# adityaX1412/Experiment-YOLO

Hardware: AMD Instinct MI355X
Metric: images/sec (train) DEAL-YOLO-N 640x640 bs=64/GPU (higher is better)
Workload: dtype f16; 1 GPU; DEAL-YOLO-N (yolov8n-ASF-P2P2.yaml) train step 640x640, per-GPU batch 64, fwd+TAL/WIOU+NWD/DFL/BCE loss+bwd+SGD+EMA, BASELINE.json configs[1]; loss_mode=wiou+nwd, settle_steps=18, capture_retries=0, global_batch=64, parallelism=dp1, hipgraph=True

## Files before the change

### experiment-yolo_amd/csrc/conv_wgrad.hip

```cpp
#include <cstdio>
#include "common.h"
#include "dealyolo_hip.h"

typedef short short4v __attribute__((ext_vector_type(4)));
typedef unsigned int u32x4 __attribute__((ext_vector_type(4)));

struct WgArgs {
  const f16* x;
  const f16* dy;
  float* slabs;
  int ldx, lddy;
  int N, H, W, Ho, Wo;
  int cin_p, cout_p;
  int cin_r8, cout_r8;
  int nci_chunks;
  int tiles_x, tiles_y, ntiles;
  long npix;
  const f16* raw;
  f16* draw;
  const float* coef;
  const double* acc;
  float* dgamma;
  float* dbeta;
  int ldraw, cout;
  float count;
  DySegs xs;
  int dy_csplit;
  unsigned dy_plane;
  const f16* wt;
  f16* dx;
  int lddx, dx_acc;
  int dg_mt, dg_rows;
  DySegs dxs;
};

static __device__ __forceinline__ half8 tr_frag(const char* base0, const char* base1) {
  union {
    short4v s[2];
    half8 h;
  } u;
  u.s[0] = __builtin_amdgcn_ds_read_tr16_b64_v4i16((LDS_AS short4v*)(base0));
  u.s[1] = __builtin_amdgcn_ds_read_tr16_b64_v4i16((LDS_AS short4v*)(base1));
  return u.h;
}

static constexpr __host__ __device__ int wg_th(int ks, int stride, int nci, int mtc) {
  if (ks == 1) return (nci + mtc <= 4) ? 8 : 4;
  if (stride == 1) return (nci * mtc <= 1) ? 16 : ((nci + mtc <= 4) ? 8 : 4);
  return (nci * mtc <= 1) ? 8 : ((nci + mtc <= 4) ? 4 : 2);
}

template <int KS, int STRIDE, int NCI, int MTC, int BNF>
__global__ __launch_bounds__(256, (BNF & 8) ? 3 : ((KS == 3 && NCI * MTC >= 16) ? 1 : 2)) void conv_wgrad_kernel(const WgArgs a) {
  constexpr bool FLAT = (KS == 1);
  constexpr bool DG = (BNF & 4) != 0;
  constexpr bool NOX = (BNF & 8) != 0;
  static_assert(!NOX || DG, "the form without X exists for the fused input gradient only");
  constexpr bool BN1 = ((BNF & 3) == 1 || (BNF & 3) == 3);
  constexpr bool XSEG = ((BNF & 3) == 3);
  static_assert(!DG || (KS == 1 && BN1), "the fused input gradient exists for the 1x1 BatchNorm forms");
  constexpr int TAPS = KS * KS;
  constexpr int NCOL = NCI * TAPS;
  constexpr int CPW = (NCOL + 3) / 4;
  constexpr int TH = wg_th(KS, STRIDE, NCI, MTC), TW = 32;
  constexpr int HWX = FLAT ? TH * TW : (TW - 1) * STRIDE + KS;
  constexpr int HHX = FLAT ? 1 : (TH - 1) * STRIDE + KS;
  constexpr int PAD = KS / 2;
  constexpr int CIN_C = 16 * NCI, COUT_C = 16 * MTC;
  constexpr int PSX = (STRIDE == 2) ? CIN_C * 2 + 16 : (((CIN_C / 2 + 7) / 16) * 16 + 8) * 4;
  constexpr int PSY = (((COUT_C / 2 + 7) / 16) * 16 + 8) * 4;
  constexpr int XBYTES = NOX ? 0 : HHX * HWX * PSX, YBYTES = TH * TW * PSY;
  __shared__ __attribute__((aligned(16))) char smem[XBYTES + YBYTES];
  char* const sx = smem;
  char* const sy = smem + XBYTES;
  __shared__ __attribute__((aligned(16))) float sbn[BN1 ? 4 * COUT_C : (BNF == 2 ? 256 * 8 : 4)];
  float bsum[8] = {0.f, 0.f, 0.f, 0.f, 0.f, 0.f, 0.f, 0.f};
  (void)bsum;
  constexpr int DKS = MTC == 4 ? 2 : (MTC == 3 ? 3 : 1), DCPK = (MTC & 1) ? 16 : 32;
  constexpr int DNT = TH / 2;
  constexpr int DNC = 4 * NCI;
  constexpr int DXROW = CIN_C * 2 + 16;
  constexpr int DPPR = CIN_C / 8;
  constexpr int DPIXPASS = 64 / DPPR > 16 ? 16 : 64 / DPPR;
  constexpr int DNPASS = (16 + DPIXPASS - 1) / DPIXPASS;
  __shared__ __attribute__((aligned(16))) char sdx[DG ? 4 * 16 * DXROW : 16];

  const int tid = threadIdx.x, wave = tid >> 6, lane = tid & 63, p = lane & 15, q = lane >> 4;
  const int qq = p >> 2, pp = p & 3;
  const int co_chunk = blockIdx.y / a.nci_chunks, ci_chunk = blockIdx.y - co_chunk * a.nci_chunks;
  const int ci0 = ci_chunk * CIN_C, co0 = co_chunk * COUT_C;

  f32x4 acc[NOX ? 1 : MTC][NOX ? 1 : CPW];
  if (!NOX) {
#pragma unroll
    for (int m = 0; m < MTC; ++m)
#pragma unroll
      for (int c = 0; c < CPW; ++c) acc[NOX ? 0 : m][NOX ? 0 : c] = (f32x4){0.f, 0.f, 0.f, 0.f};
  }
  (void)acc;

  constexpr int NGX = HHX * HWX * (CIN_C / 8), NGY = TH * TW * (COUT_C / 8);
  constexpr int NPX = NOX ? 1 : (NGX + 255) / 256, NPY = (NGY + 255) / 256;
  uint4 pfx[NPX], pfy[NPY];
  uint4 pfr[BN1 ? NPY : 1];
  unsigned roff[BN1 ? NPY : 1];
  int ncur = 0, nnext = 0;
  (void)ncur; (void)nnext;
  unsigned vnext = 0, vcur = 0, ornext = 0, orcur = 0;
  (void)pfr; (void)roff; (void)vnext; (void)vcur; (void)ornext; (void)orcur;
  constexpr unsigned NEVER = 0x80000000u;
  constexpr int CPGX = CIN_C / 8, CPGY = COUT_C / 8;
  unsigned xoff[NPX], yoff[NPY];
  (void)pfx; (void)xoff;
#pragma unroll
  for (int i = 0; i < NPX; ++i) {
    const int id = tid + i * 256;
    const int pixel = id / CPGX, part = id - pixel * CPGX;
    const bool ok = !NOX && id < NGX && ci0 + part * 8 < a.cin_r8;
    const int hy = FLAT ? 0 : pixel / HWX, hx = FLAT ? pixel : pixel - hy * HWX;
    xoff[i] = ok ? (unsigned)(((hy * a.W + hx) * a.ldx + ci0 + part * 8) * 2) : NEVER;
  }
  constexpr bool XIN = XSEG && !NOX;
  const char* xb[XIN ? NPX : 1];
  int xl[XIN ? NPX : 1];
  unsigned xup = 0;
  bool any_up = false;
  if (XIN)
    for (int k = 0; k < a.xs.nseg; ++k) any_up = any_up || (a.xs.acc[k] & 2);
  (void)xb; (void)xl; (void)xup; (void)any_up;
  if (XIN) {
#pragma unroll
    for (int i = 0; i < NPX; ++i) {
      const int id = tid + i * 256;
      const int part = id % CPGX, ch = ci0 + part * 8;
      int sg = 0;
      while (sg + 1 < a.xs.nseg && ch >= a.xs.c_end[sg]) ++sg;
      const int cb = sg ? a.xs.c_end[sg - 1] : 0;
      const bool ok = id < NGX && ch < a.cin_r8;
      xb[XIN ? i : 0] = ok ? reinterpret_cast<const char*>(a.xs.ptr[sg]) + (ch - cb) * 2 : nullptr;
      xl[XIN ? i : 0] = a.xs.ld[sg] * 2;
      if (ok && (a.xs.acc[sg] & 2)) xup |= 1u << i;
    }
  }
#pragma unroll
  for (int i = 0; i < NPY; ++i) {
    const int id = tid + i * 256;
    const int pixel = id / CPGY, part = id - pixel * CPGY;
    const bool ok = id < NGY && co0 + part * 8 < a.cout_r8;
    const int ty = FLAT ? 0 : pixel / TW, tx = FLAT ? pixel : pixel - ty * TW;
    yoff[i] = ok ? (unsigned)(((ty * a.Wo + tx) * a.lddy + co0 + part * 8) * 2) : NEVER;
    if (FLAT && BN1 && a.dy_csplit && ok) {
      const int ch = co0 + part * 8;
      yoff[i] = (unsigned)((tx * a.lddy + (ch < a.dy_csplit ? ch : ch - a.dy_csplit)) * 2) + (ch < a.dy_csplit ? 0u : a.dy_plane);
    }
    if (BN1) roff[i] = ok ? (unsigned)(((ty * a.Wo + tx) * a.ldraw + co0 + part * 8) * 2) : NEVER;
  }
  if (BN1) {
    for (int c = tid; c < COUT_C; c += 256) {
      const int ch = co0 + c;
      float sc = 0.f, sh = 0.f, kb = 0.f, kc = 0.f;
      if (ch < a.cout) {
        double s1 = 0.0, s2 = 0.0;
#pragma unroll
        for (int k = 0; k < DY_BN_COPIES; ++k) {
          s1 += a.acc[(size_t)(k * 2 + 0) * a.cout + ch];
          s2 += a.acc[(size_t)(k * 2 + 1) * a.cout + ch];
        }
        const float mg = (float)(s1 / a.count), mgx = (float)(s2 / a.count);
        sc = a.coef[ch];
        sh = a.coef[a.cout + ch];
        const float mean = a.coef[2 * a.cout + ch], inv = a.coef[3 * a.cout + ch];
        kb = sc * inv * mgx;
        kc = sc * mg - kb * mean;
        if (!NOX && blockIdx.x == 0 && ci_chunk == 0) {
          if (a.dbeta) a.dbeta[ch] = (float)s1;
          if (a.dgamma) a.dgamma[ch] = (float)s2;
        }
      }
      sbn[c] = sc;
      sbn[COUT_C + c] = sh;
      sbn[2 * COUT_C + c] = kb;
      sbn[3 * COUT_C + c] = kc;
    }
    __syncthreads();
  }
  half8 wf[DG ? DKS : 1][DG ? NCI : 1];
  unsigned dboff[DG ? DKS : 1];
  char* dxb = nullptr;
  unsigned dxld2 = 0;
  bool dxacc = false, dxadd = false;
  const int dpix = lane / DPPR, dpiece = lane - dpix * DPPR;
  (void)wf; (void)dboff; (void)dxb; (void)dxld2; (void)dxacc; (void)dxadd; (void)dpix; (void)dpiece;
  if (DG) {
#pragma unroll
    for (int k = 0; k < DKS; ++k) {
      dboff[DG ? k : 0] = (unsigned)((k * DCPK + ((q * 8) & (DCPK - 1))) * 2);
#pragma unroll
      for (int j = 0; j < NCI; ++j) {
        const int ch = ci0 + (p >> 2) * DNC + 4 * j + (p & 3);
        const int gw = 16 * a.dg_mt, g = ch / gw, rem = ch - g * gw;
        const int row = g * gw + ((rem % (4 * a.dg_mt)) >> 2) * 16 + (rem / (4 * a.dg_mt)) * 4 + (rem & 3);
        const int grow = (g * DKS + k) * gw + (row - g * gw);
        half8 v;
#pragma unroll
        for (int e = 0; e < 8; ++e) v[e] = (f16)0.f;
        if (row < a.dg_rows) v = *reinterpret_cast<const half8*>(a.wt + ((size_t)grow * 32 + q * 8));
        wf[DG ? k : 0][DG ? j : 0] = v;
      }
    }
    const int chn = ci0 + dpiece * 8;
    if (lane < DPIXPASS * DPPR && chn < a.cin_r8) {
      if (XSEG) {
        int sg = 0;
        while (sg + 1 < a.dxs.nseg && chn >= a.dxs.c_end[sg]) ++sg;
        const int cb = sg ? a.dxs.c_end[sg - 1] : 0;
        dxb = reinterpret_cast<char*>(const_cast<void*>(a.dxs.ptr[sg])) + (chn - cb) * 2;
        dxld2 = (unsigned)a.dxs.ld[sg] * 2u;
        dxacc = a.dxs.acc[sg] != 0;
      } else {
        dxb = reinterpret_cast<char*>(a.dx) + chn * 2;
        dxld2 = (unsigned)a.lddx * 2u;
        dxacc = a.dx_acc != 0;
      }
    }
    if (XSEG) {
      for (int k = 0; k < a.dxs.nseg; ++k) dxadd = dxadd || a.dxs.acc[k] != 0;
    } else {
      dxadd = a.dx_acc != 0;
    }
  }
  union DU4 { uint4 u; half2_ h[4]; };
  DU4 dold[DG ? DNT : 1][DG ? DNPASS : 1];
  (void)dold;
  auto ld16 = [](__amdgpu_buffer_rsrc_t r, unsigned off) {
    const auto v = __builtin_amdgcn_raw_buffer_load_b128(r, (int)off, 0, 0);
    return *reinterpret_cast<const uint4*>(&v);
  };
  auto prefetch = [&](int tile) {
    if (FLAT) {
      const auto rx = __builtin_amdgcn_make_buffer_rsrc(const_cast<f16*>(a.x), 0, (int)((unsigned)a.npix * (unsigned)a.ldx * 2u), 0x00020000);
      const auto ry = __builtin_amdgcn_make_buffer_rsrc(const_cast<f16*>(a.dy), 0, (int)((unsigned)a.npix * (unsigned)a.lddy * 2u + (a.dy_csplit ? a.dy_plane : 0u)), 0x00020000);
      const unsigned ox = (unsigned)tile * (TH * TW) * a.ldx * 2u, oy = (unsigned)tile * (TH * TW) * a.lddy * 2u;
      if (NOX) {
      } else if (XIN) {
        const long p0 = (long)tile * (TH * TW);
        int n0 = 0, y0 = 0, x0 = 0;
        if (any_up) {
          const int hw = a.H * a.W, g0 = (int)p0;
          n0 = g0 / hw;
          const int r0 = g0 - n0 * hw;
          y0 = r0 / a.W;
          x0 = r0 - y0 * a.W;
        }
        const float invW = 1.0f / (float)a.W, invH = 1.0f / (float)a.H;
#pragma unroll
        for (int i = 0; i < NPX; ++i) {
          const int lp = (tid + i * 256) / CPGX;
          long gp = p0 + lp;
          const bool inside = gp < a.npix;
          if ((xup >> i) & 1u) {
            const int xx = x0 + lp, dy_ = (int)(((float)xx + 0.5f) * invW), x = xx - dy_ * a.W;
            const int yt = y0 + dy_, dn = (int)(((float)yt + 0.5f) * invH), y = yt - dn * a.H;
            gp = ((long)(n0 + dn) * (a.H >> 1) + (y >> 1)) * (a.W >> 1) + (x >> 1);
          }
          const char* src = xb[XIN ? i : 0];
          pfx[i] = (src && inside) ? *reinterpret_cast<const uint4*>(src + gp * xl[XIN ? i : 0]) : make_uint4(0, 0, 0, 0);
        }
      } else {
#pragma unroll
        for (int i = 0; i < NPX; ++i) pfx[i] = ld16(rx, xoff[i] + ox);
      }
#pragma unroll
      for (int i = 0; i < NPY; ++i) pfy[i] = ld16(ry, yoff[i] + oy);
      if (BN1) {
        const unsigned nbytes = (unsigned)a.npix * (unsigned)a.ldraw * 2u;
        const auto rr = __builtin_amdgcn_make_buffer_rsrc(const_cast<f16*>(a.raw), 0, (int)nbytes, 0x00020000);
        ornext = (unsigned)tile * (TH * TW) * a.ldraw * 2u;
        vnext = 0;
#pragma unroll
        for (int i = 0; i < NPY; ++i) {
          const unsigned off = roff[i] + ornext;
          pfr[i] = ld16(rr, off);
          vnext |= (roff[i] != NEVER && off < nbytes) ? (1u << i) : 0u;
        }
      }
    } else {
      const int bx = tile % a.tiles_x;
      const int t2 = tile / a.tiles_x;
      const int n = t2 / a.tiles_y;
      const int oy0 = (t2 % a.tiles_y) * TH, ox0 = bx * TW;
      const int iy0 = oy0 * STRIDE - PAD, ix0 = ox0 * STRIDE - PAD;
      const auto rx = __builtin_amdgcn_make_buffer_rsrc(const_cast<f16*>(a.x) + (size_t)n * a.H * a.W * a.ldx, 0, a.H * a.W * a.ldx * 2, 0x00020000);
      const auto ry = __builtin_amdgcn_make_buffer_rsrc(const_cast<f16*>(a.dy) + (size_t)n * a.Ho * a.Wo * a.lddy, 0, a.Ho * a.Wo * a.lddy * 2, 0x00020000);
      const unsigned ox = (unsigned)((iy0 * a.W + ix0) * a.ldx * 2), oy = (unsigned)((oy0 * a.Wo + ox0) * a.lddy * 2);
      if (ix0 >= 0 && ix0 + HWX <= a.W) {
#pragma unroll
        for (int i = 0; i < NPX; ++i) pfx[i] = ld16(rx, xoff[i] + ox);
      } else {
#pragma unroll
        for (int i = 0; i < NPX; ++i) {
          const int hx = ((tid + i * 256) / CPGX) % HWX;
          pfx[i] = ld16(rx, (unsigned)(ix0 + hx) < (unsigned)a.W ? xoff[i] + ox : NEVER);
        }
      }
      if (ox0 + TW <= a.Wo) {
#pragma unroll
        for (int i = 0; i < NPY; ++i) pfy[i] = ld16(ry, yoff[i] + oy);
      } else {
#pragma unroll
        for (int i = 0; i < NPY; ++i) {
          const int tx = ((tid + i * 256) / CPGY) % TW;
          pfy[i] = ld16(ry, ox0 + tx < a.Wo ? yoff[i] + oy : NEVER);
        }
      }
      if (BN1) {
        const unsigned nbytes = (unsigned)(a.Ho * a.Wo * a.ldraw * 2);
        const auto rr = __builtin_amdgcn_make_buffer_rsrc(const_cast<f16*>(a.raw) + (size_t)n * a.Ho * a.Wo * a.ldraw, 0, (int)nbytes, 0x00020000);
        ornext = (unsigned)((oy0 * a.Wo + ox0) * a.ldraw * 2);
        vnext = 0;
        const bool xfull = ox0 + TW <= a.Wo;
#pragma unroll
        for (int i = 0; i < NPY; ++i) {
          unsigned off = roff[i] == NEVER ? NEVER : roff[i] + ornext;
          if (!xfull) {
            const int tx = ((tid + i * 256) / CPGY) % TW;
            off = ox0 + tx < a.Wo ? off : NEVER;
          }
          pfr[i] = ld16(rr, off);
          vnext |= off < nbytes ? (1u << i) : 0u;
        }
        nnext = n;
      }
    }
  };


  int tile = (!FLAT && !(gridDim.x & 7)) ? (int)(blockIdx.x & 7) * (int)(gridDim.x >> 3) + (int)(blockIdx.x >> 3) : (int)blockIdx.x;
  if (tile < a.ntiles) prefetch(tile);
  for (; tile < a.ntiles; tile += gridDim.x) {
    __syncthreads();
#pragma unroll
    for (int i = 0; i < NPX; ++i) {
      const int id = tid + i * 256;
      if (!NOX && id < NGX) *reinterpret_cast<uint4*>(sx + (id / (CIN_C / 8)) * PSX + (id % (CIN_C / 8)) * 16) = pfx[i];
    }
    if (BN1) {
      vcur = vnext; orcur = ornext; ncur = nnext;
      const unsigned nbytes = FLAT ? (unsigned)a.npix * (unsigned)a.ldraw * 2u : (unsigned)(a.Ho * a.Wo * a.ldraw * 2);
      const auto rd = __builtin_amdgcn_make_buffer_rsrc(FLAT ? a.draw : a.draw + (size_t)ncur * a.Ho * a.Wo * a.ldraw, 0, (int)nbytes, 0x00020000);
#pragma unroll
      for (int i = 0; i < NPY; ++i) {
        const int id = tid + i * 256;
        const int part = id % CPGY;
        const bool valid = (vcur >> i) & 1u;
        const float* cf = sbn + part * 8;
        union { half8 h; uint4 u; u32x4 v; } o;
        o.h = bn_bwd_apply8<DY_ACT_SILU>(*reinterpret_cast<const half8*>(&pfy[i]), *reinterpret_cast<const half8*>(&pfr[i]), cf,
                                         cf + COUT_C, cf + 2 * COUT_C, cf + 3 * COUT_C);
        if (!valid) o.u = make_uint4(0, 0, 0, 0);
        if (id < NGY) *reinterpret_cast<uint4*>(sy + (id / (COUT_C / 8)) * PSY + (id % (COUT_C / 8)) * 16) = o.u;
        if (!DG && ci_chunk == 0 && a.draw) __builtin_amdgcn_raw_buffer_store_b128(o.v, rd, (int)(valid ? roff[i] + orcur : NEVER), 0, 0);
      }
    } else {
#pragma unroll
      for (int i = 0; i < NPY; ++i) {
        const int id = tid + i * 256;
        if (id < NGY) *reinterpret_cast<uint4*>(sy + (id / (COUT_C / 8)) * PSY + (id % (COUT_C / 8)) * 16) = pfy[i];
        if (BNF == 2 && id < NGY) {
          const half8 v = *reinterpret_cast<const half8*>(&pfy[i]);
#pragma unroll
          for (int j = 0; j < 8; ++j) bsum[j] += (float)v[j];
        }
      }
    }
    __syncthreads();
    const long dpix0 = (long)tile * (TH * TW) + wave * (16 * DNT);
    (void)dpix0;
    if (DG && dxadd) {
#pragma unroll
      for (int t = 0; t < DNT; ++t)
#pragma unroll
        for (int ps = 0; ps < DNPASS; ++ps) {
          const int rowi = ps * DPIXPASS + dpix;
          const long gp = dpix0 + t * 16 + rowi;
          const bool ok = dxb && dxacc && rowi < 16 && gp < a.npix;
          dold[DG ? t : 0][DG ? ps : 0].u = ok ? *reinterpret_cast<const uint4*>(dxb + (size_t)gp * dxld2) : make_uint4(0, 0, 0, 0);
        }
      __builtin_amdgcn_sched_barrier(0);
    }
    if (tile + (int)gridDim.x < a.ntiles) prefetch(tile + gridDim.x);
    if constexpr (!NOX) {
    const int kpix = 4 * q + qq;
    half8 af[2][MTC], bf[2];
    auto load_a = [&](int buf, int r) {
#pragma unroll
      for (int m = 0; m < MTC; ++m) {
        const char* b0 = sy + (r * TW + kpix) * PSY + (m * 16 + 4 * pp) * 2;
        af[buf][m] = tr_frag(b0, b0 + 16 * PSY);
      }
    };
    auto load_b = [&](int buf, int r, int c) {
      const int col = wave + 4 * c;
      if (col < NCOL) {
        const int cit = col / TAPS, tap = col - cit * TAPS;
        const int dy = tap / KS, dx = tap - dy * KS;
        const char* b0;
        int step;
        if (FLAT) {
          b0 = sx + (r * TW + kpix) * PSX + (cit * 16 + 4 * pp) * 2;
          step = 16 * PSX;
        } else {
          b0 = sx + ((r * STRIDE + dy) * HWX + kpix * STRIDE + dx) * PSX + (cit * 16 + 4 * pp) * 2;
          step = 16 * STRIDE * PSX;
        }
        bf[buf] = tr_frag(b0, b0 + step);
      }
    };
    load_a(0, 0);
    load_b(0, 0, 0);
#pragma unroll
    for (int r = 0; r < TH; ++r) {
      if (r + 1 < TH) load_a((r + 1) & 1, r + 1);
#pragma unroll
      for (int c = 0; c < CPW; ++c) {
        const int lin = r * CPW + c;
        if (c + 1 < CPW) load_b((lin + 1) & 1, r, c + 1);
        else if (r + 1 < TH) load_b((lin + 1) & 1, r + 1, 0);
        __builtin_amdgcn_sched_barrier(0);
        if (wave + 4 * c < NCOL) {
#pragma unroll
          for (int m = 0; m < MTC; ++m)
            acc[NOX ? 0 : m][NOX ? 0 : c] = __builtin_amdgcn_mfma_f32_16x16x32_f16(af[r & 1][m], bf[lin & 1], acc[NOX ? 0 : m][NOX ? 0 : c], 0, 0, 0);
        }
        __builtin_amdgcn_sched_barrier(0);
      }
    }
    }
    if (DG) {
      half8 db[DNT][DKS];
#pragma unroll
      for (int t = 0; t < DNT; ++t)
#pragma unroll
        for (int k = 0; k < DKS; ++k)
          db[t][k] = *reinterpret_cast<const half8*>(sy + ((wave * DNT + t) * 16 + p) * PSY + dboff[DG ? k : 0]);
      f32x4 dacc[NCI][DNT];
#pragma unroll
      for (int j = 0; j < NCI; ++j)
#pragma unroll
        for (int t = 0; t < DNT; ++t) dacc[j][t] = (f32x4){0.f, 0.f, 0.f, 0.f};
#pragma unroll
      for (int k = 0; k < DKS; ++k)
#pragma unroll
        for (int j = 0; j < NCI; ++j)
#pragma unroll
          for (int t = 0; t < DNT; ++t)
            dacc[j][t] = __builtin_amdgcn_mfma_f32_16x16x32_f16(wf[DG ? k : 0][DG ? j : 0], db[t][k], dacc[j][t], 0, 0, 0);
      typedef uint2 __attribute__((may_alias)) uint2_a;
      typedef uint4 __attribute__((may_alias)) uint4_a;
      char* const xs = sdx + wave * (16 * DXROW);
      char* const xw = xs + p * DXROW + q * (DNC * 2);
      const int rrow = dpix < 16 ? dpix : 15;
      auto lds_order = []() {
        __builtin_amdgcn_fence(__ATOMIC_RELEASE, "wavefront", "local");
        __builtin_amdgcn_wave_barrier();
        __builtin_amdgcn_fence(__ATOMIC_ACQUIRE, "wavefront", "local");
      };
#pragma unroll
      for (int t = 0; t < DNT; ++t) {
        union { half2_ h[DNC / 2]; uint2 u2[DNC / 4]; } hv;
#pragma unroll
        for (int j = 0; j < NCI; ++j) {
          const f32x2 lo = {dacc[j][t][0], dacc[j][t][1]}, hi = {dacc[j][t][2], dacc[j][t][3]};
          hv.h[j * 2] = __builtin_convertvector(lo, half2_);
          hv.h[j * 2 + 1] = __builtin_convertvector(hi, half2_);
        }
        lds_order();
#pragma unroll
        for (int j = 0; j < NCI; ++j) reinterpret_cast<uint2_a*>(xw)[j] = hv.u2[j];
        lds_order();
#pragma unroll
        for (int ps = 0; ps < DNPASS; ++ps) {
          const int rowi = ps * DPIXPASS + dpix;
          const int rr = ps * DPIXPASS + rrow < 16 ? ps * DPIXPASS + rrow : 15;
          DU4 v;
          v.u = *reinterpret_cast<const uint4_a*>(xs + rr * DXROW + dpiece * 16);
          const long gp = dpix0 + t * 16 + rowi;
          if (dxadd) {
#pragma unroll
            for (int k = 0; k < 4; ++k)
              v.h[k] = __builtin_convertvector(__builtin_convertvector(v.h[k], f32x2) + __builtin_convertvector(dold[DG ? t : 0][DG ? ps : 0].h[k], f32x2), half2_);
          }
          if (dxb && rowi < 16 && gp < a.npix) *reinterpret_cast<uint4*>(dxb + (size_t)gp * dxld2) = v.u;
        }
      }
    }
  }

  if (BNF == 2 && ci_chunk == 0) {
    __syncthreads();
#pragma unroll
    for (int j = 0; j < 8; ++j) sbn[tid * 8 + j] = bsum[j];
    __syncthreads();
    if (tid < COUT_C && co0 + tid < a.cout) {
      const int part = tid >> 3, j = tid & 7;
      float t = 0.f;
      for (int k = part; k < 256; k += CPGY) t += sbn[k * 8 + j];
      unsafeAtomicAdd(const_cast<double*>(a.acc) + (size_t)(blockIdx.x % DY_BN_COPIES) * a.cout + co0 + tid, (double)t);
    }
  }
  if constexpr (NOX) return;
  float* slab = a.slabs + (size_t)blockIdx.x * TAPS * a.cout_p * a.cin_p;
#pragma unroll
  for (int c = 0; c < CPW; ++c) {
    const int col = wave + 4 * c;
    if (col < NCOL) {
      const int cit = col / TAPS, tap = col - cit * TAPS;
#pragma unroll
      for (int m = 0; m < MTC; ++m)
#pragma unroll
        for (int r = 0; r < 4; ++r) {
          const int co = co0 + m * 16 + q * 4 + r, ci = ci0 + cit * 16 + p;
          slab[((size_t)tap * a.cout_p + co) * a.cin_p + ci] = acc[NOX ? 0 : m][NOX ? 0 : c][r];
        }
    }
  }
}

static __device__ __forceinline__ void wgrad_reduce_block(int block, const float* slabs, int nslabs, float* dw, int cout, int cin,
                                                          int taps, int cout_p, int cin_p, int accumulate,
                                                          int ld_taps, int ld_cphys, int ld_cin) {
  const int lane = threadIdx.x & 63, grp = threadIdx.x >> 6;
  const long S = (long)taps * cout_p * cin_p;
  const long o = (long)block * 64 + lane;
  float s0 = 0.f, s1 = 0.f, s2 = 0.f, s3 = 0.f;
  if (o < S) {
    const float* p = slabs + o;
    int k = grp;
    for (; k + 12 < nslabs; k += 16) {
      s0 += p[(long)k * S];
      s1 += p[(long)(k + 4) * S];
      s2 += p[(long)(k + 8) * S];
      s3 += p[(long)(k + 12) * S];
    }
    for (; k < nslabs; k += 4) s0 += p[(long)k * S];
  }
  __shared__ float red[4][64];
  red[grp][lane] = (s0 + s1) + (s2 + s3);
  __syncthreads();
  if (grp == 0 && o < S) {
    const float tot = (red[0][lane] + red[1][lane]) + (red[2][lane] + red[3][lane]);
    const int ci = (int)(o % cin_p);
    const long t = o / cin_p;
    const int co = (int)(t % cout_p), tap = (int)(t / cout_p);
    if (ld_taps) {
      const int n = ci / ld_cphys, ch = ci - n * ld_cphys;
      if (co < cout && n < ld_taps && ch < ld_cin) {
        float* d = dw + ((long)co * ld_cin + ch) * ld_taps + n;
        *d = accumulate ? *d + tot : tot;
      }
    } else if (co < cout && ci < cin) {
      float* d = dw + ((long)co * cin + ci) * taps + tap;
      *d = accumulate ? *d + tot : tot;
    }
  }
}

__global__ __launch_bounds__(256) void wgrad_reduce_kernel(const float* slabs, int nslabs, float* dw, int cout, int cin,
                                                           int taps, int cout_p, int cin_p, int accumulate,
                                                           int ld_taps, int ld_cphys, int ld_cin) {
  wgrad_reduce_block(blockIdx.x, slabs, nslabs, dw, cout, cin, taps, cout_p, cin_p, accumulate, ld_taps, ld_cphys, ld_cin);
}

struct WgReduceDesc {
  const float* slabs;
  float* dw;
  int nslabs, cout, cin, taps, cout_p, cin_p, accumulate, ld_taps, ld_cphys, ld_cin;
  int first_block, bias_c;
  const double* bias_acc;
  float* dbias;
};
__global__ __launch_bounds__(256) void wgrad_reduce_batched_kernel(const WgReduceDesc* descs, int n) {
  int lo = 0, hi = n - 1;
  while (lo < hi) {
    const int mid = (lo + hi + 1) >> 1;
    if (descs[mid].first_block <= (int)blockIdx.x) lo = mid;
    else hi = mid - 1;
  }
  const WgReduceDesc d = descs[lo];
  if (d.bias_c > 0 && (int)blockIdx.x == d.first_block && (int)threadIdx.x < d.bias_c) {
    double t = 0.0;
#pragma unroll
    for (int k = 0; k < DY_BN_COPIES; ++k) t += d.bias_acc[(size_t)k * d.bias_c + threadIdx.x];
    d.dbias[threadIdx.x] = (float)t;
  }
  wgrad_reduce_block(blockIdx.x - d.first_block, d.slabs, d.nslabs, d.dw, d.cout, d.cin, d.taps, d.cout_p, d.cin_p, d.accumulate,
                     d.ld_taps, d.ld_cphys, d.ld_cin);
}
extern "C" int dy_wgrad_reduce_desc_bytes(void) { return (int)sizeof(WgReduceDesc); }
static void wgrad_geometry(int cin, int cout, int ks, int stride, int* cin_p, int* cout_p, int* nci, int* mtc, long npix_out = 0);
extern "C" int dy_wgrad_reduce_desc_fill(void* desc, const float* slabs, int nslabs, float* dw, int cin, int cout, int ks, int stride,
                                         int accumulate, int ld_taps, int ld_cphys, int ld_cin, int first_block) {
  if (!desc || !slabs || !dw || nslabs < 1) return DY_ERR_ARG;
  int cp, op, nci, mtc;
  const int cin_eff = ld_taps ? ld_taps * ld_cphys : cin;
  wgrad_geometry(cin_eff, cout, ld_taps ? 1 : ks, ld_taps ? 1 : stride, &cp, &op, &nci, &mtc);
  const int taps = ld_taps ? 1 : ks * ks;
  WgReduceDesc* d = reinterpret_cast<WgReduceDesc*>(desc);
  *d = WgReduceDesc{slabs, dw, nslabs, cout, cin_eff, taps, op, cp, accumulate, ld_taps, ld_cphys, ld_cin, first_block, 0, nullptr, nullptr};
  return cdiv(taps * op * cp, 64);
}
extern "C" int dy_wgrad_reduce_desc_bias(void* desc, const double* bias_acc, float* dbias, int c) {
  if (!desc || !bias_acc || !dbias || c < 1 || c > 256) return DY_ERR_ARG;
  WgReduceDesc* d = reinterpret_cast<WgReduceDesc*>(desc);
  d->bias_acc = bias_acc; d->dbias = dbias; d->bias_c = c;
  return DY_OK;
}
extern "C" int dy_wgrad_reduce_batched(const void* descs_device, int n, int total_blocks, hipStream_t stream) {
  if (n <= 0 || total_blocks <= 0 || !descs_device) return DY_ERR_ARG;
  hipLaunchKernelGGL(wgrad_reduce_batched_kernel, dim3(total_blocks), dim3(256), 0, stream, (const WgReduceDesc*)descs_device, n);
  DY_CHECK_LAUNCH();
  return DY_OK;
}

template <int KS, int STRIDE, int NCI, int MTC>
static int launch_wgrad(const WgArgs& a, int gx, int gy, hipStream_t s) {
  if (a.wt) {
    if constexpr (KS == 1) {
      if (!a.raw || gy != a.nci_chunks) return DY_ERR_ARG;
      if (!a.x) {
        if (a.dxs.nseg > 0) hipLaunchKernelGGL((conv_wgrad_kernel<KS, STRIDE, NCI, MTC, 15>), dim3(gx, gy), dim3(256), 0, s, a);
        else hipLaunchKernelGGL((conv_wgrad_kernel<KS, STRIDE, NCI, MTC, 13>), dim3(gx, gy), dim3(256), 0, s, a);
      } else if (a.xs.nseg > 0) hipLaunchKernelGGL((conv_wgrad_kernel<KS, STRIDE, NCI, MTC, 7>), dim3(gx, gy), dim3(256), 0, s, a);
      else hipLaunchKernelGGL((conv_wgrad_kernel<KS, STRIDE, NCI, MTC, 5>), dim3(gx, gy), dim3(256), 0, s, a);
    } else return DY_ERR_ARG;
  } else if (a.raw && a.xs.nseg > 0) {
    if constexpr (KS == 1) hipLaunchKernelGGL((conv_wgrad_kernel<KS, STRIDE, NCI, MTC, 3>), dim3(gx, gy), dim3(256), 0, s, a);
    else return DY_ERR_ARG;
  } else if (a.raw) hipLaunchKernelGGL((conv_wgrad_kernel<KS, STRIDE, NCI, MTC, 1>), dim3(gx, gy), dim3(256), 0, s, a);
  else if (a.acc && MTC != 3) hipLaunchKernelGGL((conv_wgrad_kernel<KS, STRIDE, NCI, MTC, 2>), dim3(gx, gy), dim3(256), 0, s, a);
  else if (a.acc) return DY_ERR_ARG;
  else hipLaunchKernelGGL((conv_wgrad_kernel<KS, STRIDE, NCI, MTC, 0>), dim3(gx, gy), dim3(256), 0, s, a);
  DY_CHECK_LAUNCH();
  return DY_OK;
}
template <int KS, int STRIDE>
static int dispatch_wgrad(int nci, int mtc, const WgArgs& a, int gx, int gy, hipStream_t s) {
#define DY_CASE(I, M) \
  if (nci == I && mtc == M) return launch_wgrad<KS, STRIDE, I, M>(a, gx, gy, s);
  DY_CASE(1, 1) DY_CASE(1, 2) DY_CASE(1, 4)
  DY_CASE(2, 1) DY_CASE(2, 2) DY_CASE(2, 4)
  if (!(KS == 3 && STRIDE == 2)) { DY_CASE(4, 1) DY_CASE(4, 2) DY_CASE(4, 4) }
  if (KS == 1) {
    DY_CASE(3, 1) DY_CASE(3, 2) DY_CASE(3, 4) DY_CASE(1, 3) DY_CASE(2, 3) DY_CASE(4, 3) DY_CASE(3, 3)
  }
#undef DY_CASE
  return DY_ERR_ARG;
}

static int wgrad_per_cu(int ks, int nci, int mtc) {
  static const int light = getenv("DY_WGRAD_LIGHT_WGS") ? atoi(getenv("DY_WGRAD_LIGHT_WGS")) : 2;
  if (ks == 3 && nci * mtc >= 16) return 1;
  return nci * mtc <= 2 ? light : 2;
}
static long wgrad_columns(int ks, int nci, int mtc, int cp, int op) {
  const int gy = (cp / (16 * nci)) * (op / (16 * mtc));
  const int per_cu = wgrad_per_cu(ks, nci, mtc);
  int gx = (256 * per_cu) / gy;
  return gx < 32 ? 32 : gx;
}
static void wgrad_geometry(int cin, int cout, int ks, int stride, int* cin_p, int* cout_p, int* nci, int* mtc, long npix_out) {
  *cin_p = (cin + 15) / 16 * 16;
  *cout_p = (cout + 15) / 16 * 16;
  const int cit = *cin_p / 16, cot = *cout_p / 16;
  const int cap = (ks == 3 && stride == 2) ? 2 : 4;
  *nci = (cit % 4 == 0 && cap >= 4) ? 4 : ((ks == 1 && cit % 3 == 0) ? 3 : (cit % 2 == 0 ? 2 : 1));
  *mtc = cot % 4 == 0 ? 4 : ((ks == 1 && cot % 3 == 0) ? 3 : (cot % 2 == 0 ? 2 : 1));
  static const bool split = !(getenv("DY_WGRAD_SPLIT") && atoi(getenv("DY_WGRAD_SPLIT")) == 0);
  static const double f = getenv("DY_WGRAD_SPLIT_F") ? atof(getenv("DY_WGRAD_SPLIT_F")) : 2.0;
  if (!split || npix_out <= 0) return;
  const double wbytes = (double)ks * ks * *cin_p * *cout_p * 4.0;
  const double act = (double)npix_out * (*cin_p * stride * stride + *cout_p) * 2.0;
  while (2.0 * wgrad_columns(ks, *nci, *mtc, *cin_p, *cout_p) * wbytes > f * act) {
    if (*mtc % 2 == 0 && *mtc >= *nci) *mtc /= 2;
    else if (*nci % 2 == 0) *nci /= 2;
    else if (*mtc % 2 == 0) *mtc /= 2;
    else break;
  }
}

extern "C" int dy_wgrad_workspace(int n, int h, int w, int cin, int cout, int ks, int stride, int* nslabs,
                                  long* slab_elems) {
  int cp, op, nci, mtc;
  const int pad = ks / 2, Ho = (h + 2 * pad - ks) / stride + 1, Wo = (w + 2 * pad - ks) / stride + 1;
  wgrad_geometry(cin, cout, ks, stride, &cp, &op, &nci, &mtc, (long)n * Ho * Wo);
  const int th = wg_th(ks, stride, nci, mtc);
  int ntiles;
  if (ks == 1) ntiles = (int)(((long)n * Ho * Wo + th * 32 - 1) / (th * 32));
  else ntiles = cdiv(Wo, 32) * cdiv(Ho, th) * n;
  *slab_elems = (long)ks * ks * cp * op;
  const int gy = (cp / (16 * nci)) * (op / (16 * mtc));
  const int per_cu = wgrad_per_cu(ks, nci, mtc);
  int gx = (256 * per_cu) / gy;
  if (gx < 32) gx = 32;
  static const int tpb = getenv("DY_WGRAD_TPB") ? atoi(getenv("DY_WGRAD_TPB")) : 1;
  if (tpb > 1 && gx > ntiles / tpb) gx = ntiles / tpb > 32 ? ntiles / tpb : (ntiles < 32 ? ntiles : 32);
  if (gx > ntiles) gx = ntiles;
  if (gx < 1) gx = 1;
  *nslabs = gx;
  return DY_OK;
}

struct WgBnHost {
  const void* raw; void* draw; const float* coef; const double* acc; float* dgamma; float* dbeta; int ldraw; float count;
  const DySegs* xs = nullptr;
  int dy_csplit = 0;
  unsigned dy_plane = 0;
  const void* wt = nullptr; void* dx = nullptr; int lddx = 0, dx_acc = 0; const DySegs* dxs = nullptr;
  bool dgrad_only = false;
};
static int conv_wgrad_impl(const void* x, int ldx, const void* dy, int lddy, float* slabs, float* dw, int n, int h, int w,
                           int cin, int cout, int ks, int stride, int accumulate, int ld_taps, int ld_cphys, int ld_cin,
                           hipStream_t stream, const WgBnHost* bn = nullptr);

extern "C" int dy_wgrad_kernel_name(int cin, int cout, int ks, int stride, char* out, int cap) {
  if (!out || cap < 8) return DY_ERR_ARG;
  int cp, op, nci, mtc;
  wgrad_geometry(cin, cout, ks, stride, &cp, &op, &nci, &mtc);
  snprintf(out, cap, "conv_wgrad_kernel<%d, %d, %d, %d, 0>", ks, stride, nci, mtc);
  return DY_OK;
}

extern "C" int dy_wgrad_kernel_name_at(int n, int h, int w, int cin, int cout, int ks, int stride, char* out, int cap) {
  if (!out || cap < 8) return DY_ERR_ARG;
  int cp, op, nci, mtc;
  wgrad_geometry(cin, cout, ks, stride, &cp, &op, &nci, &mtc,
                 (long)n * ((h + 2 * (ks / 2) - ks) / stride + 1) * ((w + 2 * (ks / 2) - ks) / stride + 1));
  snprintf(out, cap, "conv_wgrad_kernel<%d, %d, %d, %d, 0>", ks, stride, nci, mtc);
  return DY_OK;
}

extern "C" int dy_conv_wgrad(const void* x, int ldx, const void* dy, int lddy, float* slabs, float* dw, int n, int h,
                             int w, int cin, int cout, int ks, int stride, int accumulate, hipStream_t stream) {
  return conv_wgrad_impl(x, ldx, dy, lddy, slabs, dw, n, h, w, cin, cout, ks, stride, accumulate, 0, 0, 0, stream);
}
extern "C" int dy_conv_wgrad_ld(const void* x, int ldx, const void* dy, int lddy, float* slabs, float* dw, int n, int h,
                                int w, int cout, int ld_cin, int ld_taps, int ld_cphys, int accumulate, hipStream_t stream) {
  return conv_wgrad_impl(x, ldx, dy, lddy, slabs, dw, n, h, w, ld_taps * ld_cphys, cout, 1, 1, accumulate, ld_taps, ld_cphys,
                         ld_cin, stream);
}

extern "C" int dy_conv_wgrad_bn(const void* x, int ldx, const void* dy, int lddy, const void* raw, int ldraw, void* draw,
                                const float* coef, const double* acc, float* dgamma, float* dbeta, float count, float* slabs,
                                float* dw, int n, int h, int w, int cin, int cout, int ks, int stride, int accumulate,
                                hipStream_t stream) {
  if (!raw || !coef || !acc || (ldraw & 7) || ((uintptr_t)raw & 15) || ((uintptr_t)draw & 15) || (cout & 15)) return DY_ERR_ARG;
  const WgBnHost bn{raw, draw, coef, acc, dgamma, dbeta, ldraw, count};
  return conv_wgrad_impl(x, ldx, dy, lddy, slabs, dw, n, h, w, cin, cout, ks, stride, accumulate, 0, 0, 0, stream, &bn);
}
extern "C" int dy_conv_wgrad_bias(const void* x, int ldx, const void* dy, int lddy, double* bias_acc, float* slabs, float* dw, int n,
                                  int h, int w, int cin, int cout, int ks, int stride, int accumulate, hipStream_t stream) {
  if (!bias_acc) return DY_ERR_ARG;
  const WgBnHost bn{nullptr, nullptr, nullptr, bias_acc, nullptr, nullptr, 0, 1.f};
  return conv_wgrad_impl(x, ldx, dy, lddy, slabs, dw, n, h, w, cin, cout, ks, stride, accumulate, 0, 0, 0, stream, &bn);
}
extern "C" int dy_conv1x1_wgrad_bn_segs(const DySegs* xs, const void* dy, int lddy, const void* raw, int ldraw, void* draw, const float* coef,
                                        const double* acc, float* dgamma, float* dbeta, float count, float* slabs, float* dw, int n, int h,
                                        int w, int cin, int cout, int accumulate, hipStream_t stream) {
  if (!raw || !coef || !acc || (ldraw & 7) || ((uintptr_t)raw & 15) || ((uintptr_t)draw & 15) || (cout & 15)) return DY_ERR_ARG;
  if (!xs || xs->nseg < 1 || xs->nseg > DY_MAX_SEGS || xs->c_end[xs->nseg - 1] != cin) return DY_ERR_ARG;
  for (int k = 0; k < xs->nseg; ++k)
    if ((xs->c_end[k] & 7) || (xs->ld[k] & 7) || !xs->ptr[k] || ((uintptr_t)xs->ptr[k] & 15) || xs->c_end[k] <= (k ? xs->c_end[k - 1] : 0) ||
        ((xs->acc[k] & 2) && ((h | w) & 1))) return DY_ERR_ARG;
  WgBnHost bn{raw, draw, coef, acc, dgamma, dbeta, ldraw, count};
  bn.xs = xs;
  return conv_wgrad_impl(xs->ptr[0], 8, dy, lddy, slabs, dw, n, h, w, cin, cout, 1, 1, accumulate, 0, 0, 0, stream, &bn);
}
extern "C" int dy_conv1x1_wgrad_bn_planes(const DySegs* xs, const void* x, int ldx, const void* dy, const void* dy2, int lddy, int csplit,
                                          const void* raw, int ldraw, void* draw, const float* coef, const double* acc, float* dgamma,
                                          float* dbeta, float count, float* slabs, float* dw, int n, int h, int w, int cin, int cout,
                                          int accumulate, hipStream_t stream) {
  if (!raw || !coef || !acc || (ldraw & 7) || ((uintptr_t)raw & 15) || ((uintptr_t)draw & 15) || (cout & 15)) return DY_ERR_ARG;
  if (!dy || !dy2 || (csplit & 7) || csplit <= 0 || csplit >= cout || ((uintptr_t)dy2 & 15)) return DY_ERR_ARG;
  const long plane = (const char*)dy2 - (const char*)dy;
  if (plane < (long)n * h * w * lddy * 2 || plane + (double)n * h * w * lddy * 2.0 >= 2147483648.0) return DY_ERR_ARG;
  if (xs) {
    if (xs->nseg < 1 || xs->nseg > DY_MAX_SEGS || xs->c_end[xs->nseg - 1] != cin) return DY_ERR_ARG;
    for (int k = 0; k < xs->nseg; ++k)
      if ((xs->c_end[k] & 7) || (xs->ld[k] & 7) || !xs->ptr[k] || ((uintptr_t)xs->ptr[k] & 15) || xs->c_end[k] <= (k ? xs->c_end[k - 1] : 0) ||
          ((xs->acc[k] & 2) && ((h | w) & 1))) return DY_ERR_ARG;
  }
  WgBnHost bn{raw, draw, coef, acc, dgamma, dbeta, ldraw, count};
  bn.xs = xs;
  bn.dy_csplit = csplit; bn.dy_plane = (unsigned)plane;
  return conv_wgrad_impl(xs ? xs->ptr[0] : x, xs ? 8 : ldx, dy, lddy, slabs, dw, n, h, w, cin, cout, 1, 1, accumulate, 0, 0, 0, stream, &bn);
}

struct WgDgPlan { int ok, nci, mtc, dg_mt, dg_rows; };
static WgDgPlan wgrad_dgrad_plan(int n, int h, int w, int cin, int cout) {
  WgDgPlan r{};
  if (n < 1 || h < 1 || w < 1 || cin < 8 || (cin & 7) || cout < 16 || (cout & 15) || cout > 64) return r;
  int cp, op, nci, mtc;
  wgrad_geometry(cin, cout, 1, 1, &cp, &op, &nci, &mtc, (long)n * h * w);
  if (16 * mtc != op) return r;
  int gcin, gcout, cc, nch, mt, ng, kst, pe;
  if (dy_conv_geometry(cout, cin, 1, 1, &gcin, &gcout, &cc, &nch, &mt, &ng, &kst, &pe) != DY_OK) return r;
  const int dks = mtc == 4 ? 2 : (mtc == 3 ? 3 : 1), dcpk = (mtc & 1) ? 16 : 32;
  if (gcin != cout || nch * kst != dks || (cc < 32 ? cc : 32) != dcpk || gcout < cp) return r;
  r.ok = 1; r.nci = nci; r.mtc = mtc; r.dg_mt = mt; r.dg_rows = gcout;
  return r;
}
extern "C" int dy_conv1x1_wgrad_dgrad_supported(int n, int h, int w, int cin, int cout) { return wgrad_dgrad_plan(n, h, w, cin, cout).ok; }
extern "C" int dy_wgrad_dgrad_kernel_name(int n, int h, int w, int cin, int cout, int segs, char* out, int cap) {
  const WgDgPlan pl = wgrad_dgrad_plan(n, h, w, cin, cout);
  if (!out || cap < 8 || !pl.ok) return DY_ERR_ARG;
  snprintf(out, cap, "conv_wgrad_kernel<1, 1, %d, %d, %d>", pl.nci, pl.mtc, segs ? 7 : 5);
  return DY_OK;
}
static bool dgrad_segs_valid(const DySegs* xs, const DySegs* dxs) {
  if (!xs || !dxs || dxs->nseg != xs->nseg) return false;
  for (int k = 0; k < dxs->nseg; ++k) {
    const int cb = k ? dxs->c_end[k - 1] : 0;
    if (dxs->c_end[k] != xs->c_end[k] || (dxs->ld[k] & 7) || dxs->ld[k] < dxs->c_end[k] - cb || !dxs->ptr[k] || ((uintptr_t)dxs->ptr[k] & 15) ||
        (dxs->acc[k] & ~1)) return false;
  }
  return true;
}
static bool segs_in_valid(const DySegs* xs, int cin, int h, int w) {
  if (!xs || xs->nseg < 1 || xs->nseg > DY_MAX_SEGS || xs->c_end[xs->nseg - 1] != cin) return false;
  for (int k = 0; k < xs->nseg; ++k)
    if ((xs->c_end[k] & 7) || (xs->ld[k] & 7) || !xs->ptr[k] || ((uintptr_t)xs->ptr[k] & 15) || xs->c_end[k] <= (k ? xs->c_end[k - 1] : 0) ||
        ((xs->acc[k] & 2) && ((h | w) & 1))) return false;
  return true;
}
static int dgrad_only_columns(int ntiles, int gy) {
  int gx = (256 * 3) / (gy > 0 ? gy : 1);
  if (gx < 32) gx = 32;
  if (gx > ntiles) gx = ntiles;
  return gx < 1 ? 1 : gx;
}
extern "C" int dy_conv1x1_dgrad_bn_supported(int n, int h, int w, int cin, int cout) { return wgrad_dgrad_plan(n, h, w, cin, cout).ok; }
extern "C" int dy_dgrad_only_kernel_name(int n, int h, int w, int cin, int cout, int segs, char* out, int cap) {
  const WgDgPlan pl = wgrad_dgrad_plan(n, h, w, cin, cout);
  if (!out || cap < 8 || !pl.ok) return DY_ERR_ARG;
  snprintf(out, cap, "conv_wgrad_kernel<1, 1, %d, %d, %d>", pl.nci, pl.mtc, segs ? 15 : 13);
  return DY_OK;
}
extern "C" int dy_conv1x1_dgrad_bn(const void* dy, const void* dy2, int lddy, int csplit, const void* raw, int ldraw, const float* coef,
                                   const double* acc, float count, const void* w_packed_t, void* dx, int lddx, int dx_accumulate,
                                   const DySegs* dxs, int n, int h, int w, int cin, int cout, hipStream_t stream) {
  if (!dy || !raw || !coef || !acc || (ldraw & 7) || ((uintptr_t)raw & 15)) return DY_ERR_ARG;
  if (!w_packed_t || ((uintptr_t)w_packed_t & 15) || !wgrad_dgrad_plan(n, h, w, cin, cout).ok) return DY_ERR_ARG;
  long plane = 0;
  if (dy2) {
    if ((csplit & 7) || csplit <= 0 || csplit >= cout || ((uintptr_t)dy2 & 15)) return DY_ERR_ARG;
    plane = (const char*)dy2 - (const char*)dy;
    if (plane < (long)n * h * w * lddy * 2 || plane + (double)n * h * w * lddy * 2.0 >= 2147483648.0) return DY_ERR_ARG;
  } else if (csplit) {
    return DY_ERR_ARG;
  }
  if (dxs) {
    if (dxs->nseg < 1 || dxs->nseg > DY_MAX_SEGS || dxs->c_end[dxs->nseg - 1] != cin) return DY_ERR_ARG;
    for (int k = 0; k < dxs->nseg; ++k) {
      const int cb = k ? dxs->c_end[k - 1] : 0;
      if ((dxs->c_end[k] & 7) || dxs->c_end[k] <= cb || (dxs->ld[k] & 7) || dxs->ld[k] < dxs->c_end[k] - cb || !dxs->ptr[k] ||
          ((uintptr_t)dxs->ptr[k] & 15) || (dxs->acc[k] & ~1)) return DY_ERR_ARG;
    }
  } else if (!dx || ((uintptr_t)dx & 15) || (lddx & 7) || lddx < cin || (double)n * h * w * lddx * 2.0 >= 2147483648.0) {
    return DY_ERR_ARG;
  }
  WgBnHost bn{raw, nullptr, coef, acc, nullptr, nullptr, ldraw, count};
  bn.dy_csplit = dy2 ? csplit : 0; bn.dy_plane = (unsigned)plane;
  bn.wt = w_packed_t; bn.dxs = dxs; bn.dx = dxs ? nullptr : dx; bn.lddx = lddx; bn.dx_acc = dx_accumulate != 0;
  bn.dgrad_only = true;
  return conv_wgrad_impl(nullptr, 8, dy, lddy, nullptr, nullptr, n, h, w, cin, cout, 1, 1, 0, 0, 0, 0, stream, &bn);
}
extern "C" int dy_conv1x1_wgrad_dgrad_bn(const void* x, int ldx, const void* dy, int lddy, const void* raw, int ldraw, const float* coef,
                                         const double* acc, float* dgamma, float* dbeta, float count, float* slabs, float* dw,
                                         const void* w_packed_t, void* dx, int lddx, int dx_accumulate, int n, int h, int w, int cin,
                                         int cout, int accumulate, hipStream_t stream) {
  if (!raw || !coef || !acc || (ldraw & 7) || ((uintptr_t)raw & 15)) return DY_ERR_ARG;
  if (!w_packed_t || ((uintptr_t)w_packed_t & 15) || !dx || ((uintptr_t)dx & 15) || (lddx & 7) || lddx < cin) return DY_ERR_ARG;
  if (!wgrad_dgrad_plan(n, h, w, cin, cout).ok || (double)n * h * w * lddx * 2.0 >= 2147483648.0) return DY_ERR_ARG;
  WgBnHost bn{raw, nullptr, coef, acc, dgamma, dbeta, ldraw, count};
  bn.wt = w_packed_t; bn.dx = dx; bn.lddx = lddx; bn.dx_acc = dx_accumulate != 0;
  return conv_wgrad_impl(x, ldx, dy, lddy, slabs, dw, n, h, w, cin, cout, 1, 1, accumulate, 0, 0, 0, stream, &bn);
}
extern "C" int dy_conv1x1_wgrad_dgrad_bn_segs(const DySegs* xs, const void* dy, int lddy, const void* raw, int ldraw, const float* coef,
                                              const double* acc, float* dgamma, float* dbeta, float count, float* slabs, float* dw,
                                              const void* w_packed_t, const DySegs* dxs, int n, int h, int w, int cin, int cout,
                                              int accumulate, hipStream_t stream) {
  if (!raw || !coef || !acc || (ldraw & 7) || ((uintptr_t)raw & 15)) return DY_ERR_ARG;
  if (!w_packed_t || ((uintptr_t)w_packed_t & 15) || !segs_in_valid(xs, cin, h, w) || !dgrad_segs_valid(xs, dxs)) return DY_ERR_ARG;
  if (!wgrad_dgrad_plan(n, h, w, cin, cout).ok) return DY_ERR_ARG;
  WgBnHost bn{raw, nullptr, coef, acc, dgamma, dbeta, ldraw, count};
  bn.xs = xs; bn.wt = w_packed_t; bn.dxs = dxs;
  return conv_wgrad_impl(xs->ptr[0], 8, dy, lddy, slabs, dw, n, h, w, cin, cout, 1, 1, accumulate, 0, 0, 0, stream, &bn);
}
extern "C" int dy_conv1x1_wgrad_dgrad_bn_planes(const DySegs* xs, const void* x, int ldx, const void* dy, const void* dy2, int lddy, int csplit,
                                                const void* raw, int ldraw, const float* coef, const double* acc, float* dgamma,
                                                float* dbeta, float count, float* slabs, float* dw, const void* w_packed_t, void* dx,
                                                int lddx, int dx_accumulate, const DySegs* dxs, int n, int h, int w, int cin, int cout,
                                                int accumulate, hipStream_t stream) {
  if (!raw || !coef || !acc || (ldraw & 7) || ((uintptr_t)raw & 15)) return DY_ERR_ARG;
  if (!dy || !dy2 || (csplit & 7) || csplit <= 0 || csplit >= cout || ((uintptr_t)dy2 & 15)) return DY_ERR_ARG;
  const long plane = (const char*)dy2 - (const char*)dy;
  if (plane < (long)n * h * w * lddy * 2 || plane + (double)n * h * w * lddy * 2.0 >= 2147483648.0) return DY_ERR_ARG;
  if (!w_packed_t || ((uintptr_t)w_packed_t & 15) || !wgrad_dgrad_plan(n, h, w, cin, cout).ok) return DY_ERR_ARG;
  if (xs) {
    if (!segs_in_valid(xs, cin, h, w) || !dgrad_segs_valid(xs, dxs)) return DY_ERR_ARG;
  } else if (dxs || !dx || ((uintptr_t)dx & 15) || (lddx & 7) || lddx < cin || (double)n * h * w * lddx * 2.0 >= 2147483648.0) {
    return DY_ERR_ARG;
  }
  WgBnHost bn{raw, nullptr, coef, acc, dgamma, dbeta, ldraw, count};
  bn.xs = xs; bn.dy_csplit = csplit; bn.dy_plane = (unsigned)plane;
  bn.wt = w_packed_t; bn.dxs = xs ? dxs : nullptr; bn.dx = xs ? nullptr : dx; bn.lddx = lddx; bn.dx_acc = dx_accumulate != 0;
  return conv_wgrad_impl(xs ? xs->ptr[0] : x, xs ? 8 : ldx, dy, lddy, slabs, dw, n, h, w, cin, cout, 1, 1, accumulate, 0, 0, 0, stream, &bn);
}
extern "C" int dy_conv_wgrad_ld_bn(const void* x, int ldx, const void* dy, int lddy, const void* raw, int ldraw, void* draw,
                                   const float* coef, const double* acc, float* dgamma, float* dbeta, float count, float* slabs,
                                   float* dw, int n, int h, int w, int cout, int ld_cin, int ld_taps, int ld_cphys, int accumulate,
                                   hipStream_t stream) {
  if (!raw || !coef || !acc || (ldraw & 7) || ((uintptr_t)raw & 15) || ((uintptr_t)draw & 15) || (cout & 15)) return DY_ERR_ARG;
  const WgBnHost bn{raw, draw, coef, acc, dgamma, dbeta, ldraw, count};
  return conv_wgrad_impl(x, ldx, dy, lddy, slabs, dw, n, h, w, ld_taps * ld_cphys, cout, 1, 1, accumulate, ld_taps, ld_cphys, ld_cin,
                         stream, &bn);
}

static int conv_wgrad_impl(const void* x, int ldx, const void* dy, int lddy, float* slabs, float* dw, int n, int h, int w,
                           int cin, int cout, int ks, int stride, int accumulate, int ld_taps, int ld_cphys, int ld_cin,
                           hipStream_t stream, const WgBnHost* bn) {
  if (!(ks == 1 || ks == 3) || !(stride == 1 || stride == 2) || (ks == 1 && stride != 1)) return DY_ERR_ARG;
  if ((ldx & 7) || (lddy & 7) || ((uintptr_t)x & 15) || ((uintptr_t)dy & 15)) return DY_ERR_ALIGN;
  const bool dgrad_only = bn && bn->dgrad_only;
  if (dgrad_only != (x == nullptr) || (dgrad_only && (!bn->wt || slabs || dw))) return DY_ERR_ARG;
  if ((ks == 1 ? (double)n : 1.0) * h * w * (ldx > lddy ? ldx : lddy) * 2.0 >= 2147483648.0) return DY_ERR_ARG;
  int cp, op, nci, mtc;
  wgrad_geometry(cin, cout, ks, stride, &cp, &op, &nci, &mtc,
                 (long)n * ((h + 2 * (ks / 2) - ks) / stride + 1) * ((w + 2 * (ks / 2) - ks) / stride + 1));
  WgArgs a{};
  a.x = (const f16*)x; a.dy = (const f16*)dy; a.slabs = slabs; a.ldx = ldx; a.lddy = lddy;
  a.N = n; a.H = h; a.W = w;
  const int pad = ks / 2;
  a.Ho = (h + 2 * pad - ks) / stride + 1;
  a.Wo = (w + 2 * pad - ks) / stride + 1;
  a.cin_p = cp; a.cout_p = op;
  a.cin_r8 = (cin + 7) / 8 * 8; a.cout_r8 = (cout + 7) / 8 * 8;
  if (bn) {
    if ((ks == 1 ? (double)n : 1.0) * a.Ho * a.Wo * bn->ldraw * 2.0 >= 2147483648.0) return DY_ERR_ARG;
    a.raw = (const f16*)bn->raw; a.draw = (f16*)bn->draw; a.coef = bn->coef; a.acc = bn->acc;
    a.dgamma = bn->dgamma; a.dbeta = bn->dbeta; a.ldraw = bn->ldraw; a.count = bn->count;
    a.cout = bn->raw ? cout : (cout + 7) / 8 * 8;
    if (bn->xs) a.xs = *bn->xs;
    a.dy_csplit = bn->dy_csplit; a.dy_plane = bn->dy_plane;
    if (bn->wt) {
      const WgDgPlan pl = wgrad_dgrad_plan(n, h, w, cin, cout);
      if (!pl.ok || pl.nci != nci || pl.mtc != mtc || ks != 1 || ld_taps) return DY_ERR_ARG;
      a.wt = (const f16*)bn->wt; a.dx = (f16*)bn->dx; a.lddx = bn->lddx; a.dx_acc = bn->dx_acc;
      a.dg_mt = pl.dg_mt; a.dg_rows = pl.dg_rows;
      if (bn->dxs) a.dxs = *bn->dxs;
    }
  }
  a.nci_chunks = cp / (16 * nci);
  const int nco_chunks = op / (16 * mtc);
  const int th = wg_th(ks, stride, nci, mtc);
  if (ks == 1) {
    a.npix = (long)n * a.Ho * a.Wo;
    a.ntiles = (int)((a.npix + th * 32 - 1) / (th * 32));
  } else {
    a.tiles_x = cdiv(a.Wo, 32);
    a.tiles_y = cdiv(a.Ho, th);
    a.ntiles = a.tiles_x * a.tiles_y * n;
  }
  int nslabs;
  long slab_elems;
  dy_wgrad_workspace(n, h, w, cin, cout, ks, stride, &nslabs, &slab_elems);
  const int gy = a.nci_chunks * nco_chunks;
  if (dgrad_only) nslabs = dgrad_only_columns(a.ntiles, gy);
  int rc;
  if (ks == 1) rc = dispatch_wgrad<1, 1>(nci, mtc, a, nslabs, gy, stream);
  else if (stride == 1) rc = dispatch_wgrad<3, 1>(nci, mtc, a, nslabs, gy, stream);
  else rc = dispatch_wgrad<3, 2>(nci, mtc, a, nslabs, gy, stream);
  if (rc != DY_OK) return rc;
  if (!dw) return DY_OK;
  const int total = ks * ks * op * cp;
  hipLaunchKernelGGL(wgrad_reduce_kernel, dim3(cdiv(total, 64)), dim3(256), 0, stream, slabs, nslabs, dw, cout, cin,
                     ks * ks, op, cp, accumulate, ld_taps, ld_cphys, ld_cin);
  DY_CHECK_LAUNCH();
  return DY_OK;
}
```

### experiment-yolo_amd/ultralytics/hip/__init__.py

```python
from __future__ import annotations

import ctypes as C
import os
import sys

_FLAG = "DEBUG_CLR_GRAPH_PACKET_CAPTURE"


def _hip_already_up():
    t = sys.modules.get("torch")
    try:
        return bool(t is not None and t.cuda.is_initialized())
    except Exception:
        return False


if os.environ.get(_FLAG) is None and not _hip_already_up():
    os.environ[_FLAG] = "0"
GRAPH_SAFE = os.environ.get(_FLAG) == "0"

_HERE = os.path.dirname(os.path.abspath(__file__))
LIB_PATH = os.environ.get("DY_HIP_LIB") or os.path.normpath(os.path.join(_HERE, "..", "..", "csrc", "libdealyolo_hip.so"))

DY_EPI_STATS, DY_EPI_BIAS, DY_EPI_SILU, DY_EPI_F32OUT, DY_EPI_ACCUM, DY_EPI_STATS_ACC = 1, 2, 4, 8, 16, 32
DY_BN_COPIES = 16
DY_ACT_NONE, DY_ACT_SILU, DY_ACT_LEAKY = 0, 1, 2
_ERR = {-1: "DY_ERR_ARG (unsupported shape/argument)", -2: "DY_ERR_LAUNCH (HIP launch failed)",
        -3: "DY_ERR_ALIGN (pointer/stride alignment)", -4: "DY_ERR_CAPACITY (more items than the kernel's table holds)"}

vp, i32, f32, i64, sz = C.c_void_p, C.c_int, C.c_float, C.c_long, C.c_size_t
ip = C.POINTER(C.c_int)
lp = C.POINTER(C.c_long)


class DyLossArgs(C.Structure):
    _fields_ = [("nl", i32), ("B", i32), ("nc", i32), ("ncp", i32), ("nmax", i32),
                ("box", vp * 4), ("cls", vp * 4), ("dbox", vp * 4), ("dcls", vp * 4),
                ("H", i32 * 4), ("W", i32 * 4), ("stride", f32 * 4),
                ("t_batch_idx", vp), ("t_cls", vp), ("t_boxes", vp), ("n_targets", i32), ("n_targets_dev", vp),
                ("img_w", f32), ("img_h", f32), ("hyp_box", f32), ("hyp_cls", f32), ("hyp_dfl", f32),
                ("use_wiou", i32), ("use_nwd", i32), ("iou_ratio", f32), ("gscale", vp), ("scalars", vp),
                ("workspace", vp), ("dbox_rows_only", i32), ("box_from_input", i32), ("box_in", vp * 4), ("box_in_ld", i32 * 4),
                ("box_w", vp * 4), ("box_b", vp * 4), ("box_in_coef", vp * 4),
                ("box_family", i32), ("box_ltype", i32), ("box_fm", i32), ("box_modifier", i32), ("inner_ratio", f32),
                ("focaler_d", f32), ("focaler_u", f32), ("shape_scale", f32), ("piou_lambda", f32)]


class DySegs(C.Structure):
    _fields_ = [("nseg", i32), ("c_end", i32 * 8), ("ld", i32 * 8), ("acc", i32 * 8), ("ptr", vp * 8)]


SIGNATURES = {
    "dy_abi_version": (i32, []),
    "dy_loss_args_bytes": (i32, []),
    "dy_conv_geometry": (i32, [i32, i32, i32, i32, ip, ip, ip, ip, ip, ip, ip, ip]),
    "dy_pack_weights": (i32, [vp, vp, vp, i32, i32, i32, i32, i32, vp]),
    "dy_pack_desc_bytes": (i32, []),
    "dy_pack_desc_fill": (i32, [vp, vp, vp, vp, i32, i32, i32, i32, i32, i32, i32, i32]),
    "dy_pack_weights_batched": (i32, [vp, i32, i32, vp]),
    "dy_conv_forward": (i32, [vp, i32, vp, vp, vp, i32, vp, i32, i32, i32, i32, i32, i32, i32, i32, i32, i32, i32, ip, vp]),
    "dy_segs_bytes": (i32, []),
    "dy_conv1x1_segs_supported": (i32, [i32, i32, C.POINTER(DySegs)]),
    "dy_conv1x1_forward_segs": (i32, [C.POINTER(DySegs), vp, vp, vp, i32, vp, i32, i32, i32, i32, i32, i32, vp]),
    "dy_conv1x1_input_grad_segs": (i32, [vp, i32, vp, C.POINTER(DySegs), i32, i32, i32, i32, i32, vp]),
    "dy_conv1x1_wgrad_bn_segs": (i32, [C.POINTER(DySegs), vp, i32, vp, i32, vp, vp, vp, vp, vp, f32, vp, vp, i32, i32, i32, i32, i32, i32, vp]),
    "dy_conv_res_supported": (i32, [i32, i32, i32, i32]),
    "dy_conv_forward_res": (i32, [vp, i32, vp, vp, vp, i32, vp, i32, i32, i32, i32, i32, i32, i32, i32, vp]),
    "dy_conv_red_supported": (i32, [i32, i32, i32]),
    "dy_conv_input_grad_red": (i32, [vp, i32, vp, vp, i32, i32, i32, i32, i32, i32, i32, vp, i32, vp, vp, i32, vp]),
    "dy_conv_kernel_name": (i32, [i32, i32, i32, i32, C.c_char_p, i32]),
    "dy_conv1x1_segs_kernel_name": (i32, [i32, i32, C.POINTER(DySegs), C.c_char_p, i32]),
    "dy_conv1x1_kernel_name_live": (i32, [i32, i32, i32, i32, i32, i32, C.POINTER(DySegs), C.POINTER(DySegs), C.c_char_p, i32]),
    "dy_conv_kernel_name_at": (i32, [i32, i32, i32, i32, i32, i32, i32, C.c_char_p, i32]),
    "dy_wgrad_kernel_name": (i32, [i32, i32, i32, i32, C.c_char_p, i32]),
    "dy_wgrad_kernel_name_at": (i32, [i32, i32, i32, i32, i32, i32, i32, C.c_char_p, i32]),
    "dy_wgrad_reduce_desc_bytes": (i32, []),
    "dy_wgrad_reduce_desc_fill": (i32, [vp, vp, i32, vp, i32, i32, i32, i32, i32, i32, i32, i32, i32]),
    "dy_wgrad_reduce_batched": (i32, [vp, i32, i32, vp]),
    "dy_match_predictions": (i32, [vp, vp, vp, vp, vp, i32, vp, vp, i32, i32, i32, i32, vp, vp, vp, vp]),
    "dy_box_iou": (i32, [vp, i32, vp, i32, vp, vp]),
    "dy_conv_num_partials": (i32, [i32, i32, i32, i32, i32, i32, i32, i32]),
    "dy_wgrad_workspace": (i32, [i32, i32, i32, i32, i32, i32, i32, ip, lp]),
    "dy_conv_wgrad": (i32, [vp, i32, vp, i32, vp, vp, i32, i32, i32, i32, i32, i32, i32, i32, vp]),
    "dy_stem_grid": (i32, [i32, i32, i32]),
    "dy_stem_forward": (i32, [vp, vp, vp, i32, vp, i32, i32, i32, f32, vp]),
    "dy_stem_forward_eval": (i32, [vp, vp, vp, vp, i32, i32, i32, i32, f32, i32, vp]),
    "dy_stem_wgrad_bn": (i32, [vp, vp, i32, vp, i32, vp, vp, vp, vp, f32, vp, i32, i32, i32, f32, vp]),
    "dy_conv_wgrad_bias": (i32, [vp, i32, vp, i32, vp, vp, vp, i32, i32, i32, i32, i32, i32, i32, i32, vp]),
    "dy_wgrad_reduce_desc_bias": (i32, [vp, vp, vp, i32]),
    "dy_conv_wgrad_bn": (i32, [vp, i32, vp, i32, vp, i32, vp, vp, vp, vp, vp, f32, vp, vp, i32, i32, i32, i32, i32, i32, i32, i32, vp]),
    "dy_conv_wgrad_ld_bn": (i32, [vp, i32, vp, i32, vp, i32, vp, vp, vp, vp, vp, f32, vp, vp, i32, i32, i32, i32, i32, i32, i32, i32, vp]),
    "dy_ldconv_sample": (i32, [vp, i32, vp, i32, vp, vp, i32, i32, i32, i32, i32, i32, i32, i32, i32, vp]),
    "dy_ldconv_sample_backward": (i32, [vp, i32, vp, i32, vp, vp, i32, vp, vp, i32, i32, i32, i32, i32, i32, i32, i32, i32, vp]),
    "dy_ldconv_sample_backward_gather": (i32, [vp, i32, vp, i32, vp, vp, i32, vp, i32, i32, vp, vp, i32, vp, i32, i32, i32, i32, i32, i32, i32, i32, i32, vp]),
    "dy_f32_to_f16_add": (i32, [vp, vp, i32, i64, i32, i32, vp]),
    "dy_pack_weights_ld": (i32, [vp, vp, i32, i32, i32, i32, i32, vp]),
    "dy_conv_wgrad_ld": (i32, [vp, i32, vp, i32, vp, vp, i32, i32, i32, i32, i32, i32, i32, i32, vp]),
    "dy_bn_finalize": (i32, [vp, i32, f32, vp, i32, f32, vp, i32, f32, vp, vp, vp, vp, vp, i32, f32, f32, f32, i32, vp]),
    "dy_bn_eval_coef": (i32, [vp, vp, vp, vp, vp, i32, f32, vp]),
    "dy_bn_act_apply": (i32, [vp, i32, vp, i32, vp, i32, vp, i64, i32, i32, vp]),
    "dy_bn_act_apply_acc": (i32, [vp, i32, vp, i32, vp, i32, vp, vp, vp, vp, vp, vp, i64, i32, i32, f32, f32, f32, vp]),
    "dy_bn_act_bwd_reduce_acc": (i32, [vp, i32, vp, i32, vp, vp, i64, i32, i32, vp, i32, i32, vp]),
    "dy_bn_act_bwd_apply_acc": (i32, [vp, i32, vp, i32, vp, i32, vp, vp, vp, vp, i64, i32, i32, f32, vp]),
    "dy_bn_act_bwd_reduce": (i32, [vp, i32, vp, i32, vp, vp, i32, i64, i32, i32, ip, vp]),
    "dy_bn_bwd_finalize": (i32, [vp, i32, vp, vp, vp, i32, f32, i32, vp]),
    "dy_bn_act_bwd_apply": (i32, [vp, i32, vp, i32, vp, i32, vp, vp, i64, i32, i32, i32, vp]),
    "dy_bn_finalize_ld": (i32, [vp, i32, i32, vp, vp, vp, vp, vp, i32, f32, f32, f32, i32, vp, vp]),
    "dy_bn_act_apply_c": (i32, [vp, i32, vp, i32, vp, i32, vp, i64, i32, i32, vp]),
    "dy_bn_act_bwd_reduce_c": (i32, [vp, i32, vp, i32, vp, vp, i32, i64, i32, i32, ip, vp]),
    "dy_bn_bwd_finalize_ld": (i32, [vp, i32, i32, vp, vp, vp, i32, f32, i32, vp]),
    "dy_bn_act_bwd_apply_c": (i32, [vp, i32, vp, i32, vp, i32, vp, vp, i64, i32, i32, i32, vp]),
    "dy_pad_f32": (i32, [vp, i32, vp, i32, vp]),
    "dy_import_image": (i32, [vp, vp, i32, i32, i32, i32, i32, f32, vp]),
    "dy_crop_letterbox_u8": (i32, [vp, i32, i32, vp, vp, i32, i32, vp, vp]),
    "dy_refine_select": (i32, [vp, vp, vp, vp, vp, i32, C.c_float, C.c_float, vp, vp, vp]),
    "dy_nms_hard": (i32, [vp, vp, vp, i32, C.c_float, vp, vp]),
    "dy_crop_letterbox_u8_multi": (i32, [vp, vp, vp, vp, vp, vp, i32, i32, vp, vp]),
    "dy_refine_select_multi": (i32, [vp, vp, vp, vp, vp, vp, vp, i32, vp, vp, vp]),
    "dy_two_stage_merge": (i32, [vp, vp, vp, vp, vp, vp, i32, f32, vp, vp, f32, i32, vp, vp, vp, vp]),
    "dy_tile_gather_f32": (i32, [vp, vp, vp, vp, vp, vp, vp, i32, i32, vp, vp]),
    "dy_tile_merge": (i32, [vp, vp, vp, vp, vp, i32, i32, i32, f32, i32, i32, vp, vp, vp, vp, vp]),
    "dy_warp_import_u8": (i32, [vp, vp, vp, i32, i32, i32, vp]),
    "dy_warp_slot_bytes": (i32, []),
    "dy_import_image_u8": (i32, [vp, vp, i32, i32, i32, i32, vp, vp, vp, vp]),
    "dy_add": (i32, [vp, i32, vp, i32, vp, i32, vp, i32, i64, i32, vp]),
    "dy_upsample2x": (i32, [vp, i32, vp, i32, i32, i32, i32, i32, i32, i32, vp]),
    "dy_space_to_depth": (i32, [vp, i32, vp, i32, i32, i32, i32, i32, i32, i32, vp]),
    "dy_dysample_supported": (i32, [i32, i32, i32]),
    "dy_dysample": (i32, [vp, i32, vp, i32, vp, i32, i32, i32, i32, i32, i32, i32, vp]),
    "dy_dysample_backward": (i32, [vp, i32, vp, i32, vp, i32, vp, i32, i32, vp, vp, i32, vp, i32, i32, i32, i32, i32, i32, i32, vp]),
    "dy_maxpool5": (i32, [vp, i32, vp, i32, vp, i32, i32, i32, i32, vp]),
    "dy_maxpool5_backward": (i32, [vp, i32, vp, vp, i32, i32, i32, i32, i32, i32, vp]),
    "dy_bn_group_max": (i32, []),
    "dy_bn_act_apply_acc_split": (i32, [vp, i32, vp, i32, vp, i32, i32, vp, vp, vp, vp, vp, vp, i64, i32, i32, f32, f32, f32, vp]),
    "dy_bn_act_bwd_reduce_acc_split": (i32, [vp, i32, vp, i32, i32, vp, i32, vp, vp, i64, i32, i32, vp]),
    "dy_conv1x1_wgrad_bn_planes": (i32, [C.POINTER(DySegs), vp, i32, vp, vp, i32, i32, vp, i32, vp, vp, vp, vp, vp, f32, vp, vp, i32, i32, i32,
                                         i32, i32, i32, vp]),
    "dy_conv1x1_wgrad_dgrad_supported": (i32, [i32, i32, i32, i32, i32]),
    "dy_wgrad_dgrad_kernel_name": (i32, [i32, i32, i32, i32, i32, i32, C.c_char_p, i32]),
    "dy_conv1x1_wgrad_dgrad_bn": (i32, [vp, i32, vp, i32, vp, i32, vp, vp, vp, vp, f32, vp, vp, vp, vp, i32, i32, i32, i32, i32, i32, i32, i32, vp]),
    "dy_conv1x1_wgrad_dgrad_bn_segs": (i32, [C.POINTER(DySegs), vp, i32, vp, i32, vp, vp, vp, vp, f32, vp, vp, vp, C.POINTER(DySegs), i32, i32,
                                             i32, i32, i32, i32, vp]),
    "dy_conv1x1_wgrad_dgrad_bn_planes": (i32, [C.POINTER(DySegs), vp, i32, vp, vp, i32, i32, vp, i32, vp, vp, vp, vp, f32, vp, vp, vp, vp, i32, i32,
                                               C.POINTER(DySegs), i32, i32, i32, i32, i32, i32, vp]),
    "dy_conv1x1_dgrad_bn_supported": (i32, [i32, i32, i32, i32, i32]),
    "dy_dgrad_only_kernel_name": (i32, [i32, i32, i32, i32, i32, i32, C.c_char_p, i32]),
    "dy_conv1x1_dgrad_bn": (i32, [vp, vp, i32, i32, vp, i32, vp, vp, f32, vp, vp, i32, i32, C.POINTER(DySegs), i32, i32, i32, i32, i32, vp]),
    "dy_bn_act_apply_acc_group": (i32, [i32, vp, vp, vp, vp, vp, vp, vp, vp, vp, vp, vp, vp, vp, vp, vp, vp]),
    "dy_bn_act_bwd_reduce_acc_group": (i32, [i32, vp, vp, vp, vp, vp, vp, vp, vp, vp]),
    "dy_bn_act_bwd_reduce_rows": (i32, [vp, i32, vp, i32, vp, vp, i32, i32, i32, i32, vp, i32, i32, vp]),
    "dy_head_box_decode": (i32, [vp, i32, vp, vp, vp, vp, i32, i32, i32, i32, i32, i32, i32, vp]),
    "dy_cls_head_supported": (i32, [i32, i32]),
    "dy_cls_head_slabs": (i32, []),
    "dy_cls_head_forward": (i32, [vp, i32, vp, vp, vp, vp, i64, i32, i32, vp]),
    "dy_cls_head_backward": (i32, [vp, i32, vp, vp, vp, vp, i32, i32, vp, vp, i64, i32, i32, vp]),
    "dy_head_box_decode_levels": (i32, [i32, vp, vp, vp, vp, vp, vp, i32, vp, i32, vp, vp, i32, i32, vp]),
    "dy_conv1x1_rows_backward_levels": (i32, [i32, vp, vp, vp, vp, vp, vp, i32, vp, vp, vp, vp, vp, vp, vp, i32, vp, vp, i32, i32, vp]),
    "dy_cls_head_forward_levels": (i32, [i32, vp, vp, vp, vp, vp, vp, vp, i32, i32, vp]),
    "dy_cls_head_backward_levels": (i32, [i32, vp, vp, vp, vp, vp, vp, vp, vp, vp, vp, vp, i32, i32, vp]),
    "dy_conv1x1_rows_supported": (i32, [i32, i32]),
    "dy_conv1x1_rows_slabs": (i32, [i32, i32, i32]),
    "dy_conv1x1_rows_backward": (i32, [vp, i32, vp, vp, i32, vp, i32, i32, vp, vp, i32, i32, vp, vp, i32, i32, i32, i32, i32, vp]),
    "dy_sppf_pool3_supported": (i32, [i32, i32, i32]),
    "dy_sppf_pool3": (i32, [vp, i32, i32, vp, vp, vp, i32, i32, i32, vp]),
    "dy_sppf_pool3_backward": (i32, [vp, i32, i32, vp, vp, vp, i32, i32, i32, i32, i32, i32, vp]),
    "dy_scalseq_tail": (i32, [vp, i32, vp, i32, vp, i32, vp, i32, vp, i32, vp, i32, i32, i32, i32, vp]),
    "dy_scalseq_tail_backward": (i32, [vp, i32, vp, i32, vp, i32, vp, i32, vp, i32, vp, vp, vp, i32, i32, i32, i32, i32,
                                       i32, i32, ip, vp]),
    "dy_scalseq_tail_backward_all": (i32, [vp, i32, vp, i32, vp, i32, vp, i32, vp, i32, vp, i32, vp, i32, vp, vp, vp, i32, i32,
                                           i32, i32, i32, i32, ip, vp]),
    "dy_scalseq_bwd_grid_cap": (i32, [i32]),
    "dy_zoom_pool": (i32, [vp, i32, vp, i32, i32, i32, i32, i32, vp]),
    "dy_zoom_pool_backward": (i32, [vp, i32, vp, i32, vp, i32, i32, i32, i32, i32, i32, vp]),
    "dy_copy_slice": (i32, [vp, i32, vp, i32, i64, i32, vp]),
    "dy_fill_zero": (i32, [vp, sz, vp]),
    "dy_loss_workspace_bytes": (sz, [i32, i32, i32]),
    "dy_loss_workspace_layout": (i32, [i32, i32, i32, C.POINTER(sz), C.POINTER(sz), C.POINTER(sz)]),
    "dy_detection_loss": (i32, [C.POINTER(DyLossArgs), vp]),
    "dy_tal_assign": (i32, [vp, ip, ip, C.POINTER(f32), i32, i32, i32, i32, i32, vp, vp, vp, vp, vp, vp, vp, vp]),
    "dy_head_infer_supported": (i32, [i32, i32, i32, i32]),
    "dy_head_infer_levels": (i32, [i32, vp, vp, vp, vp, vp, vp, vp, vp, vp, vp, vp, i32, i32, i32, vp, vp]),
    "dy_head_infer_levels_logits": (i32, [i32, vp, vp, vp, vp, vp, vp, vp, vp, vp, vp, vp, i32, i32, i32, vp, vp, vp, vp]),
    "dy_decode_predictions": (i32, [vp, vp, ip, ip, C.POINTER(f32), i32, i32, i32, i32, vp, vp]),
    "dy_nms_candidates": (i32, [vp, i32, i32, i32, f32, i32, vp, i32, vp, vp, vp, vp, i32, vp]),
    "dy_nms_presort_workspace": (sz, [i32, i32]),
    "dy_nms_presort": (i32, [vp, vp, vp, vp, i32, i32, i32, vp, vp, vp, vp, vp]),
    "dy_soft_nms": (i32, [vp, vp, vp, vp, vp, vp, vp, vp, i32, i32, f32, f32, f32, f32, vp]),
    "dy_set_hyper": (i32, [vp, vp, vp]),
    "dy_optimizer_step": (i32, [vp, vp, vp, vp, vp, i64, i64, i64, vp, vp, vp, i64, vp, vp, vp, i32, vp]),
    "dy_optimizer_step_seg": (i32, [vp, vp, vp, vp, vp, i64, lp, vp, vp, vp, i64, vp, vp, vp, i32, vp]),
    "dy_axpy_f32": (i32, [vp, vp, f32, i64, vp]),
    "dy_scale_img": (i32, [vp, i32, i32, i32, i32, i32, i32, i32, i32, vp, vp]),
    "dy_tta_merge": (i32, [i32, C.POINTER(vp), ip, ip, ip, C.POINTER(f32), ip, i32, i32, i32, i32, vp, vp]),
    "dy_bootstrap_ap": (i32, [vp, vp, vp, vp, vp, i32, i32, i32, i32, vp, vp, vp]),
    "dy_confusion_matrix": (i32, [vp, vp, i32, vp, vp, vp, i32, vp, i32, i32, i32, i32, f32, f32, i32, vp, vp, vp]),
    "dy_count_fp": (i32, [vp, vp, vp, vp, vp, i32, f32, C.c_double, vp, vp, vp]),
}

_LIB = None


def lib():
    global _LIB
    if _LIB is None:
        if not os.path.exists(LIB_PATH):
            raise RuntimeError(
                f"{LIB_PATH} not found. The DEAL-YOLO hot path has no CPU/PyTorch fallback: build the HIP library "
                f"first (python -c 'import __graft_entry__ as g; g.build()' or `make -C experiment-yolo_amd/csrc`).")
        L = C.CDLL(LIB_PATH)
        for name, (res, args) in SIGNATURES.items():
            fn = getattr(L, name)
            fn.restype, fn.argtypes = res, args
        if L.dy_segs_bytes() != C.sizeof(DySegs):
            raise RuntimeError(f"{LIB_PATH} lays DySegs out in {L.dy_segs_bytes()} bytes, this binding in {C.sizeof(DySegs)}: rebuild the library")
        if L.dy_loss_args_bytes() != C.sizeof(DyLossArgs):
            raise RuntimeError(f"{LIB_PATH} was built with a DyLossArgs of {L.dy_loss_args_bytes()} bytes, this binding lays out "
                               f"{C.sizeof(DyLossArgs)}: rebuild the library (make -C experiment-yolo_amd/csrc)")
        _LIB = L
    return _LIB


def check(rc, name):
    if rc != 0:
        raise RuntimeError(f"{name} failed: {_ERR.get(rc, rc)}")
```

### experiment-yolo_amd/ultralytics/hip/engine.py

```python
from __future__ import annotations

import ctypes as C
import os

import numpy as np
import torch

from . import (DY_ACT_LEAKY, DY_ACT_NONE, DY_ACT_SILU, DY_BN_COPIES, DY_EPI_ACCUM, DY_EPI_BIAS, DY_EPI_F32OUT, DY_EPI_SILU,
               DY_EPI_STATS, DY_EPI_STATS_ACC, DySegs, check, lib)

BN2D_EPS, BN2D_MOM = 1e-3, 0.03
BN3D_EPS, BN3D_MOM = 1e-5, 0.1


def _ptr(t):
    return 0 if t is None else t.data_ptr()


POISON = os.environ.get("DY_POISON", "0") == "1"

BN_ACC = os.environ.get("DY_BN_ACC", "1") != "0"
BN_WGRAD = BN_ACC and os.environ.get("DY_BN_WGRAD", "1") != "0"
STEM_DIRECT = BN_WGRAD and os.environ.get("DY_STEM_DIRECT", "1") != "0"
BN_RES = BN_ACC and os.environ.get("DY_BN_RES", "1") != "0"
BIAS_WGRAD = BN_ACC and os.environ.get("DY_BIAS_WGRAD", "1") != "0"
SPPF_FUSED = True
PLANAR_CV1 = os.environ.get("DY_PLANAR_CV1", "1") != "0"
UPSEG = os.environ.get("DY_UPSEG", "1") != "0"
SIDE_SMALL = int(os.environ.get("DY_SIDE_SMALL", "0"))
UPSEG_TRAIN = UPSEG and os.environ.get("DY_UPSEG_TRAIN", "1") != "0"
ADD_ALIAS = os.environ.get("DY_ADD_ALIAS", "1") != "0"
SCALSEQ_ADD = os.environ.get("DY_SCALSEQ_ADD", "1") != "0"
HEAD_ROWS = BIAS_WGRAD and os.environ.get("DY_HEAD_ROWS", "1") != "0"
HEAD_DECODE = HEAD_ROWS and os.environ.get("DY_HEAD_DECODE", "1") != "0"
HEAD_CLS = BIAS_WGRAD and os.environ.get("DY_HEAD_CLS", "1") != "0"
HEAD_BATCH = os.environ.get("DY_HEAD_BATCH", "1") != "0"
BN_GROUP = BN_ACC and os.environ.get("DY_BN_GROUP", "1") != "0"
HEAD_STREAMS = os.environ.get("DY_HEAD_STREAMS", "0") != "0"
CONV_RES = os.environ.get("DY_CONV_RES", "1") != "0"
PLANAR = os.environ.get("DY_PLANAR", "1") != "0"
HEAD_APPLY = HEAD_DECODE and os.environ.get("DY_SILU_FAST", "1") != "0" and os.environ.get("DY_HEAD_APPLY", "1") != "0"
BN_DGRED = BN_WGRAD and os.environ.get("DY_BN_DGRED", "0") != "0"
WGRAD_DGRAD = BN_WGRAD and not BN_DGRED and os.environ.get("DY_WGRAD_DGRAD", "1") != "0"
FROZEN_DGRAD = BN_WGRAD and not BN_DGRED and os.environ.get("DY_FROZEN_DGRAD", "1") != "0"
BN_DGRED_MAXC = int(os.environ.get("DY_BN_DGRED_MAXC", "64"))
BN_DGRED_MAXPIX = int(os.environ.get("DY_BN_DGRED_MAXPIX", str(1 << 40)))


def round8(c):
    return (c + 7) // 8 * 8


def dev_empty(shape, dtype, device):
    t = torch.empty(shape, dtype=dtype, device=device)
    if POISON and t.numel():
        t.view(-1).view(torch.uint8).fill_(0xFF)
    return t


class Arena:

    ALIGN = 256

    def __init__(self, nbytes, device, measure=False):
        self.device, self.measure = torch.device(device), measure
        self.buf = None if measure else dev_empty(int(nbytes), torch.uint8, self.device)
        self.cap, self.off, self.peak = int(nbytes), 0, 0

    def reset(self):
        self.off = 0
        if POISON and self.buf is not None:
            self.buf.fill_(0xFF)

    def take(self, shape, dtype):
        n = int(np.prod(shape)) * torch.empty((), dtype=dtype).element_size()
        start = (self.off + self.ALIGN - 1) // self.ALIGN * self.ALIGN
        self.off = start + n
        self.peak = max(self.peak, self.off)
        if self.measure:
            return dev_empty(shape, dtype, self.device)
        if self.off > self.cap:
            raise MemoryError(f"step-local buffers need more than the shared arena's {self.cap / 2**30:.2f} GiB "
                              f"(request of {n / 2**20:.1f} MiB at offset {start / 2**30:.2f} GiB): the arena is sized on the largest input size")
        return self.buf[start:start + n].view(dtype).view(shape)


class Storage:

    def __init__(self, eng, N, H, W, C, dtype=torch.float16):
        assert C % 8 == 0, f"channel count {C} must be a multiple of 8"
        self.eng, self.N, self.H, self.W, self.C = eng, N, H, W, C
        self.buf = eng.transient((N, H, W, C), dtype)
        self.gbuf = None
        self.gwritten = []

    nograd = ()

    def grad_free(self, c0, c1):
        pos = c0
        for a, b in sorted(self.nograd):
            if a > pos:
                break
            pos = max(pos, b)
        return pos >= c1

    def act(self, c0=0, C=None):
        return Act(self, c0, self.C - c0 if C is None else C)

    @classmethod
    def grad_only(cls, eng, N, H, W, C):
        st = object.__new__(cls)
        st.eng, st.N, st.H, st.W, st.C = eng, N, H, W, C
        st.buf, st.gbuf, st.gwritten = None, None, []
        return st

    @classmethod
    def over(cls, eng, t):
        assert t.dim() == 4 and t.is_contiguous() and t.shape[3] % 8 == 0
        st = object.__new__(cls)
        st.eng, (st.N, st.H, st.W, st.C) = eng, t.shape
        st.buf, st.gbuf, st.gwritten = t, None, []
        return st


class Act:
    __slots__ = ("st", "c0", "C", "needs_grad")

    def __init__(self, st, c0, C, needs_grad=None):
        assert c0 % 8 == 0 and C >= 1 and c0 + round8(C) <= st.C, (c0, C, st.C)
        if needs_grad is None:
            needs_grad = not (st.nograd and st.grad_free(c0, c0 + C))
        self.st, self.c0, self.C, self.needs_grad = st, c0, C, needs_grad

    N = property(lambda s: s.st.N)
    H = property(lambda s: s.st.H)
    W = property(lambda s: s.st.W)
    ld = property(lambda s: s.st.C)
    Cp = property(lambda s: round8(s.C))
    npix = property(lambda s: s.st.N * s.st.H * s.st.W)

    @property
    def ptr(self):
        return self.st.buf.data_ptr() + self.c0 * self.st.buf.element_size()

    def sub(self, c0, C):
        return Act(self.st, self.c0 + c0, C, self.needs_grad)

    def _gbuf(self):
        st = self.st
        if st.gbuf is None:
            st.gbuf = (st.eng.transient(tuple(st.buf.shape), st.buf.dtype) if st.buf is not None
                       else st.eng.transient((st.N, st.H, st.W, st.C), torch.float16))
            st.eng.hold(st.gbuf)
        return st.gbuf

    @property
    def gptr(self):
        g = self._gbuf()
        return g.data_ptr() + self.c0 * g.element_size()

    def grad_ready(self):
        c0, c1 = self.c0, self.c0 + self.C
        cov = sorted(self.st.gwritten)
        pos = c0
        for a, b in cov:
            if a > pos:
                break
            pos = max(pos, b)
            if pos >= c1:
                return True
        return pos >= c1

    def grad_target(self):
        gw = self.st.eng._gw
        k = (id(self.st), self.c0, self.C)
        gw[k] = gw.get(k, 0) + 1
        c0, c1 = self.c0, self.c0 + self.C
        self._gbuf()
        overl = [(a, b) for a, b in self.st.gwritten if a < c1 and b > c0]
        if not overl:
            self.st.gwritten.append((c0, c1))
            return 0
        if self.grad_ready():
            return 1
        covered = torch.zeros(self.st.C, dtype=torch.bool)
        for a, b in self.st.gwritten:
            covered[a:b] = True
        c = c0
        while c < c1:
            if not covered[c]:
                e = c
                while e < c1 and not covered[e]:
                    e += 1
                self.st.eng.zero_grad_slice(self.st, c, e)
                c = e
            else:
# ... 611 lines not shown
        if self.tape is not None and not spec.trainable:
            self._no_grad(y)
        elif self.tape is not None:
            def bwd():
                assert y.grad_ready(), f"gradient of {spec.name} output incomplete"
                self.call("dy_bn_act_bwd_reduce_acc", y.gptr, y.ld, raw.ptr, raw.ld, spec.coef.data_ptr(), self._acc_ready(spec.acc_b), npix,
                          spec.cout, spec.act, 0, 0, 0)
                ns = self.L.dy_stem_grid(x.N, x.H, x.W)
                se = 9 * 16 * 16
                deferred = self.deferred_wgrad is not None
                slabs = self.transient((ns * se,), torch.float32) if deferred else self.scratch("slabs", ns * se * 4)
                self.hold(slabs)
                self.call("dy_stem_wgrad_bn", x.img.data_ptr(), y.gptr, y.ld, raw.ptr, raw.ld, spec.coef.data_ptr(), spec.acc_b.data_ptr(),
                          spec.gbn_w.data_ptr(), spec.gbn_b.data_ptr(), float(npix), slabs.data_ptr(), x.N, x.H, x.W, x.mul)
                if deferred:
                    self.deferred_wgrad.append((spec, slabs, ns))
                else:
                    keep, self.deferred_wgrad = self.deferred_wgrad, [(spec, slabs, ns)]
                    self.flush_wgrad()
                    self.deferred_wgrad = keep
            self.tape.append(bwd)
        return y

    def conv_bn_act_group(self, members, defer=None):
        defer = list(defer) if defer is not None else [False] * len(members)
        ok = (BN_GROUP and self.training and self.tape is not None and 1 < len(members) <= self.L.dy_bn_group_max()
              and all(sp.acc_f is not None and sp.acc_b is not None and sp.act == DY_ACT_SILU and sp.ld is None and not isinstance(x, ImageAct)
                      and self._live(sp, x) for sp, x in members))
        if not ok:
            return [self.conv_bn_act(sp, x, defer_apply=d) for (sp, x), d in zip(members, defer)]
        outs = []
        for (spec, x), d in zip(members, defer):
            assert x.C == spec.cin_phys, (spec.name, x.C, spec.cin_phys)
            Ho, Wo = self.out_hw(spec, x)
            raw = self.new_act(x.N, Ho, Wo, spec.cout)
            y = self.new_act(x.N, Ho, Wo, spec.cout)
            self._use(x)
            self._prod[(id(y.st), y.c0, y.C)] = (spec, raw)
            self._conv_raw(spec, x, raw.ptr, raw.ld, DY_EPI_STATS | DY_EPI_STATS_ACC, self._acc_ready(spec.acc_f))
            outs.append((spec, x, raw, y, bool(d)))
        P, I, Lg, F = C.c_void_p, C.c_int, C.c_long, C.c_float
        bn = [sp.bn for sp, *_ in outs]
        npx = [y.npix for _, _, _, y, _ in outs]
        self.call("dy_bn_act_apply_acc_group", len(outs), self._arr(P, [raw.ptr for _, _, raw, _, _ in outs]), self._arr(I, [raw.ld for _, _, raw, _, _ in outs]),
                  self._arr(P, [y.ptr for _, _, _, y, _ in outs]), self._arr(I, [y.ld for _, _, _, y, _ in outs]),
                  self._arr(P, [sp.acc_f.data_ptr() for sp, *_ in outs]), self._arr(P, [b["weight"].data_ptr() for b in bn]),
                  self._arr(P, [b["bias"].data_ptr() for b in bn]), self._arr(P, [b["running_mean"].data_ptr() for b in bn]),
                  self._arr(P, [b["running_var"].data_ptr() for b in bn]), self._arr(P, [sp.coef.data_ptr() for sp, *_ in outs]),
                  self._arr(Lg, [0 if d else n for n, (*_, d) in zip(npx, outs)]), self._arr(I, [sp.cout for sp, *_ in outs]),
                  self._arr(F, [float(n) for n in npx]), self._arr(F, [sp.bn_eps for sp, *_ in outs]), self._arr(F, [sp.bn_mom for sp, *_ in outs]))
        for spec, x, raw, y, d in outs:
            if d:
                self._unapplied[(id(y.st), y.c0, y.C)] = (raw, spec)

        def bwd():
            dense = []
            for spec, x, raw, y, _ in outs:
                assert y.grad_ready(), f"gradient of {spec.name} output incomplete"
                ykey = (id(y.st), y.c0, y.C)
                rows = self._rows_grad.get(ykey)
                if rows is not None and self._gw.get(ykey) == 1:
                    asg, A, a0 = rows
                    self.call("dy_bn_act_bwd_reduce_rows", y.gptr, y.ld, raw.ptr, raw.ld, spec.coef.data_ptr(), self._acc_ready(spec.acc_b),
                              y.N, y.H * y.W, spec.cout, spec.act, asg, A, a0)
                else:
                    dense.append((spec, raw, y))
            if len(dense) == 1:
                spec, raw, y = dense[0]
                self.call("dy_bn_act_bwd_reduce_acc", y.gptr, y.ld, raw.ptr, raw.ld, spec.coef.data_ptr(), self._acc_ready(spec.acc_b), y.npix,
                          spec.cout, spec.act, 0, 0, 0)
            elif dense:
                self.call("dy_bn_act_bwd_reduce_acc_group", len(dense), self._arr(P, [y.gptr for _, _, y in dense]), self._arr(I, [y.ld for _, _, y in dense]),
                          self._arr(P, [raw.ptr for _, raw, _ in dense]), self._arr(I, [raw.ld for _, raw, _ in dense]),
                          self._arr(P, [sp.coef.data_ptr() for sp, _, _ in dense]), self._arr(P, [self._acc_ready(sp.acc_b) for sp, _, _ in dense]),
                          self._arr(Lg, [y.npix for _, _, y in dense]), self._arr(I, [sp.cout for sp, _, _ in dense]))
            for spec, x, raw, y, _ in reversed(outs):
                self._conv_bn_act_bwd(spec, x, raw, y, None, reduced=True)
        self.tape.append(bwd)
        return [y for _, _, _, y, _ in outs]

    def _conv_bn_act_bwd(self, spec, x, raw, y, res, reduced=False):
        if isinstance(y, SegAct):
            y0, y1 = y.parts
            assert y0.grad_ready() and y1.grad_ready(), f"gradient of {spec.name} output incomplete"
            assert y1.gptr - y0.gptr == y0.npix * y0.ld * 2 and y0.ld == y1.ld == y0.C, "the planes' gradients are not one allocation"
            npix = y0.npix
            self.call("dy_bn_act_bwd_reduce_acc_split", y0.gptr, y0.ld, y1.gptr, y1.ld, y0.C, raw.ptr, raw.ld, spec.coef.data_ptr(),
                      self._acc_ready(spec.acc_b), npix, spec.cout, spec.act)
            if not spec.trainable and self._dgrad_only_ok(spec, x):
                self._dgrad_only(spec, x, raw, y0.gptr, y0.ld, npix, planes=(y1.gptr, y0.C))
                return
            if self._wgrad_dgrad_ok(spec, x):
                draw = None
            elif self.cur_sid:
                draw = self.transient((npix * spec.cout,), torch.float16)
                self.hold(draw)
            else:
                draw = self.scratch("draw", npix * spec.cout * 2)
            bn = (raw, draw, spec.coef.data_ptr(), spec.acc_b.data_ptr(), spec.gbn_w.data_ptr(), spec.gbn_b.data_ptr(), float(npix))
            self._conv_bwd(spec, x, y0.gptr, y0.ld, y0.H, y0.W, bn=bn, planes=(y1.gptr, y0.C))
            return
        assert y.grad_ready(), f"gradient of {spec.name} output incomplete"
        npix = y.npix
        acc = BN_ACC and spec.acc_b is not None
        fused_red = id(spec) in self._reduced
        if fused_red and self._gw.get((id(y.st), y.c0, y.C)) != 1:
            raise RuntimeError(f"{spec.name}: BatchNorm backward reduce was fused into a dgrad that is not the only writer of the gradient")
        rg = (0, 0, 0)
        if res is not None and res.needs_grad:
            racc = res.grad_target()
            if acc and BN_RES and res.C == spec.cout and not fused_red:
                rg = (res.gptr, res.ld, racc)
            elif racc:
                self.call("dy_add", res.gptr, res.ld, y.gptr, y.ld, 0, 0, res.gptr, res.ld, npix, res.C)
            else:
                self.call("dy_copy_slice", y.gptr, y.ld, res.gptr, res.ld, npix, res.C)
        ykey = (id(y.st), y.c0, y.C)
        rows = self._rows_grad.get(ykey)
        if rows is not None and self._gw.get(ykey) != 1:
            rows = None
        if acc and (fused_red or reduced):
            pass
        elif acc and rows is not None and rg == (0, 0, 0):
            asg, A, a0 = rows
            self.call("dy_bn_act_bwd_reduce_rows", y.gptr, y.ld, raw.ptr, raw.ld, spec.coef.data_ptr(), self._acc_ready(spec.acc_b),
                      y.N, y.H * y.W, spec.cout, spec.act, asg, A, a0)
        elif acc:
            self.call("dy_bn_act_bwd_reduce_acc", y.gptr, y.ld, raw.ptr, raw.ld, spec.coef.data_ptr(), self._acc_ready(spec.acc_b),
                      npix, spec.cout, spec.act, *rg)
        elif spec.cout != spec.cout_phys:
            part = self._partials(2048 * 2 * spec.cout_phys * 4 + 4096)
            n = C.c_int(0)
            self.call("dy_bn_act_bwd_reduce_c", y.gptr, y.ld, raw.ptr, raw.ld, spec.coef.data_ptr(), part.data_ptr(), 2048, npix,
                      spec.cout, spec.act, C.byref(n))
            self.call("dy_bn_bwd_finalize_ld", part.data_ptr(), n.value, spec.cout_phys, spec.gbn_w.data_ptr(), spec.gbn_b.data_ptr(),
                      spec.bwdcoef.data_ptr(), spec.cout, float(npix), 0)
        else:
            part = self._partials(2048 * 2 * spec.cout * 4 + 4096)
            n = C.c_int(0)
            self.call("dy_bn_act_bwd_reduce", y.gptr, y.ld, raw.ptr, raw.ld, spec.coef.data_ptr(), part.data_ptr(), 2048, npix,
                      spec.cout, spec.act, C.byref(n))
            self.call("dy_bn_bwd_finalize", part.data_ptr(), n.value, spec.gbn_w.data_ptr(), spec.gbn_b.data_ptr(),
                      spec.bwdcoef.data_ptr(), spec.cout, float(npix), 0)
        frozen = not spec.trainable
        if frozen:
            if not x.needs_grad:
                return
            if acc and spec.act == DY_ACT_SILU and self._dgrad_only_ok(spec, x):
                self._dgrad_only(spec, x, raw, y.gptr, y.ld, npix)
                return
        side_small = bool(not frozen and SIDE_SMALL and npix <= SIDE_SMALL and self.deferred_wgrad is not None and not self.cur_sid and not self.side_wgrad
                          and acc and isinstance(x, Act) and x.needs_grad and spec.ld is None)
        bn_wgrad = bool(not frozen and acc and BN_WGRAD and spec.act == DY_ACT_SILU and not self.side_wgrad and not side_small and raw.ld == spec.cout)
        if bn_wgrad and self._wgrad_dgrad_ok(spec, x):
            draw = None
        elif ((self.side_wgrad or side_small) and self.deferred_wgrad is not None) or self.cur_sid:
            draw = self.transient((npix * spec.cout_phys,), torch.float16)
            self.hold(draw)
        else:
            draw = self.scratch("draw", npix * spec.cout_phys * 2)
        if bn_wgrad:
            bn = (raw, draw, spec.coef.data_ptr(), spec.acc_b.data_ptr(), spec.gbn_w.data_ptr(), spec.gbn_b.data_ptr(), float(npix))
            self._conv_bwd(spec, x, y.gptr, y.ld, y.H, y.W, bn=bn)
            return
        if acc:
            self.call("dy_bn_act_bwd_apply_acc", y.gptr, y.ld, raw.ptr, raw.ld, draw.data_ptr(), spec.cout, spec.coef.data_ptr(),
                      spec.acc_b.data_ptr(), spec.gbn_w.data_ptr(), spec.gbn_b.data_ptr(), npix, spec.cout, spec.act, float(npix))
        else:
            self.call("dy_bn_act_bwd_apply_c" if spec.cout != spec.cout_phys else "dy_bn_act_bwd_apply", y.gptr, y.ld, raw.ptr, raw.ld,
                      draw.data_ptr(), spec.cout_phys, spec.coef.data_ptr(), spec.bwdcoef.data_ptr(), npix, spec.cout, spec.act, 0)
        self._conv_bwd(spec, x, draw.data_ptr(), spec.cout_phys, y.H, y.W, side_hint=side_small, wgrad=not frozen)

    def _dgrad_only_ok(self, spec, x):
        if not (FROZEN_DGRAD and BN_ACC and spec.bn is not None and spec.acc_b is not None and spec.act == DY_ACT_SILU and spec.ks == 1
                and spec.stride == 1 and spec.ld is None and isinstance(x, (Act, SegAct)) and x.needs_grad
                and spec.cout == spec.cout_phys and spec.cin == spec.cin_phys):
            return False
        return bool(self.L.dy_conv1x1_dgrad_bn_supported(x.N, x.H, x.W, spec.cin, spec.cout))

    def _dgrad_only(self, spec, x, raw, dy_ptr, lddy, npix, planes=None):
        if isinstance(x, SegAct):
            accs = [q.grad_target() if q.needs_grad else 0 for q in x.parts]
            dxs, dx = C.byref(self._segs(x, grad=True, acc=accs)), (0, 0, 0)
        else:
            acc = x.grad_target()
            dxs, dx = None, (x.gptr, x.ld, int(acc))
        self.call("dy_conv1x1_dgrad_bn", dy_ptr, planes[0] if planes else 0, lddy, planes[1] if planes else 0, raw.ptr, raw.ld,
                  spec.coef.data_ptr(), spec.acc_b.data_ptr(), float(npix), spec.wpack_t.data_ptr(), *dx, dxs, x.N, x.H, x.W, spec.cin, spec.cout)

    def _wgrad_dgrad_ok(self, spec, x):
        if not (WGRAD_DGRAD and spec.ks == 1 and spec.stride == 1 and spec.ld is None and isinstance(x, (Act, SegAct)) and x.needs_grad
                and not self.cur_sid and not self.side_wgrad and spec.cout == spec.cout_phys and spec.cin == spec.cin_phys):
            return False
        return bool(self.L.dy_conv1x1_wgrad_dgrad_supported(x.N, x.H, x.W, spec.cin, spec.cout))

    def _conv_bwd(self, spec, x, dy_ptr, lddy, Ho, Wo, accumulate_w=0, defer=True, bn=None, bias_acc=None, planes=None, side_hint=False,
                  wgrad=True):
        if not wgrad:
            assert bn is None and bias_acc is None and planes is None
            return self._input_grad(spec, x, dy_ptr, lddy, Ho, Wo)
        ns, se = C.c_int(), C.c_long()
        self.L.dy_wgrad_workspace(x.N, x.H, x.W, spec.cin, spec.cout, spec.ks, spec.stride, C.byref(ns), C.byref(se))
        deferred = defer and not accumulate_w and self.deferred_wgrad is not None
        if self.wgrad_log is not None and not deferred:
            self.wgrad_log.append(spec)
        if deferred:
            slabs = self.transient((ns.value * se.value,), torch.float32)
            self.hold(slabs)
            self.deferred_wgrad.append((spec, slabs, ns.value) if bias_acc is None else (spec, slabs, ns.value, bias_acc))
            dw = 0
        else:
            slabs = self.scratch("slabs", ns.value * se.value * 4)
            dw = spec.gweight.data_ptr()
        side = deferred and (self.side_wgrad or side_hint)
        if side:
            self._side_used = True
            self.fork()
        if bn is not None and bn[1] is None:
            raw, _, coef, accb, gw, gb, cnt = bn
            assert not side and self._wgrad_dgrad_ok(spec, x)
            seg = isinstance(x, SegAct)
            if seg:
                accs = [q.grad_target() if q.needs_grad else 0 for q in x.parts]
                dxs, dx = C.byref(self._segs(x, grad=True, acc=accs)), (0, 0, 0)
            else:
                acc = x.grad_target()
                dxs, dx = None, (x.gptr, x.ld, int(acc))
            tail = (x.N, x.H, x.W, spec.cin, spec.cout, accumulate_w)
            wt = spec.wpack_t.data_ptr()
            if planes is not None:
                self.call("dy_conv1x1_wgrad_dgrad_bn_planes", C.byref(self._segs(x)) if seg else None, 0 if seg else x.ptr, 0 if seg else x.ld,
                          dy_ptr, planes[0], lddy, planes[1], raw.ptr, raw.ld, coef, accb, gw, gb, cnt, slabs.data_ptr(), dw, wt, *dx, dxs, *tail)
            elif seg:
                self.call("dy_conv1x1_wgrad_dgrad_bn_segs", C.byref(self._segs(x)), dy_ptr, lddy, raw.ptr, raw.ld, coef, accb, gw, gb, cnt,
                          slabs.data_ptr(), dw, wt, dxs, *tail)
            else:
                self.call("dy_conv1x1_wgrad_dgrad_bn", x.ptr, x.ld, dy_ptr, lddy, raw.ptr, raw.ld, coef, accb, gw, gb, cnt, slabs.data_ptr(), dw,
                          wt, *dx, *tail)
            return
        if planes is not None:
            raw, draw, coef, accb, gw, gb, cnt = bn
            seg = isinstance(x, SegAct)
            self.call("dy_conv1x1_wgrad_bn_planes", C.byref(self._segs(x)) if seg else None, 0 if seg else x.ptr, 0 if seg else x.ld, dy_ptr,
                      planes[0], lddy, planes[1], raw.ptr, raw.ld, draw.data_ptr() if x.needs_grad else 0, coef, accb, gw, gb, cnt,
                      slabs.data_ptr(), dw, x.N, x.H, x.W, spec.cin, spec.cout, accumulate_w)
            dy_ptr, lddy = draw.data_ptr(), spec.cout
        elif bn is not None and isinstance(x, SegAct):
            raw, draw, coef, accb, gw, gb, cnt = bn
            self.call("dy_conv1x1_wgrad_bn_segs", C.byref(self._segs(x)), dy_ptr, lddy, raw.ptr, raw.ld, draw.data_ptr() if x.needs_grad else 0,
                      coef, accb, gw, gb, cnt, slabs.data_ptr(), dw, x.N, x.H, x.W, spec.cin, spec.cout, accumulate_w)
            dy_ptr, lddy = draw.data_ptr(), spec.cout
        elif bn is not None:
            raw, draw, coef, accb, gw, gb, cnt = bn
            head = (x.ptr, x.ld, dy_ptr, lddy, raw.ptr, raw.ld, draw.data_ptr() if x.needs_grad else 0, coef, accb, gw, gb, cnt,
                    slabs.data_ptr(), dw, x.N, x.H, x.W)
            if spec.ld is not None:
                n, cphys, cin = spec.ld
                self.call("dy_conv_wgrad_ld_bn", *head, spec.cout, cin, n, cphys, accumulate_w)
            else:
                self.call("dy_conv_wgrad_bn", *head, spec.cin, spec.cout, spec.ks, spec.stride, accumulate_w)
            dy_ptr, lddy = draw.data_ptr(), spec.cout
        elif bias_acc is not None:
            assert deferred
            self.call("dy_conv_wgrad_bias", x.ptr, x.ld, dy_ptr, lddy, self._acc_ready(bias_acc), slabs.data_ptr(), dw, x.N, x.H, x.W,
                      spec.cin, spec.cout, spec.ks, spec.stride, accumulate_w)
        elif spec.ld is not None:
            n, cphys, cin = spec.ld
            self.call("dy_conv_wgrad_ld", x.ptr, x.ld, dy_ptr, lddy, slabs.data_ptr(), dw, x.N, x.H, x.W,
                      spec.cout, cin, n, cphys, accumulate_w, side=side)
        else:
            self.call("dy_conv_wgrad", x.ptr, x.ld, dy_ptr, lddy, slabs.data_ptr(), dw, x.N, x.H, x.W,
                      spec.cin, spec.cout, spec.ks, spec.stride, accumulate_w, side=side)
        if isinstance(x, SegAct):
            assert bn is not None, f"{spec.name}: a segmented input needs the BatchNorm-in-the-weight-gradient path"
        self._input_grad(spec, x, dy_ptr, lddy, Ho, Wo)

    wgrad_log = None

    def _input_grad(self, spec, x, dy_ptr, lddy, Ho, Wo):
        if isinstance(x, SegAct):
            if x.needs_grad:
                accs = [q.grad_target() if q.needs_grad else 0 for q in x.parts]
                self.call("dy_conv1x1_input_grad_segs", dy_ptr, lddy, spec.wpack_t.data_ptr(), C.byref(self._segs(x, grad=True, acc=accs)),
                          x.N, Ho, Wo, spec.cout_phys, spec.cin)
            return
        if x.needs_grad:
            acc = x.grad_target()
            prod = self._sole_consumer_of_conv(x) if (BN_DGRED and not acc and spec.stride == 1 and spec.ld is None) else None
            if prod is not None:
                ps, praw = prod
                if not (ps.act == DY_ACT_SILU and ps.acc_b is not None and ps.cout == x.C == spec.cin and x.C <= BN_DGRED_MAXC and x.npix <= BN_DGRED_MAXPIX
                        and (praw.N, praw.H, praw.W) == (x.N, x.H, x.W)
                        and self.L.dy_conv_red_supported(spec.cout_phys, spec.cin, spec.ks)):
                    prod = None
            if prod is not None:
                self.call("dy_conv_input_grad_red", dy_ptr, lddy, spec.wpack_t.data_ptr(), x.gptr, x.ld, x.N, Ho, Wo, spec.cout_phys, spec.cin,
                          spec.ks, praw.ptr, praw.ld, ps.coef.data_ptr(), self._acc_ready(ps.acc_b), ps.cout)
                self._reduced.add(id(ps))
            else:
                cin = spec.cin_phys if x.C != x.Cp else spec.cin
                self.call("dy_conv_forward", dy_ptr, lddy, spec.wpack_t.data_ptr(), 0, x.gptr, x.ld, 0, x.N, Ho, Wo,
                          spec.cout_phys, cin, spec.ks, 1, spec.stride, x.H, x.W, DY_EPI_ACCUM if acc else 0, None)

    deferred_wgrad = None
    tape_mark = None

    def flush_wgrad(self):
        items, self.deferred_wgrad = self.deferred_wgrad, None
        if self.side_wgrad or self._side_used:
            self.join()
            self._side_used = False
        if not items:
            return
        if self.wgrad_log is not None:
            self.wgrad_log.extend(it[0] for it in items)
        sz = self.L.dy_wgrad_reduce_desc_bytes()
        host = (C.c_char * (sz * len(items)))()
        blocks = 0
        for i, (spec, slabs, ns, *bias) in enumerate(items):
            ld = spec.ld or (0, 0, 0)
            nb = self.L.dy_wgrad_reduce_desc_fill(C.byref(host, i * sz), slabs.data_ptr(), ns, spec.gweight.data_ptr(), spec.cin, spec.cout,
                                                  spec.ks, spec.stride, 0, ld[0], ld[1], ld[2], blocks)
            if nb < 0:
                raise RuntimeError(f"dy_wgrad_reduce_desc_fill failed for {spec.name}")
            if bias:
                check(self.L.dy_wgrad_reduce_desc_bias(C.byref(host, i * sz), bias[0].data_ptr(), spec.gbias.data_ptr(), (spec.cout + 7) // 8 * 8),
                      "dy_wgrad_reduce_desc_bias")
            blocks += nb
        dev = torch.frombuffer(bytearray(host), dtype=torch.uint8).to(self.device)
        self.keep.append(dev)
        self.call("dy_wgrad_reduce_batched", dev.data_ptr(), len(items), blocks)

    def conv_fused(self, spec: ConvSpec, x: Act, out: Act | None = None, res: Act | None = None):
        if isinstance(x, ImageAct):
            if STEM_DIRECT and self._stem_eval_ok(spec, res) and spec.bias is not None:
                Ho, Wo = (x.H - 1) // 2 + 1, (x.W - 1) // 2 + 1
                y = out if out is not None else self.new_act(x.N, Ho, Wo, spec.cout)
                self.call("dy_stem_forward_eval", x.img.data_ptr(), spec.weight.data_ptr(), spec.bias.data_ptr(), y.ptr, y.ld, x.N, x.H, x.W,
                          x.mul, 1 if spec.act == DY_ACT_SILU else 0)
                return y
            x = x.materialize()
        if isinstance(x, UpAct) or (isinstance(x, SegAct) and not self.seg_conv_ok(spec, x)):
            x = self.dense(x)
        Ho, Wo = self.out_hw(spec, x)
        y = out if out is not None else self.new_act(x.N, Ho, Wo, spec.cout)
        epi = DY_EPI_BIAS | (DY_EPI_SILU if spec.act == DY_ACT_SILU else 0)
        if spec.cout != spec.cout_phys:
            if isinstance(x, SegAct):
                x = self.dense(x)
            if res is not None:
                raise NotImplementedError(f"{spec.name}: a residual operand of width {spec.cout} (not a multiple of 8)")
            if getattr(spec, "bias_pad", None) is None:
                spec.bias_pad = self.f32(spec.cout_phys, 0.0)
            self.call("dy_pad_f32", spec.bias.data_ptr(), spec.cout, spec.bias_pad.data_ptr(), spec.cout_phys)
            self._conv_raw(spec, x, y.ptr, y.ld, epi, 0, spec.bias_pad, cout=spec.cout_phys)
            return y
        if (res is not None and CONV_RES and spec.act == DY_ACT_SILU and spec.ld is None
                and self.L.dy_conv_res_supported(x.C, spec.cout, spec.ks, spec.stride)):
            self.call("dy_conv_forward_res", x.ptr, x.ld, spec.wpack.data_ptr(), spec.bias.data_ptr(), res.ptr, res.ld, y.ptr, y.ld,
                      x.N, x.H, x.W, x.C, spec.cout, spec.ks, spec.stride)
            return y
        self._conv_raw(spec, x, y.ptr, y.ld, epi, 0, spec.bias)
        if res is not None:
            self.call("dy_add", y.ptr, y.ld, res.ptr, res.ld, 0, 0, y.ptr, y.ld, y.npix, y.C)
        return y

    def conv_bias(self, spec: ConvSpec, x: Act, y_ptr, ldy, f32out=True, dy_ptr_fn=None, out_hw=None, rows_level=None):
        x = self.dense(x)
        live = self._live(spec, x)
        if live:
            self._use(x)
        self._conv_raw(spec, x, y_ptr, ldy, DY_EPI_BIAS | (DY_EPI_F32OUT if f32out else 0), 0, spec.bias)
        if self.tape is not None and live:
            if (rows_level is not None and self.rows_used is not None and spec.ks == 1 and spec.ld is None and spec.acc_bias is not None
                    and self.L.dy_conv1x1_rows_supported(spec.cin, spec.cout)):
                self.rows_used.add(rows_level)
            else:
                rows_level = None
            self.tape.append(lambda: self._conv_bias_bwd(spec, x, dy_ptr_fn, rows_level=rows_level))

    def rows_capable(self, spec):
        return (self.rows_used is not None and self.tape is not None and spec.ks == 1 and spec.ld is None and spec.acc_bias is not None
                and spec.bias is not None and bool(self.L.dy_conv1x1_rows_supported(spec.cin, spec.cout)))
# ... 504 lines not shown
```

### experiment-yolo_amd/ultralytics/hip/train.py

```python
from __future__ import annotations

import ctypes as C
import math
import os
import sys

import numpy as np
import torch
import torch.distributed as dist

from . import check, lib
from .dist import all_reduce_flat
from .engine import Recorder


class StepPlan:
    def __init__(self, model, batch_size, imgsz, nmax=16, optimizer="SGD", hyp=None, world_size=1, use_graph=False,
                 init_scale=65536.0, side_wgrad=None, dynamic_scale=True, share=None, arena=None, input_act=False):
        self.model = model
        self.arena = arena
        self.side_wgrad = bool(int(os.environ.get("DY_SIDE_WGRAD", "0"))) if side_wgrad is None else bool(side_wgrad)
        dev = next(model.parameters()).device
        self.rt = model._runtime(dev)
        self.eng = self.rt.eng
# ... 489 lines not shown
    def _soap_apply_pending(self):
        saved, self._soap_pending = getattr(self, "_soap_pending", None), None
        if not saved:
            return
        from .soap import _State
        dev = self.rt.flat_p.device
        mv = lambda t: None if t is None else t.to(dev)
        for i, (n, o, k, sh, _g) in enumerate(self._soap_views):
            if n in saved:
                d = saved[n]
                st = self._soap.state.get(i) or _State(self.rt.flat_p[o:o + k].view(sh))
                st.step, st.m, st.v, st.gg = d["step"], mv(d["m"]), mv(d["v"]), [mv(t) for t in d["gg"]]
                st.q = None if d["q"] is None else [mv(t) for t in d["q"]]
                self._soap.state[i] = st

    def optimizer_step(self):
        rt, eng = self.rt, self.eng
        grads = self.gsum if self._micro else rt.flat_g
        if self.soap:
            self._soap_step(grads)
        key = grads.data_ptr()
        if key not in self.rec_opt:
            eng.rec = Recorder()
            try:
                b = (C.c_long * 5)(*rt.seg_bounds)
                eng.call("dy_optimizer_step_seg", rt.flat_p.data_ptr(), grads.data_ptr(), self.mom.data_ptr(),
                         0 if self.adam_v is None else self.adam_v.data_ptr(), self.ema.data_ptr(), rt.n_params_flat, b,
                         rt.frozen.data_ptr(), rt.flat_b.data_ptr(), self.ema_b.data_ptr(), rt.n_buffers_flat,
                         self.hyper.data_ptr(), self.state.data_ptr(), self.partials.data_ptr(), self.mode)
            finally:
                self.rec_opt[key], eng.rec = eng.rec, None
            if self.use_graph:
                torch.cuda.synchronize()
                g = torch.cuda.CUDAGraph()
                with torch.cuda.graph(g, capture_error_mode="thread_local"):
                    eng.replay(self.rec_opt[key])
                self.graph_opt[key] = g
        elif key in self.graph_opt:
            self.graph_opt[key].replay()
        else:
            eng.replay(self.rec_opt[key])
        self.ema_updates += 1
        self.opt_calls += 1
        self._micro = 0
        rt.mark_dirty()

    def check_progress(self):
        st = self.state.cpu().tolist()
        scale, taken, skipped = st[0], int(st[5]), int(st[6])
        if taken + skipped != self.opt_calls:
            raise RuntimeError(f"optimizer step counter out of step with the host: {self.opt_calls} optimizer_step() calls, device took "
                               f"{taken} and skipped {skipped} -- the recorded optimizer launches are not executing")
        if not self.dynamic_scale and skipped:
            raise RuntimeError(f"{skipped} of {self.opt_calls} optimizer steps were skipped for non-finite gradients at the fixed loss "
                               f"scale {scale:g} (amp=False): the gradients are corrupt or overflow fp16 -- nothing was learned from them")
        if self.dynamic_scale and (scale < 1.0 or (self.opt_calls >= 32 and taken == 0)):
            raise RuntimeError(f"dynamic loss scale collapsed to {scale:g} ({skipped} of {self.opt_calls} optimizer steps skipped): "
                               "gradients stay non-finite however small the scale")
        self.crit.check_capacity()
        return taken, skipped, scale

    def step(self, batch, lr, momentum, wd):
        self.set_hyper(lr, momentum, wd)
        self.forward_backward(batch)
        self.all_reduce()
        self.optimizer_step()

    def loss_items(self):
        s = self.crit.scalars.cpu()
        self.crit.check_capacity(s)
        return float(s[8]), s[5:8].clone()

    def profile_ops(self, reps=3):
        ops = [o for o in self.rec_fb.ops if o[0] is not None]
        s = self.eng.stream
        evs = [torch.cuda.Event(enable_timing=True) for _ in range(len(ops) + 1)]
        tot = [0.0] * len(ops)
        for _ in range(reps):
            torch.cuda._sleep(60_000_000)
            evs[0].record()
            for i, (fn, args, name, _side) in enumerate(ops):
                rc = fn(*args, s)
                if rc != 0:
                    check(rc, name)
                evs[i + 1].record()
            torch.cuda.synchronize()
            for i in range(len(ops)):
                tot[i] += evs[i].elapsed_time(evs[i + 1])
        cal = [torch.cuda.Event(enable_timing=True) for _ in range(33)]
        torch.cuda._sleep(20_000_000)
        for e in cal:
            e.record()
        torch.cuda.synchronize()
        gaps = sorted(cal[i].elapsed_time(cal[i + 1]) for i in range(32))
        self.event_gap_ms = gaps[len(gaps) // 2]
        return [(ops[i][2], ops[i][1], max(tot[i] / reps - self.event_gap_ms, 0.0)) for i in range(len(ops))]

    @staticmethod
    def conv_algorithmic_bytes(args):
        (_x, _ldx, _w, _b, _y, _ldy, _p, n, h, w, cin, cout, ks, stride, dil, oh, ow, epi, _np) = args
        H, W = (2 * h, 2 * w) if dil == 2 else (h, w)
        pad = ks // 2
        Ho, Wo = ((H + 2 * pad - ks) // stride + 1, (W + 2 * pad - ks) // stride + 1) if not oh else (oh, ow)
        ob = 4 if epi & 8 else 2
        out = n * Ho * Wo * cout * ob
        return n * h * w * cin * 2 + out * (2 if epi & 16 else 1)

    @staticmethod
    def wgrad_algorithmic_bytes(args):
        (_x, _ldx, _dy, _lddy, _sl, _dw, n, h, w, cin, cout, ks, stride, _acc) = args[:14]
        pad = ks // 2
        Ho, Wo = (h + 2 * pad - ks) // stride + 1, (w + 2 * pad - ks) // stride + 1
        return n * h * w * ((cin + 7) // 8 * 8) * 2 + n * Ho * Wo * ((cout + 7) // 8 * 8) * 2

    def kernel_of(self, name, args):
        key, alg = self._kernel_alg(name, args)
        own = alg
        e = 2
        if name == "dy_bn_act_apply":
            own = int(args[7]) * int(args[8]) * e * (3 if args[2] else 2)
        elif name == "dy_bn_act_apply_acc":
            own = int(args[12]) * int(args[13]) * e * (3 if args[2] else 2)
        elif name == "dy_bn_act_bwd_reduce":
            own = int(args[7]) * int(args[8]) * e * 2
        elif name == "dy_bn_act_bwd_reduce_acc":
            own = int(args[6]) * int(args[7]) * e * (2 + ((2 if args[11] else 1) if args[9] else 0))
        elif name == "dy_bn_act_bwd_apply":
            own = int(args[8]) * int(args[9]) * e * 3
        elif name == "dy_bn_act_bwd_apply_acc":
            own = int(args[10]) * int(args[11]) * e * 3
        elif name in ("dy_conv_wgrad_bn", "dy_conv_wgrad_ld_bn"):
            n, h, w = args[14:17]
            if name == "dy_conv_wgrad_bn":
                cin, cout, ks, stride = args[17:21]
            else:
                cout, ks, stride = args[17], 1, 1
            pad = ks // 2
            own = alg + 2 * n * ((h + 2 * pad - ks) // stride + 1) * ((w + 2 * pad - ks) // stride + 1) * ((cout + 7) // 8 * 8) * e
        elif name == "dy_stem_wgrad_bn":
            n, h, w = args[11:14]
            own = alg + n * ((h - 1) // 2 + 1) * ((w - 1) // 2 + 1) * 16 * e
        elif name in ("dy_conv1x1_wgrad_bn_segs", "dy_conv1x1_wgrad_bn_planes") and alg:
            n, h, w, _cin, cout = args[13:18] if name.endswith("segs") else args[17:22]
            own = alg + 2 * n * h * w * ((cout + 7) // 8 * 8) * e
        elif name in self._FUSED_BWD and alg:
            n, h, w, cin, cout, old = self._fused_bwd_shape(name, args)
            own = n * h * w * (2 * cin + 2 * cout + old) * e
        elif name == "dy_bn_act_apply_acc_split":
            own = int(args[13]) * int(args[14]) * e * 2
        elif name == "dy_bn_act_bwd_reduce_acc_split":
            own = int(args[9]) * int(args[10]) * e * 2
        return key, alg, own

    _FUSED_BWD = {"dy_conv1x1_wgrad_dgrad_bn": 17, "dy_conv1x1_wgrad_dgrad_bn_segs": 14, "dy_conv1x1_wgrad_dgrad_bn_planes": 21}

    def _fused_bwd_shape(self, name, args):
        i = self._FUSED_BWD[name]
        n, h, w, cin, cout = args[i:i + 5]
        dxs = args[13] if name.endswith("segs") else (args[20] if name.endswith("planes") else None)
        if dxs is not None:
            t = dxs._obj
            old = sum((t.c_end[k] - (t.c_end[k - 1] if k else 0)) for k in range(t.nseg) if t.acc[k])
        else:
            old = cin if args[16 if name.endswith("bn") else 19] else 0
        return n, h, w, cin, cout, old

    def _kernel_alg(self, name, args):
        import ctypes as C
        L, buf = self.eng.L, C.create_string_buffer(128)
        if name in self._FUSED_BWD:
            n, h, w, cin, cout, old = self._fused_bwd_shape(name, args)
            seg = name.endswith("segs") or (name.endswith("planes") and args[0] is not None)
            if L.dy_wgrad_dgrad_kernel_name(n, h, w, cin, cout, int(seg), buf, 128) == 0:
                return buf.value.decode(), n * h * w * (2 * (cin + cout) + (0 if seg else old)) * 2
        if name == "dy_conv1x1_dgrad_bn":
            n, h, w, cin, cout = args[14:19]
            if L.dy_dgrad_only_kernel_name(n, h, w, cin, cout, int(args[13] is not None), buf, 128) == 0:
                return buf.value.decode(), n * h * w * (cin + cout) * 2
        if name == "dy_conv_forward":
            n, h, w, cin, cout, ks, stride, dil = args[7:15]
            if dil == 2 and ks == 3:
                return f"conv_mfma_dg2_kernel (input gradient of the {cout}->{cin} stride-2 3x3)", self.conv_algorithmic_bytes(args)
            pad = ks // 2
            if ks == 1 and L.dy_conv1x1_kernel_name_live(cin, cout, n, h, w, int(args[17]), None, None, buf, 128) == 0:
                return buf.value.decode(), self.conv_algorithmic_bytes(args)
            if L.dy_conv_kernel_name_at(cin, cout, ks, stride, (w + 2 * pad - ks) // stride + 1, dil, int(args[17]), buf, 128) == 0:
                return buf.value.decode(), self.conv_algorithmic_bytes(args)
        if name == "dy_conv1x1_forward_segs":
            n, h, w, cin, cout = args[6:11]
            if L.dy_conv1x1_kernel_name_live(cin, cout, n, h, w, int(args[11]), args[0], None, buf, 128) == 0:
                return buf.value.decode(), n * h * w * (cin + (cout + 7) // 8 * 8) * 2
        if name == "dy_conv1x1_input_grad_segs":
            n, h, w, cin, cout = args[4:9]
            if L.dy_conv1x1_kernel_name_live(cin, cout, n, h, w, 0, None, args[3], buf, 128) == 0:
                return buf.value.decode(), n * h * w * (cin + cout) * 2
        if name in ("dy_conv1x1_wgrad_bn_segs", "dy_conv1x1_wgrad_bn_planes"):
            n, h, w, cin, cout = args[13:18] if name.endswith("segs") else args[17:22]
            if L.dy_wgrad_kernel_name_at(n, h, w, cin, cout, 1, 1, buf, 128) == 0:
                seg = args[0] is not None
                return buf.value.decode().replace(", 0>", ", 3>" if seg else ", 1>"), n * h * w * (cin + (cout + 7) // 8 * 8) * 2
        if name == "dy_conv_wgrad":
            n, h, w, cin, cout, ks, stride = args[6:13]
            if L.dy_wgrad_kernel_name_at(n, h, w, cin, cout, ks, stride, buf, 128) == 0:
                return buf.value.decode(), self.wgrad_algorithmic_bytes(args)
        if name == "dy_conv_input_grad_red":
            n, h, w, cin, cout, ks = args[5:11]
            if L.dy_conv_kernel_name(cin, cout, ks, 1, buf, 128) == 0:
                return buf.value.decode().replace("false, 0>", "true, 0>"), n * h * w * (cin + cout) * 2
        if name == "dy_stem_forward":
            n, h, w = args[5:8]
            return "stem_fwd_kernel", n * h * w * 3 * 2 + n * ((h - 1) // 2 + 1) * ((w - 1) // 2 + 1) * 16 * 2
        if name == "dy_stem_wgrad_bn":
            n, h, w = args[11:14]
            return "stem_wgrad_bn_kernel", n * h * w * 3 * 2 + n * ((h - 1) // 2 + 1) * ((w - 1) // 2 + 1) * 16 * 2
        if name in ("dy_conv_wgrad_bn", "dy_conv_wgrad_ld_bn"):
            n, h, w = args[14:17]
            if name == "dy_conv_wgrad_bn":
                cin, cout, ks, stride = args[17:21]
            else:
                cout, _ld_cin, ld_taps, ld_cphys = args[17:21]
                cin, ks, stride = ld_taps * ld_cphys, 1, 1
            if L.dy_wgrad_kernel_name_at(n, h, w, cin, cout, ks, stride, buf, 128) == 0:
                pad = ks // 2
                Ho, Wo = (h + 2 * pad - ks) // stride + 1, (w + 2 * pad - ks) // stride + 1
                return (buf.value.decode().replace(", 0>", ", 1>"),
                        n * h * w * ((cin + 7) // 8 * 8) * 2 + n * Ho * Wo * ((cout + 7) // 8 * 8) * 2)
        if name == "dy_conv_wgrad_ld":
            n, h, w, cout, ld_cin, ld_taps, ld_cphys = args[6:13]
            if L.dy_wgrad_kernel_name_at(n, h, w, ld_taps * ld_cphys, cout, 1, 1, buf, 128) == 0:
                return buf.value.decode(), n * h * w * (ld_taps * ld_cphys + (cout + 7) // 8 * 8) * 2
        tmpl = {"dy_bn_act_apply": ("bn_act_apply_kernel<{}, false, false>", 9), "dy_bn_act_apply_acc": ("bn_act_apply_kernel<{}, true, " + ("false" if os.environ.get("DY_SILU_FAST") == "0" else "true") + ">", 14),
                "dy_bn_act_bwd_reduce": ("bn_act_bwd_reduce_kernel<{}, false>", 9),
                "dy_bn_act_bwd_apply": ("bn_act_bwd_apply_kernel<{}, false>", 10),
                "dy_bn_act_bwd_apply_acc": ("bn_act_bwd_apply_kernel<{}, true>", 12)}
        if name == "dy_bn_act_bwd_reduce_acc":
            return f"bn_act_bwd_reduce_kernel<{int(args[8])}, {'true' if args[9] else 'false'}>", 0
        if name == "dy_bn_act_bwd_reduce_acc_split":
            return f"bn_act_bwd_reduce_kernel<{int(args[11])}, false>", 0
        if name == "dy_bn_act_apply_acc_split":
            return f"bn_act_apply_kernel<{int(args[15])}, true, true>", 0
        if name in tmpl:
            k, i = tmpl[name]
            return k.format(int(args[i])), 0
        return name.replace("dy_", "", 1) + " (C-ABI call)", 0

    def probe_dominant_kernel(self, batch, reps=10):
        if self.rec_fb is None:
            self.forward_backward(batch)
        prof = self.profile_ops(reps)
        self.last_profile = prof
        groups = {}
        for name, args, ms in prof:
            key, by, own = self.kernel_of(name, args)
            groups.setdefault(key, []).append((ms, by, own))

        def summary(key):
            items = groups[key]
            ms = sum(t[0] for t in items) / len(items)
            by = sum(t[2] for t in items) / len(items)
            return {"kernel": key, "us": ms * 1e3, "bytes": by, "gbs": by / (ms * 1e-3) / 1e9 if ms > 0 else 0.0,
                    "algorithmic_bytes": sum(t[1] for t in items) / len(items),
                    "launches_per_step": len(items), "ms_per_step": sum(t[0] for t in items)}

        if not groups:
            return None
        rank = sorted(groups, key=lambda k: -sum(t[0] for t in groups[k]))
        top = summary(rank[0])
        convs = [k for k in rank if k.startswith("conv_")]
        top["top_conv"] = summary(convs[0]) if convs else None
        algs = [k for k in rank if sum(t[1] for t in groups[k]) > 0]
        if algs:
            ta = summary(algs[0])
            ta["alg_gbs"] = ta["algorithmic_bytes"] / (ta["us"] * 1e-6) / 1e9 if ta["us"] > 0 else 0.0
            top["top_alg"] = ta
        else:
            top["top_alg"] = None
        top["ranking"] = [{"kernel": k, "ms_per_step": round(sum(t[0] for t in groups[k]), 4), "launches": len(groups[k]),
                           "algorithmic_MB_per_step": round(sum(t[1] for t in groups[k]) / 1e6, 1),
                           "own_MB_per_step": round(sum(t[2] for t in groups[k]) / 1e6, 1)} for k in rank[:12]]
        top["step_device_ms"] = sum(t[2] for t in prof)
        top["step_algorithmic_bytes"] = sum(t[1] for v in groups.values() for t in v)
        return top

    def breakdown(self):
        agg = {}
        for name, _a, ms in getattr(self, "last_profile", []):
            k = agg.setdefault(name, [0, 0.0])
            k[0] += 1
            k[1] += ms
        return {k: {"calls": v[0], "ms": round(v[1], 3)} for k, v in sorted(agg.items(), key=lambda kv: -kv[1][1])}
```

### include/dealyolo_hip.h

```cpp
#ifndef DEALYOLO_HIP_H
#define DEALYOLO_HIP_H

#include <stddef.h>
#include <stdint.h>

#ifdef __cplusplus
extern "C" {
#endif

#ifndef __HIP__
typedef struct ihipStream_t* hipStream_t;
#endif

#define DY_OK 0
#define DY_ERR_ARG (-1)
#define DY_ERR_LAUNCH (-2)
#define DY_ERR_ALIGN (-3)
#define DY_ERR_CAPACITY (-4)

#define DY_MAX_SEGS 8
typedef struct DySegs {
  int nseg;
  int c_end[DY_MAX_SEGS];
  int ld[DY_MAX_SEGS];
  int acc[DY_MAX_SEGS];
  const void* ptr[DY_MAX_SEGS];
} DySegs;
int dy_segs_bytes(void);

#define DY_EPI_STATS 1
#define DY_EPI_BIAS 2
#define DY_EPI_SILU 4
#define DY_EPI_F32OUT 8
#define DY_EPI_ACCUM 16
#define DY_EPI_STATS_ACC 32
#define DY_BN_COPIES 16

#define DY_ACT_NONE 0
#define DY_ACT_SILU 1
#define DY_ACT_LEAKY 2

int dy_abi_version(void);

int dy_conv_geometry(int cin, int cout, int ks, int stride, int* cin_p, int* cout_p, int* cc, int* nch, int* mt,
                     int* ngroups, int* ksteps, int* packed_elems);
int dy_pack_weights(const float* w, const float* scale, void* out, int cout, int cin, int ks, int stride,
                    int transposed, hipStream_t stream);
int dy_pack_desc_bytes(void);
int dy_pack_desc_fill(void* desc, const float* w, const float* scale, void* out, int cout, int cin, int ks, int stride,
                      int transposed, int ld_taps, int ld_cphys, int first_block);
int dy_pack_weights_batched(const void* descs_device, int n, int total_blocks, hipStream_t stream);
int dy_conv_forward(const void* x, int ldx, const void* w_packed, const float* bias, void* y, int ldy, float* partials,
                    int n, int h, int w, int cin, int cout, int ks, int stride, int dil, int out_h, int out_w, int epi,
                    int* num_partials, hipStream_t stream);
int dy_conv_num_partials(int n, int h, int w, int cin, int cout, int ks, int stride, int dil);
int dy_conv_res_supported(int cin, int cout, int ks, int stride);
int dy_conv_forward_res(const void* x, int ldx, const void* w_packed, const float* bias, const void* res, int ldres, void* y, int ldy,
                        int n, int h, int w, int cin, int cout, int ks, int stride, hipStream_t stream);
int dy_conv_red_supported(int cin, int cout, int ks);
int dy_conv_input_grad_red(const void* dy, int lddy, const void* w_packed_t, void* dx, int lddx, int n, int h, int w, int cin, int cout,
                           int ks, const void* raw, int ldraw, const float* coef, double* acc, int C, hipStream_t stream);
int dy_conv_kernel_name(int cin, int cout, int ks, int stride, char* out, int cap);
int dy_conv_kernel_name_at(int cin, int cout, int ks, int stride, int out_w, int dil, int epi, char* out, int cap);

int dy_wgrad_workspace(int n, int h, int w, int cin, int cout, int ks, int stride, int* nslabs, long* slab_elems);
int dy_wgrad_kernel_name(int cin, int cout, int ks, int stride, char* out, int cap);
int dy_wgrad_kernel_name_at(int n, int h, int w, int cin, int cout, int ks, int stride, char* out, int cap);
int dy_conv_wgrad(const void* x, int ldx, const void* dy, int lddy, float* slabs, float* dw, int n, int h, int w,
                  int cin, int cout, int ks, int stride, int accumulate, hipStream_t stream);
int dy_conv_wgrad_bn(const void* x, int ldx, const void* dy, int lddy, const void* raw, int ldraw, void* draw, const float* coef,
                     const double* acc, float* dgamma, float* dbeta, float count, float* slabs, float* dw, int n, int h, int w,
                     int cin, int cout, int ks, int stride, int accumulate, hipStream_t stream);
int dy_conv_wgrad_ld_bn(const void* x, int ldx, const void* dy, int lddy, const void* raw, int ldraw, void* draw,
                        const float* coef, const double* acc, float* dgamma, float* dbeta, float count, float* slabs, float* dw,
                        int n, int h, int w, int cout, int ld_cin, int ld_taps, int ld_cphys, int accumulate, hipStream_t stream);
int dy_conv1x1_segs_supported(int cin, int cout, const DySegs* xs);
int dy_conv1x1_segs_kernel_name(int cin, int cout, const DySegs* xs, char* out, int cap);
int dy_conv1x1_kernel_name_live(int cin, int cout, int n, int h, int w, int epi, const DySegs* xs, const DySegs* ys, char* out, int cap);
int dy_conv1x1_forward_segs(const DySegs* xs, const void* w_packed, const float* bias, void* y, int ldy, float* partials, int n, int h,
                            int w, int cin, int cout, int epi, hipStream_t stream);
int dy_conv1x1_input_grad_segs(const void* dy, int lddy, const void* w_packed_t, const DySegs* dxs, int n, int h, int w, int cin, int cout,
                               hipStream_t stream);
int dy_conv1x1_wgrad_bn_segs(const DySegs* xs, const void* dy, int lddy, const void* raw, int ldraw, void* draw, const float* coef,
                             const double* acc, float* dgamma, float* dbeta, float count, float* slabs, float* dw, int n, int h, int w,
                             int cin, int cout, int accumulate, hipStream_t stream);
int dy_bn_act_apply_acc_split(const void* x, int ldx, void* y, int ldy, void* y2, int ldy2, int csplit, const double* acc,
                              const float* gamma, const float* beta, float* running_mean, float* running_var, float* coef, long npix,
                              int C, int act, float count, float eps, float momentum, hipStream_t stream);
int dy_bn_act_bwd_reduce_acc_split(const void* dy, int lddy, const void* dy2, int lddy2, int csplit, const void* x, int ldx,
                                   const float* coef, double* acc, long npix, int C, int act, hipStream_t stream);
int dy_conv1x1_wgrad_bn_planes(const DySegs* xs, const void* x, int ldx, const void* dy, const void* dy2, int lddy, int csplit,
                               const void* raw, int ldraw, void* draw, const float* coef, const double* acc, float* dgamma,
                               float* dbeta, float count, float* slabs, float* dw, int n, int h, int w, int cin, int cout,
                               int accumulate, hipStream_t stream);
int dy_conv1x1_wgrad_dgrad_supported(int n, int h, int w, int cin, int cout);
int dy_wgrad_dgrad_kernel_name(int n, int h, int w, int cin, int cout, int segs, char* out, int cap);
int dy_conv1x1_wgrad_dgrad_bn(const void* x, int ldx, const void* dy, int lddy, const void* raw, int ldraw, const float* coef,
                              const double* acc, float* dgamma, float* dbeta, float count, float* slabs, float* dw,
                              const void* w_packed_t, void* dx, int lddx, int dx_accumulate, int n, int h, int w, int cin, int cout,
                              int accumulate, hipStream_t stream);
int dy_conv1x1_wgrad_dgrad_bn_segs(const DySegs* xs, const void* dy, int lddy, const void* raw, int ldraw, const float* coef,
                                   const double* acc, float* dgamma, float* dbeta, float count, float* slabs, float* dw,
                                   const void* w_packed_t, const DySegs* dxs, int n, int h, int w, int cin, int cout, int accumulate,
                                   hipStream_t stream);
int dy_conv1x1_wgrad_dgrad_bn_planes(const DySegs* xs, const void* x, int ldx, const void* dy, const void* dy2, int lddy, int csplit,
                                     const void* raw, int ldraw, const float* coef, const double* acc, float* dgamma, float* dbeta,
                                     float count, float* slabs, float* dw, const void* w_packed_t, void* dx, int lddx,
                                     int dx_accumulate, const DySegs* dxs, int n, int h, int w, int cin, int cout, int accumulate,
                                     hipStream_t stream);
int dy_conv1x1_dgrad_bn_supported(int n, int h, int w, int cin, int cout);
int dy_dgrad_only_kernel_name(int n, int h, int w, int cin, int cout, int segs, char* out, int cap);
int dy_conv1x1_dgrad_bn(const void* dy, const void* dy2, int lddy, int csplit, const void* raw, int ldraw, const float* coef,
                        const double* acc, float count, const void* w_packed_t, void* dx, int lddx, int dx_accumulate,
                        const DySegs* dxs, int n, int h, int w, int cin, int cout, hipStream_t stream);
int dy_stem_grid(int n, int h, int w);
int dy_stem_forward(const float* img_nchw, const float* weight, void* raw, int ldraw, double* acc, int n, int h, int w, float mul,
                    hipStream_t stream);
int dy_stem_forward_eval(const float* img_nchw, const float* weight, const float* bias, void* y, int ldy, int n, int h, int w, float mul,
                         int silu, hipStream_t stream);
int dy_stem_wgrad_bn(const float* img_nchw, const void* dy, int lddy, const void* raw, int ldraw, const float* coef,
                     const double* acc, float* dgamma, float* dbeta, float count, float* slabs, int n, int h, int w, float mul,
                     hipStream_t stream);
int dy_conv_wgrad_bias(const void* x, int ldx, const void* dy, int lddy, double* bias_acc, float* slabs, float* dw, int n, int h, int w,
                       int cin, int cout, int ks, int stride, int accumulate, hipStream_t stream);
int dy_wgrad_reduce_desc_bias(void* desc, const double* bias_acc, float* dbias, int c);
int dy_wgrad_reduce_desc_bytes(void);
int dy_wgrad_reduce_desc_fill(void* desc, const float* slabs, int nslabs, float* dw, int cin, int cout, int ks, int stride,
                              int accumulate, int ld_taps, int ld_cphys, int ld_cin, int first_block);
int dy_wgrad_reduce_batched(const void* descs_device, int n, int total_blocks, hipStream_t stream);

int dy_ldconv_sample(const void* x, int ldx, const float* off, int ldoff, const int* pn, void* xo, int ldxo, int n, int H,
                     int W, int h, int w, int C, int Np, int stride, hipStream_t stream);
int dy_ldconv_sample_backward(const void* x, int ldx, const float* off, int ldoff, const int* pn, const void* dxo,
                              int lddxo, float* dx32, void* doff, int lddoff, int n, int H, int W, int h, int w, int C,
                              int Np, int stride, hipStream_t stream);
int dy_ldconv_sample_backward_gather(const void* x, int ldx, const float* off, int ldoff, const int* pn, const void* dxo,
                                     int lddxo, void* dx, int lddx, int accumulate, float* dx32, void* doff, int lddoff,
                                     void* scratch, int rmax, int n, int H, int W, int h, int w, int C, int Np, int stride,
                                     hipStream_t stream);
int dy_f32_to_f16_add(const float* src, void* dst, int ld, long npix, int C, int accumulate, hipStream_t stream);
int dy_pack_weights_ld(const float* w, void* out, int cout, int cin, int ld_taps, int ld_cphys, int transposed,
                       hipStream_t stream);
int dy_conv_wgrad_ld(const void* x, int ldx, const void* dy, int lddy, float* slabs, float* dw, int n, int h, int w,
                     int cout, int ld_cin, int ld_taps, int ld_cphys, int accumulate, hipStream_t stream);

int dy_bn_finalize(const float* p0, int n0, float w0, const float* p1, int n1, float w1, const float* p2, int n2,
                   float w2, const float* gamma, const float* beta, float* running_mean, float* running_var,
                   float* coef, int C, float count, float eps, float momentum, int update_running, hipStream_t stream);
int dy_bn_eval_coef(const float* gamma, const float* beta, const float* running_mean, const float* running_var,
                    float* coef, int C, float eps, hipStream_t stream);
int dy_bn_act_apply(const void* x, int ldx, const void* res, int ldr, void* y, int ldy, const float* coef, long npix,
                    int C, int act, hipStream_t stream);
int dy_bn_act_apply_acc(const void* x, int ldx, const void* res, int ldr, void* y, int ldy, const double* acc,
                        const float* gamma, const float* beta, float* running_mean, float* running_var, float* coef,
                        long npix, int C, int act, float count, float eps, float momentum, hipStream_t stream);
int dy_bn_act_bwd_reduce_acc(const void* dy, int lddy, const void* x, int ldx, const float* coef, double* acc, long npix,
                             int C, int act, void* res_grad, int ldrg, int res_accumulate, hipStream_t stream);
int dy_bn_group_max(void);
int dy_bn_act_apply_acc_group(int n, const void* const* x, const int* ldx, void* const* y, const int* ldy, const double* const* acc,
                              const float* const* gamma, const float* const* beta, float* const* running_mean, float* const* running_var,
                              float* const* coef, const long* npix, const int* C, const float* count, const float* eps,
                              const float* momentum, hipStream_t stream);
int dy_bn_act_bwd_reduce_acc_group(int n, const void* const* dy, const int* lddy, const void* const* x, const int* ldx,
                                   const float* const* coef, double* const* acc, const long* npix, const int* C, hipStream_t stream);
int dy_bn_act_bwd_reduce_rows(const void* dy, int lddy, const void* x, int ldx, const float* coef, double* acc, int n, int hw, int C,
                              int act, const int* assigned, int A, int a0, hipStream_t stream);
int dy_bn_act_bwd_apply_acc(const void* dy, int lddy, const void* x, int ldx, void* dx, int lddx, const float* coef,
                            const double* acc, float* dgamma, float* dbeta, long npix, int C, int act, float count,
                            hipStream_t stream);
int dy_bn_act_bwd_reduce(const void* dy, int lddy, const void* x, int ldx, const float* coef, float* partials,
                         int max_partials, long npix, int C, int act, int* nparts, hipStream_t stream);
int dy_bn_bwd_finalize(const float* partials, int nparts, float* dgamma, float* dbeta, float* bwdcoef, int C,
                       float count, int accumulate, hipStream_t stream);
int dy_bn_act_bwd_apply(const void* dy, int lddy, const void* x, int ldx, void* dx, int lddx, const float* coef,
                        const float* bwdcoef, long npix, int C, int act, int frozen_stats, hipStream_t stream);

int dy_bn_finalize_ld(const float* part, int nparts, int ldp, const float* gamma, const float* beta, float* running_mean,
                      float* running_var, float* coef, int C, float count, float eps, float momentum, int update_running,
                      long long* num_batches_tracked, hipStream_t stream);
int dy_bn_act_apply_c(const void* x, int ldx, const void* res, int ldr, void* y, int ldy, const float* coef, long npix, int C,
                      int act, hipStream_t stream);
int dy_bn_act_bwd_reduce_c(const void* dy, int lddy, const void* x, int ldx, const float* coef, float* partials, int max_partials,
                           long npix, int C, int act, int* nparts, hipStream_t stream);
int dy_bn_bwd_finalize_ld(const float* partials, int nparts, int ldp, float* dgamma, float* dbeta, float* bwdcoef, int C,
                          float count, int accumulate, hipStream_t stream);
int dy_bn_act_bwd_apply_c(const void* dy, int lddy, const void* x, int ldx, void* dx, int lddx, const float* coef,
                          const float* bwdcoef, long npix, int C, int act, int frozen_stats, hipStream_t stream);
int dy_pad_f32(const float* src, int n, float* dst, int n_pad, hipStream_t stream);

int dy_import_image(const float* x_nchw, void* y, int n, int c, int h, int w, int cp, float mul, hipStream_t stream);
int dy_import_image_u8(const void* x, void* y, int n, int h, int w, int cp, const void* flip, const int* index,
                       const float* hsv, hipStream_t stream);
int dy_warp_import_u8(const void* pool, const void* slots, void* y, int n, int s, int cp, hipStream_t stream);
int dy_warp_slot_bytes(void);
int dy_add(const void* a, int lda, const void* b, int ldb, const void* c, int ldc, void* y, int ldy, long npix, int C,
           hipStream_t stream);
int dy_upsample2x(const void* x, int ldx, void* y, int ldy, int n, int h, int w, int C, int backward, int accumulate,
                  hipStream_t stream);
int dy_space_to_depth(void* x, int ldx, void* y, int ldy, int n, int h, int w, int C, int backward, int accumulate,
                      hipStream_t stream);
int dy_dysample_supported(int C, int G, int s);
int dy_dysample(const void* x, int ldx, const float* off, int ldoff, void* y, int ldy, int n, int H, int W, int C, int G, int s,
                hipStream_t stream);
int dy_dysample_backward(const void* x, int ldx, const float* off, int ldoff, const void* dy, int lddy, void* dx, int lddx,
                         int accumulate, float* dx32, void* doff, int lddoff, void* scratch, int rmax, int n, int H, int W, int C,
                         int G, int s, hipStream_t stream);
int dy_maxpool5(const void* x, int ldx, void* y, int ldy, void* argmax, int n, int h, int w, int C, hipStream_t stream);
int dy_maxpool5_backward(const void* dy, int lddy, const void* argmax, void* dx, int lddx, int n, int h, int w, int C,
                         int accumulate, hipStream_t stream);
int dy_sppf_pool3_supported(int h, int w, int C);
int dy_sppf_pool3(void* cat, int ld, int C, void* arg0, void* arg1, void* arg2, int n, int h, int w, hipStream_t stream);
int dy_sppf_pool3_backward(void* gcat, int ld, int C, const void* arg0, const void* arg1, const void* arg2, int n, int h, int w,
                           int acc0, int acc1, int acc2, hipStream_t stream);
int dy_scalseq_tail(const void* r0, int ld0, const void* r1, int ld1, const void* r2, int ld2, const void* res,
                    int ldres, void* y, int ldy, const float* coef, int n, int h, int w, int C, hipStream_t stream);
int dy_scalseq_tail_backward(const void* r0, int ld0, const void* r1, int ld1, const void* r2, int ld2, const void* dy,
                             int lddy, void* dr, int lddr, const float* coef, const float* bwdcoef, float* partials,
                             int max_partials, int n, int h, int w, int C, int level, int mode, int* nparts,
                             hipStream_t stream);
int dy_scalseq_tail_backward_all(const void* r0, int ld0, const void* r1, int ld1, const void* r2, int ld2,
                                 const void* dy, int lddy, void* dr0, int lddr0, void* dr1, int lddr1, void* dr2,
                                 int lddr2, const float* coef, const float* bwdcoef, float* partials, int max_partials,
                                 int n, int h, int w, int C, int mode, int* nparts, hipStream_t stream);
int dy_scalseq_bwd_grid_cap(int cap);
int dy_zoom_pool(const void* x, int ldx, void* y, int ldy, int n, int h, int w, int C, hipStream_t stream);
int dy_zoom_pool_backward(const void* x, int ldx, const void* dy, int lddy, void* dx, int lddx, int n, int h, int w, int C,
                          int accumulate, hipStream_t stream);
int dy_copy_slice(const void* x, int ldx, void* y, int ldy, long npix, int C, hipStream_t stream);
int dy_fill_zero(void* p, size_t bytes, hipStream_t stream);

typedef struct DyLossArgs {
  int nl, B, nc, ncp, nmax;
  const float* box[4];
  const float* cls[4];
  void* dbox[4];
  void* dcls[4];
  int H[4], W[4];
  float stride[4];
  const float* t_batch_idx;
  const float* t_cls;
  const float* t_boxes;
  int n_targets;
  const int* n_targets_dev;
  float img_w, img_h;
  float hyp_box, hyp_cls, hyp_dfl;
  int use_wiou, use_nwd;
  float iou_ratio;
  const float* gscale;
  float* scalars;
  void* workspace;
  int dbox_rows_only;
  int box_from_input;
  const void* box_in[4];
  int box_in_ld[4];
  const float* box_w[4];
  const float* box_b[4];
  const float* box_in_coef[4];
  int box_family;
  int box_ltype;
  int box_fm;
  int box_modifier;
  float inner_ratio;
// ... 130 lines not shown
```

Measured before the change: 6121 images/s.

## Fuse input-gradient computation into 3x3 stride-1 BatchNorm weight-gradient kernel

Extends the fused wgrad+dgrad kernel to 3x3 stride-1 conv layers with 16 or 32 output channels. The dy tile is loaded with a one-pixel halo into LDS, and the input gradient is computed there with MFMA, using weights streamed through a small register ring. This removes a separate dgrad launch and a second read of dy/raw for those layers. The cost is higher register pressure and LDS use, which a resource-check script guards against, plus aliasing checks on the host side before the fused path is selected.

```diff
diff --git a/experiment-yolo_amd/csrc/check_resources.py b/experiment-yolo_amd/csrc/check_resources.py
--- /dev/null
+++ b/experiment-yolo_amd/csrc/check_resources.py
@@ -0,0 +1,23 @@
+#!/usr/bin/env python3
+import re
+import sys
+
+txt = open(sys.argv[1]).read()
+bad, seen = [], 0
+for blk in re.split(r"remark: Function Name: ", txt)[1:]:
+    name = blk.split()[0]
+    if not re.match(r"_Z17conv_wgrad_kernelILi\d+ELi\d+ELi\d+ELi\d+ELi(5|7|13|15)EE", name):
+        continue
+    seen += 1
+    scratch = int(re.search(r"ScratchSize \[bytes/lane\]: (\d+)", blk).group(1))
+    spill = int(re.search(r"VGPRs Spill: (\d+)", blk).group(1))
+    if scratch or spill:
+        bad.append(f"{name}: {scratch} bytes of scratch per lane, {spill} VGPRs spilled")
+for line in txt.splitlines():
+    if "remark:" not in line and re.search(r"\b(warning|error):", line):
+        print(line, file=sys.stderr)
+if not seen:
+    sys.exit("check_resources: no fused conv_wgrad_kernel in the resource log")
+if bad:
+    sys.exit("check_resources: register budget exceeded\n  " + "\n  ".join(bad))
+print(f"check_resources: {seen} fused conv_wgrad_kernel instantiations, no scratch, no VGPR spills")
diff --git a/experiment-yolo_amd/csrc/conv_wgrad.hip b/experiment-yolo_amd/csrc/conv_wgrad.hip
--- a/experiment-yolo_amd/csrc/conv_wgrad.hip
+++ b/experiment-yolo_amd/csrc/conv_wgrad.hip
@@ -58,7 +58,9 @@
   static_assert(!NOX || DG, "the form without X exists for the fused input gradient only");
   constexpr bool BN1 = ((BNF & 3) == 1 || (BNF & 3) == 3);
   constexpr bool XSEG = ((BNF & 3) == 3);
-  static_assert(!DG || (KS == 1 && BN1), "the fused input gradient exists for the 1x1 BatchNorm forms");
+  constexpr bool DG3 = DG && KS == 3;
+  static_assert(!DG || (BN1 && (KS == 1 || (STRIDE == 1 && !XSEG && !NOX && MTC <= 2))),
+                "the fused input gradient exists for the 1x1 BatchNorm forms and for plain 3x3 stride-1 layers of 16 / 32 output channels");
   constexpr int TAPS = KS * KS;
   constexpr int NCOL = NCI * TAPS;
   constexpr int CPW = (NCOL + 3) / 4;
@@ -69,14 +71,15 @@
   constexpr int CIN_C = 16 * NCI, COUT_C = 16 * MTC;
   constexpr int PSX = (STRIDE == 2) ? CIN_C * 2 + 16 : (((CIN_C / 2 + 7) / 16) * 16 + 8) * 4;
   constexpr int PSY = (((COUT_C / 2 + 7) / 16) * 16 + 8) * 4;
-  constexpr int XBYTES = NOX ? 0 : HHX * HWX * PSX, YBYTES = TH * TW * PSY;
+  constexpr int YH = DG3 ? TH + 2 : TH, YW = DG3 ? TW + 2 : TW, YO = DG3 ? 1 : 0;
+  constexpr int XBYTES = NOX ? 0 : HHX * HWX * PSX, YBYTES = YH * YW * PSY;
   __shared__ __attribute__((aligned(16))) char smem[XBYTES + YBYTES];
   char* const sx = smem;
   char* const sy = smem + XBYTES;
   __shared__ __attribute__((aligned(16))) float sbn[BN1 ? 4 * COUT_C : (BNF == 2 ? 256 * 8 : 4)];
   float bsum[8] = {0.f, 0.f, 0.f, 0.f, 0.f, 0.f, 0.f, 0.f};
   (void)bsum;
-  constexpr int DKS = MTC == 4 ? 2 : (MTC == 3 ? 3 : 1), DCPK = (MTC & 1) ? 16 : 32;
+  constexpr int DKS = KS == 3 ? (9 * COUT_C + 31) / 32 : (MTC == 4 ? 2 : (MTC == 3 ? 3 : 1)), DCPK = (MTC & 1) ? 16 : 32;
   constexpr int DNT = TH / 2;
   constexpr int DNC = 4 * NCI;
   constexpr int DXROW = CIN_C * 2 + 16;
@@ -99,27 +102,34 @@
   }
   (void)acc;
 
-  constexpr int NGX = HHX * HWX * (CIN_C / 8), NGY = TH * TW * (COUT_C / 8);
+  constexpr int NGX = HHX * HWX * (CIN_C / 8), NGY = YH * YW * (COUT_C / 8);
   constexpr int NPX = NOX ? 1 : (NGX + 255) / 256, NPY = (NGY + 255) / 256;
   uint4 pfx[NPX], pfy[NPY];
   uint4 pfr[BN1 ? NPY : 1];
-  unsigned roff[BN1 ? NPY : 1];
+  unsigned roff[BN1 && !DG3 ? NPY : 1];
   int ncur = 0, nnext = 0;
   (void)ncur; (void)nnext;
   unsigned vnext = 0, vcur = 0, ornext = 0, orcur = 0;
   (void)pfr; (void)roff; (void)vnext; (void)vcur; (void)ornext; (void)orcur;
   constexpr unsigned NEVER = 0x80000000u;
   constexpr int CPGX = CIN_C / 8, CPGY = COUT_C / 8;
-  unsigned xoff[NPX], yoff[NPY];
-  (void)pfx; (void)xoff;
+  unsigned xoff[DG3 ? 1 : NPX], yoff[DG3 ? 1 : NPY];
+  (void)pfx; (void)xoff; (void)yoff;
 #pragma unroll
   for (int i = 0; i < NPX; ++i) {
     const int id = tid + i * 256;
     const int pixel = id / CPGX, part = id - pixel * CPGX;
     const bool ok = !NOX && id < NGX && ci0 + part * 8 < a.cin_r8;
     const int hy = FLAT ? 0 : pixel / HWX, hx = FLAT ? pixel : pixel - hy * HWX;
-    xoff[i] = ok ? (unsigned)(((hy * a.W + hx) * a.ldx + ci0 + part * 8) * 2) : NEVER;
-  }
+    if (!DG3) xoff[DG3 ? 0 : i] = ok ? (unsigned)(((hy * a.W + hx) * a.ldx + ci0 + part * 8) * 2) : NEVER;
+  }
+  auto off3 = [&](int which, int t, int i) {
+    const int id = t + i * 256, cpg = which == 0 ? CPGX : CPGY, wpix = which == 0 ? HWX : YW;
+    const int pixel = id / cpg, part = id - pixel * cpg, hy = pixel / wpix, hx = pixel - hy * wpix;
+    const bool ok = which == 0 ? (id < NGX && ci0 + part * 8 < a.cin_r8) : (id < NGY && co0 + part * 8 < a.cout_r8);
+    const int ld = which == 0 ? a.ldx : (which == 1 ? a.lddy : a.ldraw), wd = which == 0 ? a.W : a.Wo, c0 = which == 0 ? ci0 : co0;
+    return ok ? (unsigned)(((hy * wd + hx) * ld + c0 + part * 8) * 2) : NEVER;
+  };
   constexpr bool XIN = XSEG && !NOX;
   const char* xb[XIN ? NPX : 1];
   int xl[XIN ? NPX : 1];
@@ -147,13 +157,13 @@
     const int id = tid + i * 256;
     const int pixel = id / CPGY, part = id - pixel * CPGY;
     const bool ok = id < NGY && co0 + part * 8 < a.cout_r8;
-    const int ty = FLAT ? 0 : pixel / TW, tx = FLAT ? pixel : pixel - ty * TW;
-    yoff[i] = ok ? (unsigned)(((ty * a.Wo + tx) * a.lddy + co0 + part * 8) * 2) : NEVER;
+    const int ty = FLAT ? 0 : pixel / YW, tx = FLAT ? pixel : pixel - ty * YW;
+    if (!DG3) yoff[DG3 ? 0 : i] = ok ? (unsigned)(((ty * a.Wo + tx) * a.lddy + co0 + part * 8) * 2) : NEVER;
     if (FLAT && BN1 && a.dy_csplit && ok) {
       const int ch = co0 + part * 8;
       yoff[i] = (unsigned)((tx * a.lddy + (ch < a.dy_csplit ? ch : ch - a.dy_csplit)) * 2) + (ch < a.dy_csplit ? 0u : a.dy_plane);
     }
-    if (BN1) roff[i] = ok ? (unsigned)(((ty * a.Wo + tx) * a.ldraw + co0 + part * 8) * 2) : NEVER;
+    if (BN1 && !DG3) roff[DG3 ? 0 : i] = ok ? (unsigned)(((ty * a.Wo + tx) * a.ldraw + co0 + part * 8) * 2) : NEVER;
   }
   if (BN1) {
     for (int c = tid; c < COUT_C; c += 256) {
@@ -184,17 +194,32 @@
     }
     __syncthreads();
   }
-  half8 wf[DG ? DKS : 1][DG ? NCI : 1];
-  unsigned dboff[DG ? DKS : 1];
+  half8 wf[DG && !DG3 ? DKS : 1][DG && !DG3 ? NCI : 1];
+  unsigned dboff[DG && !DG3 ? DKS : 1];
+  unsigned woff[DG3 ? NCI : 1];
   char* dxb = nullptr;
   unsigned dxld2 = 0;
   bool dxacc = false, dxadd = false;
   const int dpix = lane / DPPR, dpiece = lane - dpix * DPPR;
-  (void)wf; (void)dboff; (void)dxb; (void)dxld2; (void)dxacc; (void)dxadd; (void)dpix; (void)dpiece;
+  (void)wf; (void)woff; (void)dboff; (void)dxb; (void)dxld2; (void)dxacc; (void)dxadd; (void)dpix; (void)dpiece;
+  auto dboff3 = [&](int k) {
+    auto tapoff = [](int tap) { return ((tap > 8 ? 8 : tap) / 3 * YW + (tap > 8 ? 8 : tap) % 3) * PSY; };
+    if (COUT_C == 32) return tapoff(k);
+    return (q & 2) ? tapoff(2 * k + 1) : tapoff(2 * k);
+  };
+  if (DG3) {
+#pragma unroll
+    for (int j = 0; j < NCI; ++j) {
+      const int ch = ci0 + (p >> 2) * DNC + 4 * j + (p & 3);
+      const int gw = 16 * a.dg_mt, g = ch / gw, rem = ch - g * gw;
+      const int row = g * gw + ((rem % (4 * a.dg_mt)) >> 2) * 16 + (rem / (4 * a.dg_mt)) * 4 + (rem & 3);
+      woff[DG3 ? j : 0] = (unsigned)((g * DKS * gw + (row - g * gw)) * 64 + q * 16);
+    }
+  }
   if (DG) {
 #pragma unroll
-    for (int k = 0; k < DKS; ++k) {
-      dboff[DG ? k : 0] = (unsigned)((k * DCPK + ((q * 8) & (DCPK - 1))) * 2);
+    for (int k = 0; k < (DG3 ? 0 : DKS); ++k) {
+      dboff[DG && !DG3 ? k : 0] = (unsigned)((k * DCPK + ((q * 8) & (DCPK - 1))) * 2);
 #pragma unroll
       for (int j = 0; j < NCI; ++j) {
         const int ch = ci0 + (p >> 2) * DNC + 4 * j + (p & 3);
@@ -205,7 +230,7 @@
 #pragma unroll
         for (int e = 0; e < 8; ++e) v[e] = (f16)0.f;
         if (row < a.dg_rows) v = *reinterpret_cast<const half8*>(a.wt + ((size_t)grow * 32 + q * 8));
-        wf[DG ? k : 0][DG ? j : 0] = v;
+        wf[DG && !DG3 ? k : 0][DG && !DG3 ? j : 0] = v;
       }
     }
     const int chn = ci0 + dpiece * 8;
@@ -230,12 +255,11 @@
     }
   }
   union DU4 { uint4 u; half2_ h[4]; };
-  DU4 dold[DG ? DNT : 1][DG ? DNPASS : 1];
-  (void)dold;
   auto ld16 = [](__amdgpu_buffer_rsrc_t r, unsigned off) {
     const auto v = __builtin_amdgcn_raw_buffer_load_b128(r, (int)off, 0, 0);
     return *reinterpret_cast<const uint4*>(&v);
   };
+  constexpr int RING = DG3 ? (DKS < 8 / NCI ? DKS : 8 / NCI) : 1;
   auto prefetch = [&](int tile) {
     if (FLAT) {
       const auto rx = __builtin_amdgcn_make_buffer_rsrc(const_cast<f16*>(a.x), 0, (int)((unsigned)a.npix * (unsigned)a.ldx * 2u), 0x00020000);
@@ -268,10 +292,10 @@
         }
       } else {
 #pragma unroll
-        for (int i = 0; i < NPX; ++i) pfx[i] = ld16(rx, xoff[i] + ox);
-      }
-#pragma unroll
-      for (int i = 0; i < NPY; ++i) pfy[i] = ld16(ry, yoff[i] + oy);
+        for (int i = 0; i < NPX; ++i) pfx[i] = ld16(rx, xoff[DG3 ? 0 : i] + ox);
+      }
+#pragma unroll
+      for (int i = 0; i < NPY; ++i) pfy[i] = ld16(ry, yoff[DG3 ? 0 : i] + oy);
       if (BN1) {
         const unsigned nbytes = (unsigned)a.npix * (unsigned)a.ldraw * 2u;
         const auto rr = __builtin_amdgcn_make_buffer_rsrc(const_cast<f16*>(a.raw), 0, (int)nbytes, 0x00020000);
@@ -279,9 +303,9 @@
         vnext = 0;
 #pragma unroll
         for (int i = 0; i < NPY; ++i) {
-          const unsigned off = roff[i] + ornext;
+          const unsigned off = roff[DG3 ? 0 : i] + ornext;
           pfr[i] = ld16(rr, off);
-          vnext |= (roff[i] != NEVER && off < nbytes) ? (1u << i) : 0u;
+          vnext |= (roff[DG3 ? 0 : i] != NEVER && off < nbytes) ? (1u << i) : 0u;
         }
       }
     } else {
@@ -292,39 +316,46 @@
       const int iy0 = oy0 * STRIDE - PAD, ix0 = ox0 * STRIDE - PAD;
       const auto rx = __builtin_amdgcn_make_buffer_rsrc(const_cast<f16*>(a.x) + (size_t)n * a.H * a.W * a.ldx, 0, a.H * a.W * a.ldx * 2, 0x00020000);
       const auto ry = __builtin_amdgcn_make_buffer_rsrc(const_cast<f16*>(a.dy) + (size_t)n * a.Ho * a.Wo * a.lddy, 0, a.Ho * a.Wo * a.lddy * 2, 0x00020000);
-      const unsigned ox = (unsigned)((iy0 * a.W + ix0) * a.ldx * 2), oy = (unsigned)((oy0 * a.Wo + ox0) * a.lddy * 2);
+      const int yy0 = oy0 - YO, yx0 = ox0 - YO;
+      const unsigned ox = (unsigned)((iy0 * a.W + ix0) * a.ldx * 2), oy = (unsigned)((yy0 * a.Wo + yx0) * a.lddy * 2);
+      const bool yfull = yx0 >= 0 && yx0 + YW <= a.Wo;
+      int tv = tid;
+      if (DG3) asm volatile("" : "+v"(tv));
+      auto xo = [&](int i) { return DG3 ? off3(0, tv, i) : xoff[DG3 ? 0 : i]; };
+      auto yo = [&](int i) { return DG3 ? off3(1, tv, i) : yoff[DG3 ? 0 : i]; };
+      auto ro = [&](int i) { return DG3 ? off3(2, tv, i) : roff[DG3 ? 0 : i]; };
+      (void)ro;
       if (ix0 >= 0 && ix0 + HWX <= a.W) {
 #pragma unroll
-        for (int i = 0; i < NPX; ++i) pfx[i] = ld16(rx, xoff[i] + ox);
+        for (int i = 0; i < NPX; ++i) pfx[i] = ld16(rx, xo(i) + ox);
       } else {
 #pragma unroll
         for (int i = 0; i < NPX; ++i) {
-          const int hx = ((tid + i * 256) / CPGX) % HWX;
-          pfx[i] = ld16(rx, (unsigned)(ix0 + hx) < (unsigned)a.W ? xoff[i] + ox : NEVER);
-        }
-      }
-      if (ox0 + TW <= a.Wo) {
-#pragma unroll
-        for (int i = 0; i < NPY; ++i) pfy[i] = ld16(ry, yoff[i] + oy);
+          const int hx = ((tv + i * 256) / CPGX) % HWX;
+          pfx[i] = ld16(rx, (unsigned)(ix0 + hx) < (unsigned)a.W ? xo(i) + ox : NEVER);
+        }
+      }
+      if (yfull) {
+#pragma unroll
+        for (int i = 0; i < NPY; ++i) pfy[i] = ld16(ry, (DG3 && yo(i) == NEVER) ? NEVER : yo(i) + oy);
       } else {
 #pragma unroll
         for (int i = 0; i < NPY; ++i) {
-          const int tx = ((tid + i * 256) / CPGY) % TW;
-          pfy[i] = ld16(ry, ox0 + tx < a.Wo ? yoff[i] + oy : NEVER);
+          const int tx = ((tv + i * 256) / CPGY) % YW;
+          pfy[i] = ld16(ry, ((unsigned)(yx0 + tx) < (unsigned)a.Wo && !(DG3 && yo(i) == NEVER)) ? yo(i) + oy : NEVER);
         }
       }
       if (BN1) {
         const unsigned nbytes = (unsigned)(a.Ho * a.Wo * a.ldraw * 2);
         const auto rr = __builtin_amdgcn_make_buffer_rsrc(const_cast<f16*>(a.raw) + (size_t)n * a.Ho * a.Wo * a.ldraw, 0, (int)nbytes, 0x00020000);
-        ornext = (unsigned)((oy0 * a.Wo + ox0) * a.ldraw * 2);
+        ornext = (unsigned)((yy0 * a.Wo + yx0) * a.ldraw * 2);
         vnext = 0;
-        const bool xfull = ox0 + TW <= a.Wo;
 #pragma unroll
         for (int i = 0; i < NPY; ++i) {
-          unsigned off = roff[i] == NEVER ? NEVER : roff[i] + ornext;
-          if (!xfull) {
-            const int tx = ((tid + i * 256) / CPGY) % TW;
-            off = ox0 + tx < a.Wo ? off : NEVER;
+          unsigned off = ro(i) == NEVER ? NEVER : ro(i) + ornext;
+          if (!yfull) {
+            const int tx = ((tv + i * 256) / CPGY) % YW;
+            off = (unsigned)(yx0 + tx) < (unsigned)a.Wo ? off : NEVER;
           }
           pfr[i] = ld16(rr, off);
           vnext |= off < nbytes ? (1u << i) : 0u;
@@ -337,6 +368,17 @@
 
   int tile = (!FLAT && !(gridDim.x & 7)) ? (int)(blockIdx.x & 7) * (int)(gridDim.x >> 3) + (int)(blockIdx.x >> 3) : (int)blockIdx.x;
   if (tile < a.ntiles) prefetch(tile);
+  half8 wa[RING][DG3 ? NCI : 1];
+  (void)wa;
+  auto lda = [&](int slot, int k) {
+    const auto rw = __builtin_amdgcn_make_buffer_rsrc(const_cast<f16*>(a.wt), 0, a.dg_rows * DKS * 64, 0x00020000);
+    const int kstride = 16 * a.dg_mt * 64;
+#pragma unroll
+    for (int j = 0; j < (DG3 ? NCI : 0); ++j) {
+      const auto v = __builtin_amdgcn_raw_buffer_load_b128(rw, (int)woff[DG3 ? j : 0], k * kstride, 0);
+      wa[slot][DG3 ? j : 0] = *reinterpret_cast<const half8*>(&v);
+    }
+  };
   for (; tile < a.ntiles; tile += gridDim.x) {
     __syncthreads();
 #pragma unroll
@@ -359,7 +401,7 @@
                                          cf + COUT_C, cf + 2 * COUT_C, cf + 3 * COUT_C);
         if (!valid) o.u = make_uint4(0, 0, 0, 0);
         if (id < NGY) *reinterpret_cast<uint4*>(sy + (id / (COUT_C / 8)) * PSY + (id % (COUT_C / 8)) * 16) = o.u;
-        if (!DG && ci_chunk == 0 && a.draw) __builtin_amdgcn_raw_buffer_store_b128(o.v, rd, (int)(valid ? roff[i] + orcur : NEVER), 0, 0);
+        if (!DG && ci_chunk == 0 && a.draw) __builtin_amdgcn_raw_buffer_store_b128(o.v, rd, (int)(valid ? roff[DG3 ? 0 : i] + orcur : NEVER), 0, 0);
       }
     } else {
 #pragma unroll
@@ -373,29 +415,138 @@
         }
       }
     }
+    if (DG3) {
+#pragma unroll
+      for (int k = 0; k < RING; ++k) lda(k, k);
+    }
     __syncthreads();
     const long dpix0 = (long)tile * (TH * TW) + wave * (16 * DNT);
     (void)dpix0;
+    const int t2_ = FLAT ? 0 : tile / a.tiles_x, tn_ = FLAT ? 0 : t2_ / a.tiles_y;
+    const int toy0 = FLAT ? 0 : (t2_ - tn_ * a.tiles_y) * TH + wave * (TH / 4), tox0 = FLAT ? 0 : (tile - t2_ * a.tiles_x) * TW;
+    auto dxpix = [&](int t, int rowi, long& gp) {
+      if (DG3) {
+        const int row = toy0 + (t >> 1), col = tox0 + (t & 1) * 16 + rowi;
+        gp = ((long)tn_ * a.Ho + row) * a.Wo + col;
+        return row < a.Ho && col < a.Wo;
+      }
+      gp = dpix0 + t * 16 + rowi;
+      return gp < a.npix;
+    };
+    DU4 dold[DG ? DNT : 1][DG ? DNPASS : 1];
+    (void)dold;
     if (DG && dxadd) {
 #pragma unroll
       for (int t = 0; t < DNT; ++t)
 #pragma unroll
         for (int ps = 0; ps < DNPASS; ++ps) {
           const int rowi = ps * DPIXPASS + dpix;
-          const long gp = dpix0 + t * 16 + rowi;
-          const bool ok = dxb && dxacc && rowi < 16 && gp < a.npix;
+          long gp;
+          const bool in = dxpix(t, rowi, gp);
+          const bool ok = dxb && dxacc && rowi < 16 && in;
           dold[DG ? t : 0][DG ? ps : 0].u = ok ? *reinterpret_cast<const uint4*>(dxb + (size_t)gp * dxld2) : make_uint4(0, 0, 0, 0);
         }
       __builtin_amdgcn_sched_barrier(0);
     }
-    if (tile + (int)gridDim.x < a.ntiles) prefetch(tile + gridDim.x);
+    auto dgrad_phase = [&]() {
+      f32x4 dacc[NCI][DNT];
+#pragma unroll
+      for (int j = 0; j < NCI; ++j)
+#pragma unroll
+        for (int t = 0; t < DNT; ++t) dacc[j][t] = (f32x4){0.f, 0.f, 0.f, 0.f};
+      if constexpr (DG3) {
+        const char* const dbase = sy + ((wave * (TH / 4)) * YW + p) * PSY + ((q * 8) & (COUT_C - 1)) * 2;
+        half8 db[2][DNT];
+        auto ldb = [&](int buf, int k) {
+#pragma unroll
+          for (int t = 0; t < DNT; ++t)
+            db[buf][t] = *reinterpret_cast<const half8*>(dbase + ((t >> 1) * YW + (t & 1) * 16) * PSY + dboff3(k));
+        };
+        ldb(0, 0);
+#pragma unroll
+        for (int k = 0; k < DKS; ++k) {
+          if (k + 1 < DKS) ldb((k + 1) & 1, k + 1);
+          __builtin_amdgcn_sched_barrier(0);
+#pragma unroll
+          for (int j = 0; j < NCI; ++j)
+#pragma unroll
+            for (int t = 0; t < DNT; ++t)
+              dacc[j][t] = __builtin_amdgcn_mfma_f32_16x16x32_f16(wa[DG3 ? k % RING : 0][DG3 ? j : 0], db[k & 1][t], dacc[j][t], 0, 0, 0);
+          if (k + RING < DKS) lda(k % RING, k + RING);
+          __builtin_amdgcn_sched_barrier(0);
+        }
+      } else {
+        half8 db[DNT][DKS];
+#pragma unroll
+        for (int t = 0; t < DNT; ++t)
+#pragma unroll
+          for (int k = 0; k < DKS; ++k)
+            db[t][k] = *reinterpret_cast<const half8*>(sy + ((wave * DNT + t) * 16 + p) * PSY + dboff[DG && !DG3 ? k : 0]);
+#pragma unroll
+        for (int k = 0; k < DKS; ++k)
+#pragma unroll
+          for (int j = 0; j < NCI; ++j)
+#pragma unroll
+            for (int t = 0; t < DNT; ++t)
+              dacc[j][t] = __builtin_amdgcn_mfma_f32_16x16x32_f16(wf[DG && !DG3 ? k : 0][DG && !DG3 ? j : 0], db[t][k], dacc[j][t], 0, 0, 0);
+      }
+      typedef uint2 __attribute__((may_alias)) uint2_a;
+      typedef uint4 __attribute__((may_alias)) uint4_a;
+      char* const xs = sdx + wave * (16 * DXROW);
+      char* const xw = xs + p * DXROW + q * (DNC * 2);
+      const int rrow = dpix < 16 ? dpix : 15;
+      auto lds_order = []() {
+        __builtin_amdgcn_fence(__ATOMIC_RELEASE, "wavefront", "local");
+        __builtin_amdgcn_wave_barrier();
+        __builtin_amdgcn_fence(__ATOMIC_ACQUIRE, "wavefront", "local");
+      };
+#pragma unroll
+      for (int t = 0; t < DNT; ++t) {
+        union { half2_ h[DNC / 2]; uint2 u2[DNC / 4]; } hv;
+#pragma unroll
+        for (int j = 0; j < NCI; ++j) {
+          const f32x2 lo = {dacc[j][t][0], dacc[j][t][1]}, hi = {dacc[j][t][2], dacc[j][t][3]};
+          hv.h[j * 2] = __builtin_convertvector(lo, half2_);
+          hv.h[j * 2 + 1] = __builtin_convertvector(hi, half2_);
+        }
+        lds_order();
+#pragma unroll
+        for (int j = 0; j < NCI; ++j) reinterpret_cast<uint2_a*>(xw)[j] = hv.u2[j];
+        lds_order();
+#pragma unroll
+        for (int ps = 0; ps < DNPASS; ++ps) {
+          const int rowi = ps * DPIXPASS + dpix;
+          const int rr = ps * DPIXPASS + rrow < 16 ? ps * DPIXPASS + rrow : 15;
+          DU4 v;
+          v.u = *reinterpret_cast<const uint4_a*>(xs + rr * DXROW + dpiece * 16);
+          long gp;
+          const bool in = dxpix(t, rowi, gp);
+          if (dxadd) {
+#pragma unroll
+            for (int k = 0; k < 4; ++k)
+              v.h[k] = __builtin_convertvector(__builtin_convertvector(v.h[k], f32x2) + __builtin_convertvector(dold[DG ? t : 0][DG ? ps : 0].h[k], f32x2), half2_);
+          }
+          if (dxb && rowi < 16 && in) *reinterpret_cast<uint4*>(dxb + (size_t)gp * dxld2) = v.u;
+        }
+      }
+    };
+    if (DG3) dgrad_phase();
+    if (tile + (int)gridDim.x < a.ntiles) {
+      prefetch(tile + gridDim.x);
+    } else if (DG3) {
+#pragma unroll
+      for (int i = 0; i < NPX; ++i) pfx[i] = make_uint4(0, 0, 0, 0);
+#pragma unroll
+      for (int i = 0; i < NPY; ++i) pfy[i] = pfr[BN1 ? i : 0] = make_uint4(0, 0, 0, 0);
+      vnext = 0;
+    }
     if constexpr (!NOX) {
     const int kpix = 4 * q + qq;
     half8 af[2][MTC], bf[2];
     auto load_a = [&](int buf, int r) {
 #pragma unroll
       for (int m = 0; m < MTC; ++m) {
-        const char* b0 = sy + (r * TW + kpix) * PSY + (m * 16 + 4 * pp) * 2;
+        const char* b0 = sy + ((r + YO) * YW + kpix + YO) * PSY + (m * 16 + 4 * pp) * 2;
         af[buf][m] = tr_frag(b0, b0 + 16 * PSY);
       }
     };
@@ -436,64 +587,7 @@
       }
     }
     }
-    if (DG) {
-      half8 db[DNT][DKS];
-#pragma unroll
-      for (int t = 0; t < DNT; ++t)
-#pragma unroll
-        for (int k = 0; k < DKS; ++k)
-          db[t][k] = *reinterpret_cast<const half8*>(sy + ((wave * DNT + t) * 16 + p) * PSY + dboff[DG ? k : 0]);
-      f32x4 dacc[NCI][DNT];
-#pragma unroll
-      for (int j = 0; j < NCI; ++j)
-#pragma unroll
-        for (int t = 0; t < DNT; ++t) dacc[j][t] = (f32x4){0.f, 0.f, 0.f, 0.f};
-#pragma unroll
-      for (int k = 0; k < DKS; ++k)
-#pragma unroll
-        for (int j = 0; j < NCI; ++j)
-#pragma unroll
-          for (int t = 0; t < DNT; ++t)
-            dacc[j][t] = __builtin_amdgcn_mfma_f32_16x16x32_f16(wf[DG ? k : 0][DG ? j : 0], db[t][k], dacc[j][t], 0, 0, 0);
-      typedef uint2 __attribute__((may_alias)) uint2_a;
-      typedef uint4 __attribute__((may_alias)) uint4_a;
-      char* const xs = sdx + wave * (16 * DXROW);
-      char* const xw = xs + p * DXROW + q * (DNC * 2);
-      const int rrow = dpix < 16 ? dpix : 15;
-      auto lds_order = []() {
-        __builtin_amdgcn_fence(__ATOMIC_RELEASE, "wavefront", "local");
-        __builtin_amdgcn_wave_barrier();
-        __builtin_amdgcn_fence(__ATOMIC_ACQUIRE, "wavefront", "local");
-      };
-#pragma unroll
-      for (int t = 0; t < DNT; ++t) {
-        union { half2_ h[DNC / 2]; uint2 u2[DNC / 4]; } hv;
-#pragma unroll
-        for (int j = 0; j < NCI; ++j) {
-          const f32x2 lo = {dacc[j][t][0], dacc[j][t][1]}, hi = {dacc[j][t][2], dacc[j][t][3]};
-          hv.h[j * 2] = __builtin_convertvector(lo, half2_);
-          hv.h[j * 2 + 1] = __builtin_convertvector(hi, half2_);
-        }
-        lds_order();
-#pragma unroll
-        for (int j = 0; j < NCI; ++j) reinterpret_cast<uint2_a*>(xw)[j] = hv.u2[j];
-        lds_order();
-#pragma unroll
-        for (int ps = 0; ps < DNPASS; ++ps) {
-          const int rowi = ps * DPIXPASS + dpix;
-          const int rr = ps * DPIXPASS + rrow < 16 ? ps * DPIXPASS + rrow : 15;
-          DU4 v;
-          v.u = *reinterpret_cast<const uint4_a*>(xs + rr * DXROW + dpiece * 16);
-          const long gp = dpix0 + t * 16 + rowi;
-          if (dxadd) {
-#pragma unroll
-            for (int k = 0; k < 4; ++k)
-              v.h[k] = __builtin_convertvector(__builtin_convertvector(v.h[k], f32x2) + __builtin_convertvector(dold[DG ? t : 0][DG ? ps : 0].h[k], f32x2), half2_);
-          }
-          if (dxb && rowi < 16 && gp < a.npix) *reinterpret_cast<uint4*>(dxb + (size_t)gp * dxld2) = v.u;
-        }
-      }
-    }
+    if (DG && !DG3) dgrad_phase();
   }
 
   if (BNF == 2 && ci_chunk == 0) {
@@ -510,16 +604,19 @@
   }
   if constexpr (NOX) return;
   float* slab = a.slabs + (size_t)blockIdx.x * TAPS * a.cout_p * a.cin_p;
+  int ts = tid;
+  if (DG3) asm volatile("" : "+v"(ts));
+  const int swave = ts >> 6, sp_ = ts & 15, sq = (ts & 63) >> 4;
 #pragma unroll
   for (int c = 0; c < CPW; ++c) {
-    const int col = wave + 4 * c;
+    const int col = swave + 4 * c;
     if (col < NCOL) {
       const int cit = col / TAPS, tap = col - cit * TAPS;
 #pragma unroll
       for (int m = 0; m < MTC; ++m)
 #pragma unroll
         for (int r = 0; r < 4; ++r) {
-          const int co = co0 + m * 16 + q * 4 + r, ci = ci0 + cit * 16 + p;
+          const int co = co0 + m * 16 + sq * 4 + r, ci = ci0 + cit * 16 + sp_;
           slab[((size_t)tap * a.cout_p + co) * a.cin_p + ci] = acc[NOX ? 0 : m][NOX ? 0 : c][r];
         }
     }
@@ -632,6 +729,9 @@
         else hipLaunchKernelGGL((conv_wgrad_kernel<KS, STRIDE, NCI, MTC, 13>), dim3(gx, gy), dim3(256), 0, s, a);
       } else if (a.xs.nseg > 0) hipLaunchKernelGGL((conv_wgrad_kernel<KS, STRIDE, NCI, MTC, 7>), dim3(gx, gy), dim3(256), 0, s, a);
       else hipLaunchKernelGGL((conv_wgrad_kernel<KS, STRIDE, NCI, MTC, 5>), dim3(gx, gy), dim3(256), 0, s, a);
+    } else if constexpr (KS == 3 && STRIDE == 1 && ((NCI == 1 && MTC == 1) || (NCI == 2 && MTC == 2) || (NCI == 4 && MTC == 2))) {
+      if (!a.raw || !a.x || !a.dx || a.xs.nseg > 0 || a.dxs.nseg > 0 || gy != a.nci_chunks) return DY_ERR_ARG;
+      hipLaunchKernelGGL((conv_wgrad_kernel<KS, STRIDE, NCI, MTC, 5>), dim3(gx, gy), dim3(256), 0, s, a);
     } else return DY_ERR_ARG;
   } else if (a.raw && a.xs.nseg > 0) {
     if constexpr (KS == 1) hipLaunchKernelGGL((conv_wgrad_kernel<KS, STRIDE, NCI, MTC, 3>), dim3(gx, gy), dim3(256), 0, s, a);
@@ -816,6 +916,30 @@
   snprintf(out, cap, "conv_wgrad_kernel<1, 1, %d, %d, %d>", pl.nci, pl.mtc, segs ? 7 : 5);
   return DY_OK;
 }
+static WgDgPlan wgrad_dgrad3_plan(int n, int h, int w, int cin, int cout) {
+  WgDgPlan r{};
+  if (n < 1 || h < 1 || w < 1 || cin < 8 || (cin & 7) || cout < 16 || (cout & 15) || cout > 32) return r;
+  int cp, op, nci, mtc;
+  wgrad_geometry(cin, cout, 3, 1, &cp, &op, &nci, &mtc, (long)n * h * w);
+  if (16 * mtc != op) return r;
+  if (!((nci == 1 && mtc == 1) || (nci == 2 && mtc == 2) || (nci == 4 && mtc == 2))) return r;
+  int gcin, gcout, cc, nch, mt, ng, kst, pe;
+  if (dy_conv_geometry(cout, cin, 3, 1, &gcin, &gcout, &cc, &nch, &mt, &ng, &kst, &pe) != DY_OK) return r;
+  if (gcin != cout || cc != cout || nch != 1 || kst != (9 * cout + 31) / 32 || gcout < cp) return r;
+  r.ok = 1; r.nci = nci; r.mtc = mtc; r.dg_mt = mt; r.dg_rows = gcout;
+  return r;
+}
+extern "C" int dy_conv3x3_wgrad_dgrad_supported(int n, int h, int w, int cin, int cout) { return wgrad_dgrad3_plan(n, h, w, cin, cout).ok; }
+extern "C" int dy_conv3x3_wgrad_dgrad_selected(int n, int h, int w, int cin, int cout) {
+  const WgDgPlan pl = wgrad_dgrad3_plan(n, h, w, cin, cout);
+  return pl.ok && pl.nci != 4;
+}
+extern "C" int dy_wgrad_dgrad3_kernel_name(int n, int h, int w, int cin, int cout, char* out, int cap) {
+  const WgDgPlan pl = wgrad_dgrad3_plan(n, h, w, cin, cout);
+  if (!out || cap < 8 || !pl.ok) return DY_ERR_ARG;
+  snprintf(out, cap, "conv_wgrad_kernel<3, 1, %d, %d, 5>", pl.nci, pl.mtc);
+  return DY_OK;
+}
 static bool dgrad_segs_valid(const DySegs* xs, const DySegs* dxs) {
   if (!xs || !dxs || dxs->nseg != xs->nseg) return false;
   for (int k = 0; k < dxs->nseg; ++k) {
@@ -884,6 +1008,25 @@
   WgBnHost bn{raw, nullptr, coef, acc, dgamma, dbeta, ldraw, count};
   bn.wt = w_packed_t; bn.dx = dx; bn.lddx = lddx; bn.dx_acc = dx_accumulate != 0;
   return conv_wgrad_impl(x, ldx, dy, lddy, slabs, dw, n, h, w, cin, cout, 1, 1, accumulate, 0, 0, 0, stream, &bn);
+}
+extern "C" int dy_conv3x3_wgrad_dgrad_bn(const void* x, int ldx, const void* dy, int lddy, const void* raw, int ldraw, const float* coef,
+                                         const double* acc, float* dgamma, float* dbeta, float count, float* slabs, float* dw,
+                                         const void* w_packed_t, void* dx, int lddx, int dx_accumulate, int n, int h, int w, int cin,
+                                         int cout, int accumulate, hipStream_t stream) {
+  if (!raw || !coef || !acc || (ldraw & 7) || ((uintptr_t)raw & 15)) return DY_ERR_ARG;
+  if (!w_packed_t || ((uintptr_t)w_packed_t & 15) || !dx || ((uintptr_t)dx & 15) || (lddx & 7) || lddx < cin) return DY_ERR_ARG;
+  if (!wgrad_dgrad3_plan(n, h, w, cin, cout).ok) return DY_ERR_ARG;
+  auto disjoint = [&](const void* a_, long pa, long wa, const void* b_, long pb, long wb) {
+    const long a = (long)(uintptr_t)a_, b = (long)(uintptr_t)b_, np = (long)n * h * w;
+    if (a + np * pa <= b || b + np * pb <= a) return true;
+    if (pa != pb) return false;
+    const long d = ((b - a) % pa + pa) % pa;
+    return d >= wa && d + wb <= pa;
+  };
+  if (!disjoint(dx, lddx * 2L, cin * 2L, dy, lddy * 2L, cout * 2L) || !disjoint(dx, lddx * 2L, cin * 2L, raw, ldraw * 2L, cout * 2L)) return DY_ERR_ARG;
+  WgBnHost bn{raw, nullptr, coef, acc, dgamma, dbeta, ldraw, count};
+  bn.wt = w_packed_t; bn.dx = dx; bn.lddx = lddx; bn.dx_acc = dx_accumulate != 0;
+  return conv_wgrad_impl(x, ldx, dy, lddy, slabs, dw, n, h, w, cin, cout, 3, 1, accumulate, 0, 0, 0, stream, &bn);
 }
 extern "C" int dy_conv1x1_wgrad_dgrad_bn_segs(const DySegs* xs, const void* dy, int lddy, const void* raw, int ldraw, const float* coef,
                                               const double* acc, float* dgamma, float* dbeta, float count, float* slabs, float* dw,
@@ -953,8 +1096,9 @@
     if (bn->xs) a.xs = *bn->xs;
     a.dy_csplit = bn->dy_csplit; a.dy_plane = bn->dy_plane;
     if (bn->wt) {
-      const WgDgPlan pl = wgrad_dgrad_plan(n, h, w, cin, cout);
-      if (!pl.ok || pl.nci != nci || pl.mtc != mtc || ks != 1 || ld_taps) return DY_ERR_ARG;
+      if (stride != 1 || ld_taps || (ks == 3 && (bn->dxs || bn->xs || dgrad_only))) return DY_ERR_ARG;
+      const WgDgPlan pl = ks == 1 ? wgrad_dgrad_plan(n, h, w, cin, cout) : wgrad_dgrad3_plan(n, h, w, cin, cout);
+      if (!pl.ok || pl.nci != nci || pl.mtc != mtc) return DY_ERR_ARG;
       a.wt = (const f16*)bn->wt; a.dx = (f16*)bn->dx; a.lddx = bn->lddx; a.dx_acc = bn->dx_acc;
       a.dg_mt = pl.dg_mt; a.dg_rows = pl.dg_rows;
       if (bn->dxs) a.dxs = *bn->dxs;
diff --git a/experiment-yolo_amd/ultralytics/hip/__init__.py b/experiment-yolo_amd/ultralytics/hip/__init__.py
--- a/experiment-yolo_amd/ultralytics/hip/__init__.py
+++ b/experiment-yolo_amd/ultralytics/hip/__init__.py
@@ -139,6 +139,10 @@
     "dy_conv1x1_wgrad_dgrad_supported": (i32, [i32, i32, i32, i32, i32]),
     "dy_wgrad_dgrad_kernel_name": (i32, [i32, i32, i32, i32, i32, i32, C.c_char_p, i32]),
     "dy_conv1x1_wgrad_dgrad_bn": (i32, [vp, i32, vp, i32, vp, i32, vp, vp, vp, vp, f32, vp, vp, vp, vp, i32, i32, i32, i32, i32, i32, i32, i32, vp]),
+    "dy_conv3x3_wgrad_dgrad_supported": (i32, [i32, i32, i32, i32, i32]),
+    "dy_conv3x3_wgrad_dgrad_selected": (i32, [i32, i32, i32, i32, i32]),
+    "dy_wgrad_dgrad3_kernel_name": (i32, [i32, i32, i32, i32, i32, C.c_char_p, i32]),
+    "dy_conv3x3_wgrad_dgrad_bn": (i32, [vp, i32, vp, i32, vp, i32, vp, vp, vp, vp, f32, vp, vp, vp, vp, i32, i32, i32, i32, i32, i32, i32, i32, vp]),
     "dy_conv1x1_wgrad_dgrad_bn_segs": (i32, [C.POINTER(DySegs), vp, i32, vp, i32, vp, vp, vp, vp, f32, vp, vp, vp, C.POINTER(DySegs), i32, i32,
                                              i32, i32, i32, i32, vp]),
     "dy_conv1x1_wgrad_dgrad_bn_planes": (i32, [C.POINTER(DySegs), vp, i32, vp, vp, i32, i32, vp, i32, vp, vp, vp, vp, f32, vp, vp, vp, vp, i32, i32,
diff --git a/experiment-yolo_amd/ultralytics/hip/engine.py b/experiment-yolo_amd/ultralytics/hip/engine.py
--- a/experiment-yolo_amd/ultralytics/hip/engine.py
+++ b/experiment-yolo_amd/ultralytics/hip/engine.py
@@ -42,6 +42,7 @@
 HEAD_APPLY = HEAD_DECODE and os.environ.get("DY_SILU_FAST", "1") != "0" and os.environ.get("DY_HEAD_APPLY", "1") != "0"
 BN_DGRED = BN_WGRAD and os.environ.get("DY_BN_DGRED", "0") != "0"
 WGRAD_DGRAD = BN_WGRAD and not BN_DGRED and os.environ.get("DY_WGRAD_DGRAD", "1") != "0"
+WGRAD_DGRAD3 = WGRAD_DGRAD and os.environ.get("DY_WGRAD_DGRAD3", "1") != "0"
 FROZEN_DGRAD = BN_WGRAD and not BN_DGRED and os.environ.get("DY_FROZEN_DGRAD", "1") != "0"
 BN_DGRED_MAXC = int(os.environ.get("DY_BN_DGRED_MAXC", "64"))
 BN_DGRED_MAXPIX = int(os.environ.get("DY_BN_DGRED_MAXPIX", str(1 << 40)))
@@ -959,7 +960,7 @@
         side_small = bool(not frozen and SIDE_SMALL and npix <= SIDE_SMALL and self.deferred_wgrad is not None and not self.cur_sid and not self.side_wgrad
                           and acc and isinstance(x, Act) and x.needs_grad and spec.ld is None)
         bn_wgrad = bool(not frozen and acc and BN_WGRAD and spec.act == DY_ACT_SILU and not self.side_wgrad and not side_small and raw.ld == spec.cout)
-        if bn_wgrad and self._wgrad_dgrad_ok(spec, x):
+        if bn_wgrad and self._wgrad_dgrad_ok(spec, x, y.gptr, y.ld, raw):
             draw = None
         elif ((self.side_wgrad or side_small) and self.deferred_wgrad is not None) or self.cur_sid:
             draw = self.transient((npix * spec.cout_phys,), torch.float16)
@@ -995,7 +996,23 @@
         self.call("dy_conv1x1_dgrad_bn", dy_ptr, planes[0] if planes else 0, lddy, planes[1] if planes else 0, raw.ptr, raw.ld,
                   spec.coef.data_ptr(), spec.acc_b.data_ptr(), float(npix), spec.wpack_t.data_ptr(), *dx, dxs, x.N, x.H, x.W, spec.cin, spec.cout)
 
-    def _wgrad_dgrad_ok(self, spec, x):
+    @staticmethod
+    def _strided_disjoint(a, pa, wa, b, pb, wb, npix):
+        if a + npix * pa <= b or b + npix * pb <= a:
+            return True
+        if pa != pb:
+            return False
+        d = (b - a) % pa
+        return d >= wa and d + wb <= pa
+
+    def _wgrad_dgrad_ok(self, spec, x, dy_ptr=None, lddy=0, raw=None):
+        if (WGRAD_DGRAD3 and spec.ks == 3 and spec.stride == 1 and spec.ld is None and type(x) is Act and x.needs_grad and dy_ptr is not None
+                and not self.cur_sid and not self.side_wgrad and spec.cout == spec.cout_phys and spec.cin == spec.cin_phys):
+            if not self.L.dy_conv3x3_wgrad_dgrad_selected(x.N, x.H, x.W, spec.cin, spec.cout):
+                return False
+            n = x.npix
+            return (self._strided_disjoint(x.gptr, x.ld * 2, spec.cin * 2, dy_ptr, lddy * 2, spec.cout * 2, n)
+                    and self._strided_disjoint(x.gptr, x.ld * 2, spec.cin * 2, raw.ptr, raw.ld * 2, spec.cout * 2, n))
         if not (WGRAD_DGRAD and spec.ks == 1 and spec.stride == 1 and spec.ld is None and isinstance(x, (Act, SegAct)) and x.needs_grad
                 and not self.cur_sid and not self.side_wgrad and spec.cout == spec.cout_phys and spec.cin == spec.cin_phys):
             return False
@@ -1025,7 +1042,7 @@
             self.fork()
         if bn is not None and bn[1] is None:
             raw, _, coef, accb, gw, gb, cnt = bn
-            assert not side and self._wgrad_dgrad_ok(spec, x)
+            assert not side and self._wgrad_dgrad_ok(spec, x, dy_ptr, lddy, raw)
             seg = isinstance(x, SegAct)
             if seg:
                 accs = [q.grad_target() if q.needs_grad else 0 for q in x.parts]
@@ -1035,7 +1052,11 @@
                 dxs, dx = None, (x.gptr, x.ld, int(acc))
             tail = (x.N, x.H, x.W, spec.cin, spec.cout, accumulate_w)
             wt = spec.wpack_t.data_ptr()
-            if planes is not None:
+            if spec.ks == 3:
+                assert planes is None and not seg
+                self.call("dy_conv3x3_wgrad_dgrad_bn", x.ptr, x.ld, dy_ptr, lddy, raw.ptr, raw.ld, coef, accb, gw, gb, cnt, slabs.data_ptr(), dw,
+                          wt, *dx, *tail)
+            elif planes is not None:
                 self.call("dy_conv1x1_wgrad_dgrad_bn_planes", C.byref(self._segs(x)) if seg else None, 0 if seg else x.ptr, 0 if seg else x.ld,
                           dy_ptr, planes[0], lddy, planes[1], raw.ptr, raw.ld, coef, accb, gw, gb, cnt, slabs.data_ptr(), dw, wt, *dx, dxs, *tail)
             elif seg:
diff --git a/experiment-yolo_amd/ultralytics/hip/train.py b/experiment-yolo_amd/ultralytics/hip/train.py
--- a/experiment-yolo_amd/ultralytics/hip/train.py
+++ b/experiment-yolo_amd/ultralytics/hip/train.py
@@ -665,7 +665,8 @@
             own = int(args[9]) * int(args[10]) * e * 2
         return key, alg, own
 
-    _FUSED_BWD = {"dy_conv1x1_wgrad_dgrad_bn": 17, "dy_conv1x1_wgrad_dgrad_bn_segs": 14, "dy_conv1x1_wgrad_dgrad_bn_planes": 21}
+    _FUSED_BWD = {"dy_conv1x1_wgrad_dgrad_bn": 17, "dy_conv1x1_wgrad_dgrad_bn_segs": 14, "dy_conv1x1_wgrad_dgrad_bn_planes": 21,
+                  "dy_conv3x3_wgrad_dgrad_bn": 17}
 
     def _fused_bwd_shape(self, name, args):
         i = self._FUSED_BWD[name]
@@ -684,7 +685,10 @@
         if name in self._FUSED_BWD:
             n, h, w, cin, cout, old = self._fused_bwd_shape(name, args)
             seg = name.endswith("segs") or (name.endswith("planes") and args[0] is not None)
-            if L.dy_wgrad_dgrad_kernel_name(n, h, w, cin, cout, int(seg), buf, 128) == 0:
+            if name == "dy_conv3x3_wgrad_dgrad_bn":
+                if L.dy_wgrad_dgrad3_kernel_name(n, h, w, cin, cout, buf, 128) == 0:
+                    return buf.value.decode(), n * h * w * (2 * (cin + cout) + old) * 2
+            elif L.dy_wgrad_dgrad_kernel_name(n, h, w, cin, cout, int(seg), buf, 128) == 0:
                 return buf.value.decode(), n * h * w * (2 * (cin + cout) + (0 if seg else old)) * 2
         if name == "dy_conv1x1_dgrad_bn":
             n, h, w, cin, cout = args[14:19]
diff --git a/include/dealyolo_hip.h b/include/dealyolo_hip.h
--- a/include/dealyolo_hip.h
+++ b/include/dealyolo_hip.h
@@ -108,6 +108,13 @@
                                      float count, float* slabs, float* dw, const void* w_packed_t, void* dx, int lddx,
                                      int dx_accumulate, const DySegs* dxs, int n, int h, int w, int cin, int cout, int accumulate,
                                      hipStream_t stream);
+int dy_conv3x3_wgrad_dgrad_supported(int n, int h, int w, int cin, int cout);
+int dy_conv3x3_wgrad_dgrad_selected(int n, int h, int w, int cin, int cout);
+int dy_wgrad_dgrad3_kernel_name(int n, int h, int w, int cin, int cout, char* out, int cap);
+int dy_conv3x3_wgrad_dgrad_bn(const void* x, int ldx, const void* dy, int lddy, const void* raw, int ldraw, const float* coef,
+                              const double* acc, float* dgamma, float* dbeta, float count, float* slabs, float* dw,
+                              const void* w_packed_t, void* dx, int lddx, int dx_accumulate, int n, int h, int w, int cin, int cout,
+                              int accumulate, hipStream_t stream);
 int dy_conv1x1_dgrad_bn_supported(int n, int h, int w, int cin, int cout);
 int dy_dgrad_only_kernel_name(int n, int h, int w, int cin, int cout, int segs, char* out, int cap);
 int dy_conv1x1_dgrad_bn(const void* dy, const void* dy2, int lddy, int csplit, const void* raw, int ldraw, const float* coef,
```

Result: no change. 6181 images/s, median of 6 (+1.0%).
